# cambyse/po-rrt

Hardware: AMD Instinct MI355X
Metric: RRT node-expansions/sec on map_benchmark.pgm (higher is better)
Workload: dtype f64

## Files before the change

### po_rrt_amd/csrc/porrt_device.hpp

```cpp
#pragma once
#include <hip/hip_runtime.h>
#include <stdint.h>
#include <string>
#include <vector>
#include "../../include/porrt_hip.h"

namespace porrt {

template <int NEV>
struct ScopedEvents {
    hipEvent_t e[NEV];
    ScopedEvents() { for (int i = 0; i < NEV; ++i) e[i] = nullptr; }
    hipError_t create() {
        for (int i = 0; i < NEV; ++i) { const hipError_t r = hipEventCreate(&e[i]); if (r != hipSuccess) return r; }
        return hipSuccess;
    }
    ~ScopedEvents() { for (int i = 0; i < NEV; ++i) if (e[i]) (void)hipEventDestroy(e[i]); }
    ScopedEvents(const ScopedEvents &) = delete;
    ScopedEvents &operator=(const ScopedEvents &) = delete;
};

template <class Launch, class GoingOn>
static int sweep_to_fixpoint(hipStream_t stream, uint32_t *flags, size_t rows, int cur, Launch &&launch, GoingOn &&going_on, const char *who,
                             uint64_t &sweeps, std::string &err) {
    std::vector<uint32_t> h_flags(8 * rows), changed;
    hipError_t e;
    for (sweeps = 0;;) {
        if ((e = hipMemsetAsync(flags, 0, h_flags.size() * sizeof(uint32_t), stream)) != hipSuccess) break;
        for (uint32_t k = 0; k < 8; ++k, cur ^= 1) launch(k, cur);
        if ((e = hipMemcpyAsync(h_flags.data(), flags, h_flags.size() * sizeof(uint32_t), hipMemcpyDeviceToHost, stream)) != hipSuccess) break;
        if ((e = hipStreamSynchronize(stream)) != hipSuccess || (e = hipGetLastError()) != hipSuccess) break;
        sweeps += 8;
        changed.clear();
        for (size_t r = 0; r < rows; ++r) if (h_flags[8 * r + 7]) changed.push_back((uint32_t)r);
        if (changed.empty()) return PORRT_OK;
        if (sweeps > 16u * 1000u * 1000u) { err = std::string(who) + ": no fixpoint"; return PORRT_ERR_DEVICE; }
        if ((e = going_on(changed)) != hipSuccess) break;
    }
    err = std::string(who) + ": sweeps: " + hipGetErrorString(e);
    return PORRT_ERR_DEVICE;
}

constexpr int kConnectWaves = 4;
constexpr uint32_t kTileRMax = 31;
constexpr int kEmpty = 0x7FFFFFFF;
constexpr uint32_t kOnG = 0x80000000u;
constexpr int kParentPending = -2;

enum : uint32_t {
    ERR_RASTER = 1u,
    ERR_CAND_OVERFLOW = 2u,
    ERR_RNG_RETRY = 4u,
    ERR_EDGE_OVERFLOW = 8u,
    ERR_GPATH_OVERFLOW = 16u,
    ERR_PAGE_OVERFLOW = 32u,
    ERR_TIE_POOL = 64u
};

enum : uint8_t { CLS_FREE = 0, CLS_LOW = 1, CLS_HIGH = 2, CLS_HIGH0 = 3 , CLS_ZONE = 16, CLS_BAD = 255 };

struct __attribute__((aligned(8))) KdRec {
    double x, y;
    int child[2];
};

struct __attribute__((aligned(32))) KdBox {
    double lox, hix, loy, hiy;
};

struct KdMove {
    uint32_t t;
    int cur;
    uint32_t side, dcur, gex;
    bool onpath;
    double vx, vy;
    KdBox box;
};

struct Counters {
    uint32_t n_final;
    uint32_t n_edges;
    uint32_t err;
    uint32_t tie_fallbacks;
    unsigned long long finality;
    uint32_t g_len;
    uint32_t n_heavy;
    uint32_t g_nd_len;
    uint32_t g_first_dup[2];
    uint32_t n_pages;
    uint32_t kd_done;
    uint32_t pend_cnt, pool_n;
    uint32_t n_deferred, pend_lo;
    uint32_t n_losers;
    uint32_t kd_snap;
    uint32_t dbg[4];
    uint32_t clone_n;
    uint32_t clone_k[64];
    uint32_t coop_bar;
    uint32_t coop_filed;
    uint32_t coop_abort;
    uint32_t sched_stop;
    uint32_t sched_iter;
    uint32_t n_lca;
    uint32_t lca_next;
    unsigned long long tim[16];
};

#ifdef PORRT_TIMING
#define PORRT_T0() unsigned long long t__0 = wall_clock64()
#define PORRT_TACC(rc, slot)                                                                          \
    do {                                                                                              \
        const unsigned long long t__1 = wall_clock64();                                               \
        if ((threadIdx.x & 63u) == 0u) { atomicAdd(&(rc).cnt->tim[slot], t__1 - t__0); atomicAdd(&(rc).cnt->tim[(slot) + 8], 1ull); } \
        t__0 = t__1;                                                                                  \
    } while (0)
#else
#define PORRT_T0() do {} while (0)
#define PORRT_TACC(rc, slot) do {} while (0)
#endif
#ifndef PORRT_TIMING_FROM
#define PORRT_TIMING_FROM 0
#endif
#ifndef PORRT_TIMING_UNTIL
#define PORRT_TIMING_UNTIL 0x7FFFFFFF
#endif
#if defined(PORRT_TIMING) && PORRT_TIMING == 1
#define PORRT_TACC_A(rc, slot) do { if (b >= (uint32_t)PORRT_TIMING_FROM && b < (uint32_t)PORRT_TIMING_UNTIL) PORRT_TACC(rc, slot); else t__0 = wall_clock64(); } while (0)
#define PORRT_TACC_B(rc, slot) do { (void)t__0; } while (0)
#elif defined(PORRT_TIMING)
#define PORRT_TACC_A(rc, slot) do { (void)t__0; } while (0)
#define PORRT_TACC_B(rc, slot) do { if (b >= (uint32_t)PORRT_TIMING_FROM && b < (uint32_t)PORRT_TIMING_UNTIL) PORRT_TACC(rc, slot); else t__0 = wall_clock64(); } while (0)
#else
#define PORRT_TACC_A(rc, slot) do {} while (0)
#define PORRT_TACC_B(rc, slot) do {} while (0)
#endif
#if defined(PORRT_TIMING) && PORRT_TIMING == 3
#undef PORRT_TACC_B
#define PORRT_TACC_B(rc, slot) do { (void)t__0; } while (0)
#define PORRT_TACC_C(rc, slot) PORRT_TACC(rc, slot)
#elif defined(PORRT_TIMING)
#define PORRT_TACC_C(rc, slot) do { (void)t__0; } while (0)
#else
#define PORRT_TACC_C(rc, slot) do {} while (0)
#endif

#if defined(PORRT_TIMING) && PORRT_TIMING == 4
#undef PORRT_TACC_B
#define PORRT_TACC_B(rc, slot) do { (void)t__0; } while (0)
#define PORRT_TACC_H(rc, slot) do { if (b >= (uint32_t)PORRT_TIMING_FROM && b < (uint32_t)PORRT_TIMING_UNTIL) PORRT_TACC(rc, slot); else t__0 = wall_clock64(); } while (0)
#define PORRT_TACC_S(rc, slot) do { if (TeamT::kSize == 64 && b >= (uint32_t)PORRT_TIMING_FROM && b < (uint32_t)PORRT_TIMING_UNTIL) PORRT_TACC(rc, slot); else t__0 = wall_clock64(); } while (0)
#elif defined(PORRT_TIMING)
#define PORRT_TACC_H(rc, slot) do { (void)t__0; } while (0)
#define PORRT_TACC_S(rc, slot) PORRT_TACC_B(rc, slot)
#else
#define PORRT_TACC_H(rc, slot) do {} while (0)
#define PORRT_TACC_S(rc, slot) do {} while (0)
#endif

struct BestCost {
    unsigned long long cost_bits;
    uint32_t final_id, path_len, overflow, pad;
};

typedef float flt2 __attribute__((ext_vector_type(2)));
struct RunConst {
    double *nx, *ny;
    int *rep;
    flt2 *rep_f;
    double bx0, by0, binv_w, binv_h;
    uint32_t *rg_cnt;
    unsigned long long *rg_occ;
    uint32_t *rg_dir;
    double *pg_xy;
    int *pg_id;
    double *pg_d;
    uint32_t *slot_of;
    uint32_t rg_maxp, pg_cap;
    double *distA, *distB;
    int *parent;
    unsigned long long *reachA, *reachB;
    uint8_t *vid;
    uint8_t *final_flag;
    unsigned long long *final_mask;
    uint32_t *n_at;
    unsigned long long *valid_mask;
    Counters *cnt;
    double *sx, *sy;
    uint32_t *sworld;
    const double *inj_xy;
    unsigned long long inj_base, inj_n;
    double *q_x, *q_y;
    double *kq_x, *kq_y;
    int *kq_vid;
    int *q_nn;
    int *q_vid;
    uint32_t *cand_cnt;
    int *cand_id;
    double *cand_val;
    double *cand_xy;
    uint32_t cand_cap;
    uint32_t cand_K;
    const double *rad_T2;
    uint32_t *e_from, *e_to, *e_tv;
    uint32_t e_cap;
    KdRec *kd_rec;
    KdBox *kd_box;
    KdBox *loc_box;
    uint32_t loc_stride;
    KdMove *kd_losers;
    int *pend_new, *pend_pool;
    uint32_t *pend_off, *pend_n, *pend_cur, *pend_state;
    uint32_t pend_cap, pool_cap;
    int *bc_scratch;
    uint32_t bc_cap;
    uint32_t *bc_cursor;
    BestCost *bc_out;
    unsigned long long *kd_hint;
    int *kd_up;
    uint32_t *kd_depth;
    uint32_t *kd_gexit;
    int *loc_cur;
    uint32_t *loc_dcur, *loc_gex, *loc_flags, *g_nd;
    double *g_nd_x, *g_nd_y;
    KdBox *g_nd_box;
    int *g_id;
    double *g_x, *g_y;
    uint32_t g_cap;
    uint32_t *g_snap;
    double gp_x, gp_y;
    const uint8_t *cls;
    const uint32_t *sat;
    const uint8_t *clr;
    uint32_t W, H;
    double low0, low1, ppm;
    int domain, has_grid;
    int n_validities;
    unsigned long long validities[65];
    unsigned long long all_worlds;
    int goal_kind;
    uint32_t G;
    double gcx[64], gcy[64];
    unsigned long long gmask[64];
    double g_l1;
    double w2g_x[64], w2g_y[64];
    double zone_x, zone_y, visibility;
    double s_low0, s_low1, s_up0, s_up1;
    double max_step;
    int mode;
    uint16_t *perm;
    double *ssx, *ssy;
    double *bq_x, *bq_y;
    uint16_t *bq_k;
    double *t2_at;
    uint32_t tile_R;
    uint32_t part_stride;
    uint32_t q_stride;
    double start_x, start_y;
    unsigned long long root_reach;
    int root_vid;
    unsigned long long rng_st_lo, rng_st_hi, rng_inc_lo, rng_inc_hi;
    struct PcgJump *jump;
    RunConst *self;
    uint32_t *zero0;
    unsigned long long zero_words;
    uint32_t *sched_i0, *sched_nb;
    uint32_t sched_min, sched_max, sched_K, sched_steps;
    uint32_t sched_max_nodes;
    uint32_t cand_par3;
    uint32_t hint_max;
    uint32_t kd_lazy;
};

#define GPTR(T) T __attribute__((address_space(1))) *
template <class T>
__device__ __forceinline__ GPTR(T) as_global(T *p) { return (GPTR(T))(uintptr_t)p; }
template <class T>
__device__ __forceinline__ GPTR(const T) as_global(const T *p) { return (GPTR(const T))(uintptr_t)p; }
template <class T>
__device__ __forceinline__ T g_atomic_add(GPTR(T) p, T v) { return __hip_atomic_fetch_add(p, v, __ATOMIC_RELAXED, __HIP_MEMORY_SCOPE_AGENT); }
template <class T>
__device__ __forceinline__ T g_atomic_or(GPTR(T) p, T v) { return __hip_atomic_fetch_or(p, v, __ATOMIC_RELAXED, __HIP_MEMORY_SCOPE_AGENT); }
template <class T>
__device__ __forceinline__ T g_atomic_min(GPTR(T) p, T v) { return __hip_atomic_fetch_min(p, v, __ATOMIC_RELAXED, __HIP_MEMORY_SCOPE_AGENT); }

__device__ __forceinline__ uint32_t uni(uint32_t v) { return (uint32_t)__builtin_amdgcn_readfirstlane((int)v); }
__device__ __forceinline__ double uni_d(double v) {
    const unsigned long long b = (unsigned long long)__double_as_longlong(v);
    const unsigned long long lo = uni((uint32_t)b), hi = uni((uint32_t)(b >> 32));
    return __longlong_as_double((long long)(lo | (hi << 32)));
}

#ifndef PORRT_RC_SCALAR
#define PORRT_RC_SCALAR 1
#endif
__device__ __forceinline__ const RunConst &rc_const(const RunConst *p) {
#if PORRT_RC_SCALAR
    const uintptr_t a = (uintptr_t)p;
    const uintptr_t u = (uintptr_t)uni((uint32_t)a) | ((uintptr_t)uni((uint32_t)(a >> 32)) << 32);
    return *(const RunConst *)(const RunConst __attribute__((address_space(4))) *)u;
#else
    return *p;
#endif
}
__device__ __forceinline__ const RunConst &rc_const(const RunConst &rc) { return rc_const(&rc); }

__device__ __forceinline__ uint32_t row_nb(const RunConst &rc, uint32_t b, uint32_t nb_arg) {
    return rc.sched_nb ? ((GPTR(const uint32_t))(uintptr_t)rc.sched_nb)[b] : nb_arg;
}
__device__ __forceinline__ uint32_t row_i0(const RunConst &rc, uint32_t b, uint32_t i0_arg) {
// ... 204 lines not shown
    return false;
}

typedef unsigned __int128 u128;
__device__ __forceinline__ u128 mk128(unsigned long long lo, unsigned long long hi) { return ((u128)hi << 64) | lo; }

struct PcgJump {
    unsigned long long mult_lo[64], mult_hi[64], plus_lo[64], plus_hi[64];
};

__device__ __forceinline__ unsigned long long pcg_output(u128 s) {
    uint32_t rot = (uint32_t)(s >> 122);
    unsigned long long xsl = (unsigned long long)(s >> 64) ^ (unsigned long long)s;
    return (xsl >> rot) | (xsl << ((64 - rot) & 63));
}

__device__ __forceinline__ double gen_range_once(unsigned long long r, double low, double high, bool *retry) {
    double v12 = __longlong_as_double((long long)((r >> 12) | 0x3FF0000000000000ull));
    double v01 = v12 - 1.0;
    double scale = high - low;
    double prod = v01 * scale;
    double res = prod + low;
    if (!(res < high)) *retry = true;
    return res;
}

__global__ void k_gen_samples(const RunConst *__restrict__ rcp, const PcgJump *__restrict__ jt, unsigned long long it0,
                              unsigned long long n, unsigned long long st_lo, unsigned long long st_hi,
                              unsigned long long inc_lo, unsigned long long inc_hi, unsigned long long draws_before) {
    const RunConst &rc = rc_const(rcp + blockIdx.y);
    if (!jt) { jt = rc.jump; st_lo = rc.rng_st_lo; st_hi = rc.rng_st_hi; inc_lo = rc.rng_inc_lo; inc_hi = rc.rng_inc_hi; }
    unsigned long long t = (unsigned long long)blockIdx.x * blockDim.x + threadIdx.x;
    if (t >= n) return;
    if (rc.sched_nb && it0 + t >= rc.sched_max) return;
    unsigned long long idx = it0 + t;
    unsigned long long it = idx + 1;
    if (it % 100 == 0) {
        uint32_t w = rc.mode == 1 ? rc.sworld[idx] : 0u;
        double gx = 0.0, gy = 0.0;
        if (rc.goal_kind == 1) { gx = rc.w2g_x[w & 63]; gy = rc.w2g_y[w & 63]; }
        else if (rc.goal_kind == 2) { gx = rc.zone_x; gy = rc.zone_y; }
        rc.sx[idx] = gx;
        rc.sy[idx] = gy;
        return;
    }
    unsigned long long di = idx - idx / 100;
    if (rc.inj_xy) {
        unsigned long long e = rc.inj_base + di;
        if (e >= rc.inj_n) { atomicOr(&rc.cnt->err, ERR_RNG_RETRY); rc.sx[idx] = 0.0; rc.sy[idx] = 0.0; return; }
        rc.sx[idx] = rc.inj_xy[2 * e];
        rc.sy[idx] = rc.inj_xy[2 * e + 1];
        return;
    }
    (void)draws_before;
    unsigned long long delta = 2ull * di;
    u128 acc_mult = 1, acc_plus = 0;
    for (int b = 0; b < 64 && (delta >> b); ++b) {
        if ((delta >> b) & 1ull) {
            u128 m = mk128(jt->mult_lo[b], jt->mult_hi[b]), p = mk128(jt->plus_lo[b], jt->plus_hi[b]);
            acc_mult = acc_mult * m;
            acc_plus = acc_plus * m + p;
        }
    }
    const u128 MULT = mk128(0x4385DF649FCCF645ull, 0x2360ED051FC65DA4ull);
    u128 inc = mk128(inc_lo, inc_hi);
    u128 s = acc_mult * mk128(st_lo, st_hi) + acc_plus;
    bool retry = false;
    s = s * MULT + inc;
    double x = gen_range_once(pcg_output(s), rc.s_low0, rc.s_up0, &retry);
    s = s * MULT + inc;
    double y = gen_range_once(pcg_output(s), rc.s_low1, rc.s_up1, &retry);
    if (retry) atomicOr(&rc.cnt->err, ERR_RNG_RETRY);
    rc.sx[idx] = x;
    rc.sy[idx] = y;
}

constexpr int kRepLevels = 3;
__device__ __forceinline__ int rep_dim(int l) { return l == 0 ? 256 : (l == 1 ? 32 : 4); }
__device__ __forceinline__ int rep_off(int l) { return l == 0 ? 0 : (l == 1 ? 65536 : 65536 + 1024); }
constexpr int kRepTotal = 65536 + 1024 + 16;
constexpr uint32_t kRepCoarseUntil = 32768;
constexpr int kRepF = 65536 + 1024;
constexpr int kRepInts = kRepTotal + 2 * kRepF;
static_assert(kRepTotal % 2 == 0, "the positions start 8-byte aligned");

__device__ __forceinline__ void rep_cell(const RunConst &rc, double x, double y, int G, int &cx, int &cy) {
    double fx = (x - rc.bx0) * rc.binv_w * (double)G, fy = (y - rc.by0) * rc.binv_h * (double)G;
    cx = fx < 0.0 ? 0 : (fx >= (double)G ? G - 1 : (int)fx);
    cy = fy < 0.0 ? 0 : (fy >= (double)G ? G - 1 : (int)fy);
}

__device__ __forceinline__ void rep_insert(const RunConst &rc, double x, double y, int id) {
#pragma unroll
    for (int l = 0; l < kRepLevels; ++l) {
        int cx, cy;
        const int G = rep_dim(l);
        rep_cell(rc, x, y, G, cx, cy);
        rc.rep[rep_off(l) + cy * G + cx] = id;
        if (l < 2) rc.rep_f[rep_off(l) + cy * G + cx] = flt2{(float)x, (float)y};
    }
}

template <bool PTO>
__device__ __forceinline__ double nn_bound_wave(const RunConst &rc, uint32_t N, double qx, double qy, uint32_t world, uint32_t lane) {
    const double INF = __longlong_as_double(0x7FF0000000000000ll);
    double m = INF;
    for (int l = 0; l < kRepLevels; ++l) {
        const int G = rep_dim(l);
        int cx, cy;
        rep_cell(rc, qx, qy, G, cx, cy);
        int r = -1;
        if (lane < 9u) {
            const int x = cx + (int)(lane % 3u) - 1, y = cy + (int)(lane / 3u) - 1;
            if (x >= 0 && y >= 0 && x < G && y < G) r = as_global(rc.rep)[rep_off(l) + y * G + x];
        }
        double d2 = INF;
        if (r >= 0 && (uint32_t)r < N) {
            bool pass = true;
            if (PTO) pass = (as_global(rc.reachA)[r] >> world) & 1ull;
            if (pass) d2 = dist2(as_global(rc.nx)[r], as_global(rc.ny)[r], qx, qy);
        }
        for (int off = 8; off > 0; off >>= 1) {
            const double o = __shfl_xor(d2, off);
            d2 = o < d2 ? o : d2;
        }
        m = __shfl(d2, 0);
        if (m < INF) break;
    }
    if (m == INF && !PTO) m = dist2(rc.nx[0], rc.ny[0], qx, qy);
    return m;
}

__device__ __forceinline__ uint32_t rank_before(const RunConst &rc, uint32_t b, uint32_t vwords, uint32_t k);
__device__ __forceinline__ uint32_t wave_sum(uint32_t v);
__device__ void commit_rrt_sample(const RunConst &rc, uint32_t b, uint32_t vwords, uint32_t k, uint32_t lane, uint32_t stride = 64u, bool lag = false);
constexpr int kRG = 40;
constexpr uint32_t kRegions = kRG * kRG;
constexpr uint32_t kPage = 64;
constexpr uint32_t kOccWords = (kRegions + 63u) / 64u;
typedef double dbl2 __attribute__((ext_vector_type(2)));

__device__ __forceinline__ uint32_t region_of(const RunConst &rc, double x, double y) {
    int cx, cy;
    rep_cell(rc, x, y, kRG, cx, cy);
    return (uint32_t)(cy * kRG + cx);
}

__device__ __forceinline__ double disc_radius(double bound_d2, double qx, double qy) {
    return sqrt(bound_d2) * (1.0 + 1e-9) + 1e-12 * (1.0 + fabs(qx) + fabs(qy));
}

template <class Visit>
__device__ __forceinline__ void scan_disc(const RunConst &rc, uint32_t b, double qx, double qy, double rho, uint32_t N, uint32_t lane, Visit visit,
                                          uint32_t skip_region = 0xFFFFFFFFu) {
    int cx0, cy0, cx1, cy1;
    rep_cell(rc, qx - rho, qy - rho, kRG, cx0, cy0);
    rep_cell(rc, qx + rho, qy + rho, kRG, cx1, cy1);
    const uint32_t x0 = uni((uint32_t)cx0), y0 = uni((uint32_t)cy0);
    const uint32_t w = uni((uint32_t)(cx1 - cx0 + 1)), nreg = w * uni((uint32_t)(cy1 - cy0 + 1));
    if (nreg * 16u > N) {
        auto gx = as_global(rc.nx), gy = as_global(rc.ny);
        for (uint32_t j0 = 0; j0 < N; j0 += 128u) {
            double x[2], y[2];
#pragma unroll
            for (int u = 0; u < 2; ++u) {
                const uint32_t j = j0 + 64u * u + lane;
                x[u] = gx[j < N ? j : 0u];
                y[u] = gy[j < N ? j : 0u];
            }
#pragma unroll
            for (int u = 0; u < 2; ++u)
                if (j0 + 64u * u < N) visit(x[u], y[u], (int)(j0 + 64u * u + lane), j0 + 64u * u + lane < N);
        }
        return;
    }
    auto gcnt = as_global(rc.rg_cnt) + (b & 1u) * kRegions;
    auto gdir = as_global(rc.rg_dir);
    auto gxy = as_global(reinterpret_cast<const dbl2 *>(rc.pg_xy));
    auto gid = as_global(rc.pg_id);
    for (uint32_t r0 = 0; r0 < nreg; r0 += 64) {
        const uint32_t r = r0 + lane;
        uint32_t reg = 0, cnt = 0;
        if (r < nreg) {
            const uint32_t ry = r / w;
            reg = (y0 + ry) * kRG + x0 + (r - ry * w);
            cnt = reg == skip_region ? 0u : gcnt[reg];
        }
        const uint32_t npg = (uint32_t)__popcll(__ballot(cnt > 0u));
        if (__ballot(cnt >= npg || cnt > kPage) == 0ull && npg > 1u) {
            uint32_t cmax = cnt;
            for (int off = 32; off > 0; off >>= 1) {
                const uint32_t o = __shfl_xor(cmax, off);
                cmax = o > cmax ? o : cmax;
            }
            cmax = uni(cmax);
            for (uint32_t s0 = 0; s0 < cmax; s0 += 2) {
                dbl2 v[2];
                int id[2];
#pragma unroll
                for (int u = 0; u < 2; ++u) {
                    const uint32_t sl = s0 + u < cnt ? s0 + u : 0u;
                    v[u] = gxy[(size_t)reg * kPage + sl];
                    id[u] = gid[(size_t)reg * kPage + sl];
                }
#pragma unroll
                for (int u = 0; u < 2; ++u)
                    if (s0 + u < cmax) visit(v[u].x, v[u].y, id[u], s0 + u < cnt);
            }
            continue;
        }
        uint32_t page = reg;
        for (uint32_t j = 0;; ++j) {
            unsigned long long m = __ballot(cnt > j * kPage);
            if (!m) break;
            if (j && cnt > j * kPage) page = gdir[(size_t)reg * rc.rg_maxp + j];
            while (m) {
                uint32_t pg[2], pc[2];
#pragma unroll
                for (int u = 0; u < 2; ++u) {
                    pg[u] = 0; pc[u] = 0;
                    if (m) {
                        const uint32_t l = (uint32_t)__builtin_ctzll(m);
                        m &= m - 1;
                        pg[u] = (uint32_t)__builtin_amdgcn_readlane((int)page, (int)l);
                        const uint32_t c = (uint32_t)__builtin_amdgcn_readlane((int)cnt, (int)l) - j * kPage;
                        pc[u] = c < kPage ? c : kPage;
                    }
                }
                dbl2 v[2];
                int id[2];
#pragma unroll
                for (int u = 0; u < 2; ++u) {
                    const bool ld = lane < pc[u];
                    v[u] = ld ? gxy[(size_t)pg[u] * kPage + lane] : dbl2{0.0, 0.0};
                    id[u] = ld ? gid[(size_t)pg[u] * kPage + lane] : -1;
                }
#pragma unroll
                for (int u = 0; u < 2; ++u)
                    if (pc[u]) visit(v[u].x, v[u].y, id[u], lane < pc[u]);
            }
        }
    }
}

template <bool PTO>
__device__ __forceinline__ void near_sample(const RunConst &rc, uint32_t b, uint32_t i0, uint32_t vwords, uint32_t k, uint32_t lane) {
    const uint32_t N = uni(as_global(rc.n_at)[b]);
    const double sqx = uni_d(as_global(rc.sx)[i0 + k]), sqy = uni_d(as_global(rc.sy)[i0 + k]);
    uint32_t world = 0;
    if (PTO) world = uni(as_global(rc.sworld)[i0 + k]);
    const double INF = __longlong_as_double(0x7FF0000000000000ll);
    double bestD = INF;
    int best = 0x7FFFFFFF;
    const double T2 = rc.rad_T2[N + (rc.mode == 1 ? 1u : 0u)];
    {
        auto reach = as_global(rc.reachA);
        double thr = INF;
        auto visit = [&](double x, double y, int id, bool ok) {
            if (!ok) return;
            const double d2 = dist2(x, y, sqx, sqy);
            if (d2 > thr) return;
            bool pass = true;
            if (PTO) pass = (reach[id] >> world) & 1ull;
            if (!pass) return;
            const double D = sqrt(d2);
            if (D < bestD || (D == bestD && id < best)) { bestD = D; best = id; thr = d2 * (1.0 + 1e-15); }
        };
        auto wave_best = [&]() {
            double rd = bestD;
            int ri = best;
            for (int off = 32; off > 0; off >>= 1) {
                const double od = __shfl_xor(rd, off);
                const int oi = __shfl_xor(ri, off);
                if (od < rd || (od == rd && oi < ri)) { rd = od; ri = oi; }
            }
            const unsigned long long own = __ballot(best == ri && bestD == rd);
            const int src = own ? (int)__builtin_ctzll(own) : 0;
            thr = __shfl(thr, src);
            bestD = rd; best = ri;
        };
        const uint32_t own = uni(region_of(rc, sqx, sqy));
        scan_disc(rc, b, sqx, sqy, 0.0, N, lane, visit);
        wave_best();
        double m2;
        if (best != 0x7FFFFFFF) m2 = thr;
        else { m2 = nn_bound_wave<PTO>(rc, N, sqx, sqy, world, lane); thr = m2 * (1.0 + 1e-9); }
        scan_disc(rc, b, sqx, sqy, disc_radius(m2, sqx, sqy), N, lane, visit, own);
        wave_best();
    }
    const int nn = best == 0x7FFFFFFF ? 0 : best;
    const double fx = as_global(rc.nx)[nn], fy = as_global(rc.ny)[nn];
    double tx = sqx, ty = sqy;
    double step = fabs(tx - fx);
    step += fabs(ty - fy);
    if (step > rc.max_step) {
        const double lambda = rc.max_step / step;
        double ux = (tx - fx) * lambda, uy = (ty - fy) * lambda;
        tx = fx + ux;
        ty = fy + uy;
    }
    uint32_t err = 0;
    int vid = 0;
    bool valid = true;
    if (rc.has_grid) {
        int cls = state_class(rc, tx, ty, &err);
        if (rc.mode == 0) valid = cls == CLS_FREE;
        else { vid = class_to_validity(rc, cls); valid = vid >= 0; }
        if (err) valid = false;
    }
    if (lane == 0) {
        const uint32_t qo = q_off(rc, b);
        as_global(rc.q_x)[qo + k] = tx;
        as_global(rc.q_y)[qo + k] = ty;
        const size_t o2 = (size_t)b * rc.part_stride + k;
        as_global(rc.kq_x)[o2] = tx; as_global(rc.kq_y)[o2] = ty; as_global(rc.kq_vid)[o2] = valid ? vid : -1;
        as_global(rc.q_nn)[qo + k] = nn;
        as_global(rc.q_vid)[qo + k] = valid ? vid : -1;
        if (valid) atomicOr(&rc.valid_mask[(size_t)b * vwords + (k >> 6)], 1ull << (k & 63u));
        if (err) atomicOr(&rc.cnt->err, err);
    }
    if (!valid) return;
    auto cid = as_global(rc.cand_id) + cand_off(rc, b, k);
    auto cxy = as_global(reinterpret_cast<dbl2 *>(rc.cand_xy)) + cand_off(rc, b, k);
    const uint32_t cap = rc.cand_cap;
    uint32_t tot = 0;
    bool over = false;
    scan_disc(rc, b, tx, ty, disc_radius(T2, tx, ty), N, lane, [&](double x, double y, int id, bool ok) {
        const bool in = ok && dist2(x, y, tx, ty) <= T2;
        const unsigned long long hm = __ballot(in);
        const uint32_t pos = tot + (uint32_t)__popcll(hm & ((1ull << lane) - 1ull));
        if (in) {
            if (pos < cap) {
                cid[pos] = id;
                dbl2 v;
                v.x = x; v.y = y;
                cxy[pos] = v;
            } else {
                over = true;
            }
        }
        tot += (uint32_t)__popcll(hm);
    });
    if (lane == 0) as_global(rc.cand_cnt)[cand_cnt_at(rc, b, k)] = tot;
    if (over) atomicOr(&rc.cnt->err, (uint32_t)ERR_CAND_OVERFLOW);
}

template <bool PTO>
__global__ __launch_bounds__(256) void k_near(const RunConst *__restrict__ rcp, uint32_t b, uint32_t i0, uint32_t nb, uint32_t vwords, uint32_t cb,
                                              uint32_t cnb) {
    const RunConst &rc = rcp[blockIdx.y];
    const uint32_t lane = threadIdx.x & 63u;
    const uint32_t near_blocks = (nb + 3u) / 4u;
    if (blockIdx.x >= near_blocks) {
        const uint32_t ck = uni((blockIdx.x - near_blocks) * 4u + (threadIdx.x >> 6));
        if (!PTO && ck < cnb && ck < row_nb(rc, cb, cnb)) commit_rrt_sample(rc, cb, vwords, ck, lane);
        return;
    }
    const uint32_t k = uni(blockIdx.x * 4u + (threadIdx.x >> 6));
    if (k >= row_nb(rc, b, nb)) return;
    near_sample<PTO>(rc, b, row_i0(rc, b, i0), vwords, k, lane);
}

constexpr uint32_t kInsertLds = kRegions * 4u + 4096u * 2u + 16u;
template <int TAG = 0>
__device__ void insert_step_pages(const RunConst &rc_arg, uint32_t b, uint32_t nb, uint32_t vwords, uint8_t *scratch) {
    const RunConst &rc = TAG == 1 ? rc_const(rc_arg) : rc_arg;
    uint32_t *s_add = reinterpret_cast<uint32_t *>(scratch);
    uint16_t *s_off = reinterpret_cast<uint16_t *>(scratch + kRegions * 4u);
    uint32_t &s_np = *reinterpret_cast<uint32_t *>(scratch + kRegions * 4u + 4096u * 2u);
    uint32_t &s_base = *reinterpret_cast<uint32_t *>(scratch + kRegions * 4u + 4096u * 2u + 4u);
    const uint32_t T = blockDim.x;
    auto rg_old = as_global(rc.rg_cnt) + (b & 1u) * kRegions, rg_new = as_global(rc.rg_cnt) + ((b + 1u) & 1u) * kRegions;
    for (uint32_t r = threadIdx.x; r < kRegions; r += T) s_add[r] = 0;
    if (threadIdx.x < 64u) {
        uint32_t add = threadIdx.x < vwords ? (uint32_t)__popcll(as_global(rc.valid_mask)[(size_t)b * vwords + threadIdx.x]) : 0u;
        add = wave_sum(add);
        if (threadIdx.x == 0) {
        s_np = 0; s_base = kRegions + rc.cnt->n_pages;
        const uint32_t n_next = as_global(rc.n_at)[b] + add;
        as_global(rc.n_at)[b + 1] = n_next;
        as_global(rc.t2_at)[b + 1] = as_global(rc.rad_T2)[n_next];
        }
    }
    __syncthreads();
    const uint32_t qo = q_off(rc, b);
    for (uint32_t k = threadIdx.x; k < nb; k += T)
        if (rc.q_vid[qo + k] >= 0) s_off[k] = (uint16_t)atomicAdd(&s_add[region_of(rc, as_global(rc.q_x)[qo + k], as_global(rc.q_y)[qo + k])], 1u);
    __syncthreads();
    for (uint32_t r = threadIdx.x; r < kRegions; r += T) {
        const uint32_t add = s_add[r];
        if (!add) continue;
        const uint32_t old = rg_old[r];
        const uint32_t p_old = old ? (old + kPage - 1) / kPage : 1u, p_new = (old + add + kPage - 1) / kPage;
        if (p_new > p_old) {
            const uint32_t need = p_new - p_old;
            const uint32_t at = s_base + atomicAdd(&s_np, need);
            if (at + need > rc.pg_cap || p_new > rc.rg_maxp) { atomicOr(&rc.cnt->err, (uint32_t)ERR_PAGE_OVERFLOW); continue; }
            for (uint32_t i = 0; i < need; ++i) as_global(rc.rg_dir)[(size_t)r * rc.rg_maxp + p_old + i] = at + i;
        }
    }
    __syncthreads();
    if (rc.cnt->err & ERR_PAGE_OVERFLOW) return;
    const uint32_t N = as_global(rc.n_at)[b];
    dbl2 *pxy = reinterpret_cast<dbl2 *>(rc.pg_xy);
    for (uint32_t k = threadIdx.x; k < nb; k += T) {
        if (rc.q_vid[qo + k] < 0) continue;
        const double x = as_global(rc.q_x)[qo + k], y = as_global(rc.q_y)[qo + k];
        const uint32_t r = region_of(rc, x, y);
        const uint32_t slot = rg_old[r] + s_off[k], j = slot / kPage;
        const uint32_t page = j ? __hip_atomic_load(&rc.rg_dir[(size_t)r * rc.rg_maxp + j], __ATOMIC_RELAXED, __HIP_MEMORY_SCOPE_AGENT) : r;
        dbl2 v;
        v.x = x; v.y = y;
        pxy[(size_t)page * kPage + (slot % kPage)] = v;
        const uint32_t nid = N + rank_before(rc, b, vwords, k);
        as_global(rc.pg_id)[(size_t)page * kPage + (slot % kPage)] = (int)nid;
        as_global(rc.slot_of)[nid] = page * kPage + (slot % kPage);
        if (rc.q_stride) { as_global(rc.nx)[nid] = x; as_global(rc.ny)[nid] = y; }
    }
    __syncthreads();
    for (uint32_t r = threadIdx.x; r < kRegions; r += T) rg_new[r] = rg_old[r] + s_add[r];
    if (threadIdx.x < kOccWords) {
        unsigned long long w = 0;
        for (uint32_t i = 0; i < 64u; ++i) {
            const uint32_t r = threadIdx.x * 64u + i;
            if (r < kRegions && rg_old[r] + s_add[r] > 0u) w |= 1ull << i;
        }
        as_global(rc.rg_occ)[((b + 1u) & 1u) * kOccWords + threadIdx.x] = w;
    }
    if (threadIdx.x == 0) rc.cnt->n_pages += s_np;
}

constexpr uint32_t kFileLds = 2u * kRegions * 4u + 4096u * 2u + 64u * 8u + 66u * 4u + 32u;
template <uint32_t T = 1024u>
__device__ void file_step_fast(const RunConst &rc_arg, uint32_t b, uint32_t nb, uint32_t vwords, uint8_t *scratch) {
    const RunConst &rc = rc_const(rc_arg);
    uint32_t *s_add = reinterpret_cast<uint32_t *>(scratch);
    uint32_t *s_old = s_add + kRegions;
    uint16_t *s_off = reinterpret_cast<uint16_t *>(s_old + kRegions);
    unsigned long long *s_word = reinterpret_cast<unsigned long long *>(s_off + 4096);
    uint32_t *s_pref = reinterpret_cast<uint32_t *>(s_word + 64);
    uint32_t *s_misc = s_pref + 66;
    constexpr uint32_t SPT = 4u;
    const uint32_t tid = threadIdx.x, qo = q_off(rc, b);
    auto rg_old = as_global(rc.rg_cnt) + (b & 1u) * kRegions, rg_new = as_global(rc.rg_cnt) + ((b + 1u) & 1u) * kRegions;
    int vid[SPT];
    double x[SPT], y[SPT];
#pragma unroll
    for (uint32_t q = 0; q < SPT; ++q) {
        const uint32_t k = tid + q * T;
        vid[q] = k < nb ? as_global(rc.q_vid)[qo + k] : -1;
        x[q] = k < nb ? as_global(rc.q_x)[qo + k] : 0.0;
        y[q] = k < nb ? as_global(rc.q_y)[qo + k] : 0.0;
    }
    constexpr uint32_t RPT = (kRegions + T - 1u) / T;
    uint32_t oldc[RPT];
#pragma unroll
    for (uint32_t h = 0; h < RPT; ++h) oldc[h] = tid + h * T < kRegions ? rg_old[tid + h * T] : 0u;
    const unsigned long long word = tid < vwords ? as_global(rc.valid_mask)[(size_t)b * vwords + tid] : 0ull;
    uint32_t n_pages = 0, N0 = 0;
    if (tid == T - 1u) { n_pages = rc.cnt->n_pages; N0 = as_global(rc.n_at)[b]; }
#pragma unroll
    for (uint32_t h = 0; h < RPT; ++h) if (tid + h * T < kRegions) { s_add[tid + h * T] = 0; s_old[tid + h * T] = oldc[h]; }
    if (tid < 64u) s_word[tid] = word;
    if (tid == T - 1u) { s_misc[0] = 0; s_misc[1] = kRegions + n_pages; s_misc[2] = 0; s_misc[3] = N0; }
    __syncthreads();
    double t2_next = 0.0;
    if (tid == 0) {
        uint32_t acc = 0;
        for (uint32_t w = 0; w < vwords; ++w) { s_pref[w] = acc; acc += (uint32_t)__popcll(s_word[w]); }
        const uint32_t n_next = s_misc[3] + acc;
        as_global(rc.n_at)[b + 1] = n_next;
        t2_next = as_global(rc.rad_T2)[n_next];
    }
    uint32_t reg[SPT];
#pragma unroll
    for (uint32_t q = 0; q < SPT; ++q) {
        reg[q] = 0;
        if (vid[q] >= 0) { reg[q] = region_of(rc, x[q], y[q]); s_off[tid + q * T] = (uint16_t)atomicAdd(&s_add[reg[q]], 1u); }
    }
    __syncthreads();
#pragma unroll
    for (uint32_t h = 0; h < RPT; ++h) {
        const uint32_t r = tid + h * T;
        const uint32_t add = r < kRegions ? s_add[r] : 0u;
        if (!add) continue;
        const uint32_t old = s_old[r];
        const uint32_t p_old = old ? (old + kPage - 1) / kPage : 1u, p_new = (old + add + kPage - 1) / kPage;
        if (p_new > p_old) {
            const uint32_t need = p_new - p_old;
            const uint32_t at = s_misc[1] + atomicAdd(&s_misc[0], need);
            if (at + need > rc.pg_cap || p_new > rc.rg_maxp) { atomicOr(&rc.cnt->err, (uint32_t)ERR_PAGE_OVERFLOW); s_misc[2] = 1u; continue; }
            for (uint32_t i = 0; i < need; ++i) as_global(rc.rg_dir)[(size_t)r * rc.rg_maxp + p_old + i] = at + i;
        }
    }
    __threadfence_block();
    __syncthreads();
    if (s_misc[2]) return;
    const uint32_t N = s_misc[3];
    dbl2 *pxy = reinterpret_cast<dbl2 *>(rc.pg_xy);
#pragma unroll
    for (uint32_t q = 0; q < SPT; ++q) {
        if (vid[q] < 0) continue;
        const uint32_t k = tid + q * T, r = reg[q];
        const uint32_t slot = s_old[r] + s_off[k], j = slot / kPage;
        const uint32_t page = j ? __hip_atomic_load(&rc.rg_dir[(size_t)r * rc.rg_maxp + j], __ATOMIC_RELAXED, __HIP_MEMORY_SCOPE_AGENT) : r;
        dbl2 v;
        v.x = x[q]; v.y = y[q];
        pxy[(size_t)page * kPage + (slot % kPage)] = v;
        const uint32_t nid = N + s_pref[k >> 6] + (uint32_t)__popcll(s_word[k >> 6] & ((1ull << (k & 63u)) - 1ull));
        as_global(rc.pg_id)[(size_t)page * kPage + (slot % kPage)] = (int)nid;
        as_global(rc.slot_of)[nid] = page * kPage + (slot % kPage);
        as_global(rc.nx)[nid] = x[q];
        as_global(rc.ny)[nid] = y[q];
    }
#pragma unroll
    for (uint32_t h = 0; h < RPT; ++h) {
        const uint32_t r = tid + h * T;
        if (r < kRegions) rg_new[r] = s_old[r] + s_add[r];
    }
    if (tid < kOccWords) {
        unsigned long long w = 0;
        for (uint32_t i = 0; i < 64u; ++i) {
            const uint32_t r = tid * 64u + i;
            if (r < kRegions && s_old[r] + s_add[r] > 0u) w |= 1ull << i;
        }
        as_global(rc.rg_occ)[((b + 1u) & 1u) * kOccWords + tid] = w;
    }
    if (tid == 0) { as_global(rc.t2_at)[b + 1] = t2_next; rc.cnt->n_pages += s_misc[0]; }
}

__device__ __forceinline__ uint32_t rank_before(const RunConst &rc, uint32_t b, uint32_t vwords, uint32_t k) {
    uint32_t r = 0;
    auto vm = as_global(rc.valid_mask) + (size_t)b * vwords;
    for (uint32_t w = 0; w < (k >> 6); ++w) r += __popcll(vm[w]);
    r += __popcll(vm[k >> 6] & ((1ull << (k & 63u)) - 1ull));
    return r;
}
template <int CTRL>
__device__ __forceinline__ uint32_t dpp_u32(uint32_t v) { return (uint32_t)__builtin_amdgcn_update_dpp((int)v, (int)v, CTRL, 0xF, 0xF, false); }
template <int CTRL>
__device__ __forceinline__ double dpp_f64(double v) {
    const unsigned long long b = (unsigned long long)__double_as_longlong(v);
    const unsigned long long lo = dpp_u32<CTRL>((uint32_t)b), hi = dpp_u32<CTRL>((uint32_t)(b >> 32));
    return __longlong_as_double((long long)(lo | (hi << 32)));
}
constexpr int kDppRowRor = 0x120;
constexpr int kDppRowBcast = 0x150;
#ifndef PORRT_DPP
#define PORRT_DPP 1
#endif

__device__ __forceinline__ uint32_t rank_before_lanes(const RunConst &rc, uint32_t b, uint32_t vwords, uint32_t k, uint32_t lane, uint32_t stride) {
    auto vm = as_global(rc.valid_mask) + (size_t)b * vwords;
    const uint32_t wk = k >> 6;
    uint32_t r = 0;
    for (uint32_t w0 = 0; w0 <= wk; w0 += stride) {
        const uint32_t w = w0 + lane;
        unsigned long long v = w <= wk ? vm[w] : 0ull;
        if (w == wk) v &= (1ull << (k & 63u)) - 1ull;
        r += (uint32_t)__popcll(v);
    }
    if (PORRT_DPP && stride == 16u) {
        r += dpp_u32<kDppRowRor + 8>(r); r += dpp_u32<kDppRowRor + 4>(r); r += dpp_u32<kDppRowRor + 2>(r); r += dpp_u32<kDppRowRor + 1>(r);
        return r;
    }
    for (uint32_t off = stride >> 1; off > 0; off >>= 1) r += (uint32_t)__shfl_xor((int)r, (int)off);
    return r;
}

__device__ __forceinline__ TileGrid load_tile(const RunConst &rc, uint8_t *tile, double px, double py, uint32_t lane, uint32_t stride) {
    TileGrid g;
    g.lds = tile; g.glob = rc.cls; g.W = rc.W; g.TW = 2u * rc.tile_R + 1u;
    uint32_t ci, cj;
    to_pixel(rc, px, py, ci, cj);
    g.oi = (int)ci - (int)rc.tile_R;
    g.oj = (int)cj - (int)rc.tile_R;
    const uint32_t n = g.TW * g.TW;
    for (uint32_t t = lane; t < n; t += stride) {
        const uint32_t ri = t / g.TW, rj = t - ri * g.TW;
        const int i = g.oi + (int)ri, j = g.oj + (int)rj;
        uint8_t c = CLS_BAD;
        if (i >= 0 && j >= 0 && (uint32_t)i < rc.H && (uint32_t)j < rc.W) c = as_global(rc.cls)[(uint32_t)i * rc.W + (uint32_t)j];
        tile[t] = c;
    }
    return g;
}

template <class T>
__device__ __forceinline__ T wave_min_u(T v) {
    for (int off = 32; off > 0; off >>= 1) {
        T o = __shfl_xor(v, off);
        v = o < v ? o : v;
    }
    return v;
}
__device__ __forceinline__ uint32_t wave_sum(uint32_t v) {
    for (int off = 32; off > 0; off >>= 1) v += __shfl_xor(v, off);
    return v;
}
__device__ __forceinline__ unsigned long long wave_or(unsigned long long v) {
    for (int off = 32; off > 0; off >>= 1) v |= __shfl_xor(v, off);
    return v;
}

__device__ __forceinline__ bool kd_left(double x, double y, double wx, double wy, uint32_t depth) {
    return (depth & 1u) ? (y < wy) : (x < wx);
}

__device__ bool kd_preorder_less(const RunConst &rc, int u, int v) {
    const uint32_t gu = as_global(rc.kd_gexit)[u], gv = as_global(rc.kd_gexit)[v];
    const bool ou = gu & kOnG, ov = gv & kOnG;
    const uint32_t iu = gu & ~kOnG, iv = gv & ~kOnG;
    if (ou && ov) return iu < iv;
    if (ou) {
        if (iu <= iv) return true;
        return !kd_left(as_global(rc.nx)[v], as_global(rc.ny)[v], as_global(rc.g_x)[iv], as_global(rc.g_y)[iv], iv);
    }
    if (ov) {
        if (iv <= iu) return false;
        return kd_left(as_global(rc.nx)[u], as_global(rc.ny)[u], as_global(rc.g_x)[iu], as_global(rc.g_y)[iu], iu);
    }
    if (iu != iv) {
        if (iu < iv) return kd_left(as_global(rc.nx)[u], as_global(rc.ny)[u], as_global(rc.g_x)[iu], as_global(rc.g_y)[iu], iu);
        return !kd_left(as_global(rc.nx)[v], as_global(rc.ny)[v], as_global(rc.g_x)[iv], as_global(rc.g_y)[iv], iv);
    }
    int a = u, b = v;
    uint32_t da = as_global(rc.kd_depth)[a], db = as_global(rc.kd_depth)[b];
    int a_from = -1, b_from = -1;
    while (da > db) { const int p = as_global(rc.kd_up)[a]; a_from = as_global(rc.kd_rec)[p].child[1] == a; a = p; --da; }
    while (db > da) { const int p = as_global(rc.kd_up)[b]; b_from = as_global(rc.kd_rec)[p].child[1] == b; b = p; --db; }
    if (a == b) return a_from >= 0 ? false : true;
    while (a != b) {
        const int pa = as_global(rc.kd_up)[a], pb = as_global(rc.kd_up)[b];
        a_from = as_global(rc.kd_rec)[pa].child[1] == a;
        b_from = as_global(rc.kd_rec)[pb].child[1] == b;
        a = pa; b = pb;
    }
    return a_from < b_from;
}

template <int W>
struct Team {
    static constexpr bool kOneWave = W == 1;
    static constexpr uint32_t kSize = W * 64u;
    double *scr_d;
    int *scr_i;
    uint32_t wave, lane;
    __device__ __forceinline__ uint32_t tl() const { return wave * 64u + lane; }
    __device__ __forceinline__ uint32_t sub() const { return lane; }
    __device__ __forceinline__ unsigned long long ballot(bool p) const { return __ballot(p); }
    template <class T>
    __device__ __forceinline__ T shfl(T v, int src) const { return __shfl(v, src); }
    __device__ __forceinline__ void sync() const { if (W > 1) __syncthreads(); }
    __device__ __forceinline__ uint32_t sum(uint32_t v) const {
        v = wave_sum(v);
        if (W == 1) return v;
        sync();
        if (lane == 0) scr_i[wave] = (int)v;
        sync();
        uint32_t t = 0;
#pragma unroll
        for (int w = 0; w < W; ++w) t += (uint32_t)scr_i[w];
        return t;
    }
    __device__ __forceinline__ int min_i(int v) const {
        v = wave_min_u(v);
// ... 726 lines not shown

__global__ __launch_bounds__(1024) void k_file_commit(const RunConst *__restrict__ rcp, uint32_t bf, uint32_t nbf, uint32_t cb, uint32_t cnb, uint32_t vwords) {
    __shared__ __attribute__((aligned(16))) uint8_t s_ins[kFileLds];
    const RunConst &rc = rcp[blockIdx.y];
    if (blockIdx.x == 0) { file_step_fast<1024u>(rc, bf, nbf, vwords, s_ins); return; }
    const uint32_t ck = uni((blockIdx.x - 1u) * 16u + (threadIdx.x >> 6));
    if (ck < cnb) commit_rrt_sample(rc, cb, vwords, ck, threadIdx.x & 63u);
}

__device__ __forceinline__ bool coop_grid_sync(const RunConst &rc, uint32_t nblocks, uint32_t &phase) {
    __shared__ uint32_t s_go;
    __syncthreads();
    if (threadIdx.x == 0) {
        ++phase;
        const uint32_t target = phase * nblocks;
        __threadfence();
        __hip_atomic_fetch_add(&rc.cnt->coop_bar, 1u, __ATOMIC_RELEASE, __HIP_MEMORY_SCOPE_AGENT);
        const unsigned long long t0 = wall_clock64();
        uint32_t go = 1u;
        while (__hip_atomic_load(&rc.cnt->coop_bar, __ATOMIC_RELAXED, __HIP_MEMORY_SCOPE_AGENT) < target) {
            __builtin_amdgcn_s_sleep(1);
            if (wall_clock64() - t0 > 200000000ull || __hip_atomic_load(&rc.cnt->coop_abort, __ATOMIC_RELAXED, __HIP_MEMORY_SCOPE_AGENT)) {
                atomicOr(&rc.cnt->coop_abort, 1u); go = 0u; break;
            }
        }
        __builtin_amdgcn_fence(__ATOMIC_ACQUIRE, "agent");
        s_go = go;
    }
    __syncthreads();
    __builtin_amdgcn_s_dcache_inv();
    return s_go != 0u;
}

template <bool LDSGRID>
__global__ __launch_bounds__(kConnectWaves * 64) __attribute__((amdgpu_waves_per_eu(8, 8))) void k_coop_rrt(const RunConst *__restrict__ rcp, uint32_t n_steps, uint32_t K,
                                                                  uint32_t n_iter, uint32_t vwords) {
    extern __shared__ __attribute__((aligned(16))) uint8_t lds_tiles[];
    __shared__ double s_d[kConnectWaves];
    __shared__ int s_i[kConnectWaves];
    __shared__ uint32_t s_heavy[kConnectWaves];
    __shared__ __attribute__((aligned(16))) uint8_t s_ins[kFileLds];
    const RunConst &rc = rcp[0];
    const uint32_t bid = blockIdx.x, nblk = gridDim.x, lane = threadIdx.x & 63u, wv = threadIdx.x >> 6;
    uint32_t phase = 0;
    auto nb_of = [&](uint32_t b) { const uint32_t i0 = b * K; return b < n_steps ? (n_iter - i0 < K ? n_iter - i0 : K) : 0u; };
    {
        const uint32_t nb0 = nb_of(0);
        for (uint32_t it = bid; it * 4u < nb0; it += nblk) {
            const uint32_t k = uni(it * 4u + wv);
            if (k < nb0) near_sample<false>(rc, 0u, 0u, vwords, k, lane);
        }
        if (!coop_grid_sync(rc, nblk, phase)) return;
        if (bid == 0) file_step_fast<kConnectWaves * 64u>(rc, 0u, nb0, vwords, s_ins);
        if (!coop_grid_sync(rc, nblk, phase)) return;
        if (bid == 0 && threadIdx.x == 0) __hip_atomic_store(&rc.cnt->coop_filed, 1u, __ATOMIC_RELEASE, __HIP_MEMORY_SCOPE_AGENT);
    }
    for (uint32_t b = 0; b < n_steps; ++b) {
        const uint32_t nb = nb_of(b), nbn = nb_of(b + 1u), i0n = (b + 1u) * K;
        const uint32_t cb4 = (nb + kConnectWaves - 1u) / kConnectWaves, items = cb4 + (nbn + 3u) / 4u;
        for (uint32_t it = bid; it < items; it += nblk) {
            if (it < cb4) {
                connect_block<LDSGRID>(rc, b, nb, vwords, it, lds_tiles, s_d, s_i, s_heavy);
                __syncthreads();
            } else {
                const uint32_t k = uni((it - cb4) * 4u + wv);
                if (k < nbn) near_sample<false>(rc, b + 1u, i0n, vwords, k, lane);
            }
        }
        if (!coop_grid_sync(rc, nblk, phase)) return;
        const uint32_t first_commit = nbn ? 1u : 0u;
        if (nbn && bid == 0) file_step_fast<kConnectWaves * 64u>(rc, b + 1u, nbn, vwords, s_ins);
        if (bid >= first_commit) {
            for (uint32_t it = bid - first_commit; it * 4u < nb; it += nblk - first_commit) {
                const uint32_t ck = uni(it * 4u + wv);
                if (ck < nb) commit_rrt_sample(rc, b, vwords, ck, lane);
            }
        }
        if (!coop_grid_sync(rc, nblk, phase)) return;
        if (bid == 0 && threadIdx.x == 0) __hip_atomic_store(&rc.cnt->coop_filed, b + 2u, __ATOMIC_RELEASE, __HIP_MEMORY_SCOPE_AGENT);
    }
}

__device__ void commit_rrt_sample(const RunConst &rc, uint32_t b, uint32_t vwords, uint32_t k, uint32_t lane, uint32_t stride, bool lag) {
    const unsigned long long vword = as_global(rc.valid_mask)[(size_t)b * vwords + (k >> 6)];
    const uint32_t N = as_global(rc.n_at)[b];
    const uint32_t rank = stride < 64u ? rank_before_lanes(rc, b, vwords, k, lane, stride) : rank_before(rc, b, vwords, k);
    const uint32_t cnt = cand_count(rc, b, k);
    auto cid = as_global(rc.cand_id) + cand_off(rc, b, k);
    auto cval = as_global(rc.cand_val) + cand_val_off(rc, b, k);
    if (!((vword >> (k & 63u)) & 1ull)) return;
    const int id = (int)(N + rank);
    const bool odd = lag && (b & 1u);
    auto gdB = as_global(odd ? rc.distA : rc.distB);
    auto gother = as_global(reinterpret_cast<unsigned long long *>(odd ? rc.distB : rc.distA));
    auto gpd = as_global(rc.pg_d);
    auto gso = as_global(rc.slot_of);
    if (lane == 0) gpd[gso[id]] = as_global(rc.distA)[id];
    constexpr int U = 4;
    for (uint32_t a0 = lane; a0 < cnt; a0 += stride * U) {
        double via[U], dB[U];
        int j[U];
#pragma unroll
        for (int u = 0; u < U; ++u) {
            const uint32_t a = a0 + (uint32_t)u * stride;
            via[u] = a < cnt ? cval[a] : -1.0;
            j[u] = a < cnt ? cid[a] : 0;
        }
#pragma unroll
        for (int u = 0; u < U; ++u) dB[u] = via[u] >= 0.0 ? gdB[j[u]] : 0.0;
#pragma unroll
        for (int u = 0; u < U; ++u) {
            if (!(via[u] >= 0.0) || f64_bits(via[u]) != f64_bits(dB[u])) continue;
            auto gpar = as_global(rc.parent) + j[u];
            int old = *gpar;
            while (old < (int)N || id < old) {
                int expect = old;
                if (__hip_atomic_compare_exchange_strong(gpar, &expect, id, __ATOMIC_RELAXED, __ATOMIC_RELAXED, __HIP_MEMORY_SCOPE_AGENT)) break;
                old = expect;
            }
            if (lag) g_atomic_min(gother + j[u], f64_bits(via[u]));
            else as_global(rc.distA)[j[u]] = via[u];
            gpd[gso[j[u]]] = via[u];
        }
    }
}

__global__ __launch_bounds__(256) void k_commit_rrt(const RunConst *__restrict__ rcp, uint32_t b, uint32_t nb, uint32_t vwords, uint32_t lag) {
    const uint32_t k = uni((blockIdx.x * 256u + threadIdx.x) >> 6);
    if (k < nb && k < row_nb(rcp[blockIdx.y], b, nb)) commit_rrt_sample(rcp[blockIdx.y], b, vwords, k, threadIdx.x & 63u, 64u, lag != 0u);
}

template <int TAG> __device__ void g_track_step(const RunConst &rc_arg, uint32_t b, uint32_t nb, uint32_t vwords, uint8_t *lds) {
    const RunConst &rc = rc_const(rc_arg);
#ifdef PORRT_GTRACK_TIMING
    const unsigned long long gt0 = wall_clock64();
#define GT_MARK(slot) do { if (threadIdx.x == 0) { atomicAdd(&rc.cnt->tim[slot], wall_clock64() - gt0); atomicAdd(&rc.cnt->tim[(slot) + 8], 1ull); } } while (0)
#else
#define GT_MARK(slot) do {} while (0)
#endif
    constexpr uint32_t kNd = kGTrackNd;
    uint16_t *s_k = reinterpret_cast<uint16_t *>(lds);
    unsigned long long *s_cand = reinterpret_cast<unsigned long long *>(lds + 8192);
    uint32_t *s_wpre = reinterpret_cast<uint32_t *>(lds + 8192 + 512);
    double *s_blx = reinterpret_cast<double *>(lds + 8192 + 512 + 272);
    double *s_bhx = s_blx + kNd, *s_bly = s_bhx + kNd, *s_bhy = s_bly + kNd;
    uint32_t *s_ndi = reinterpret_cast<uint32_t *>(s_bhy + kNd);
    constexpr uint32_t kApp = 256, kCand = 160;
    double *s_ax = reinterpret_cast<double *>(lds + kGTrackLds0), *s_ay = s_ax + kApp;
    double *s_cx = s_ay + kApp, *s_cy = s_cx + kCand;
    const uint32_t tid = threadIdx.x, lane = tid & 63u;
    auto vm = as_global(rc.valid_mask) + (size_t)b * vwords;
    const uint32_t N = as_global(rc.n_at)[b];
    const uint32_t glen0 = rc.cnt->g_len, n_nd = rc.cnt->g_nd_len, d0 = rc.cnt->g_first_dup[0], d1 = rc.cnt->g_first_dup[1];
    if (tid < 64u) s_cand[tid] = 0ull;
    if (tid < 64u) {
        const uint32_t c = tid < vwords ? (uint32_t)__popcll(vm[tid]) : 0u;
        uint32_t inc = c;
        for (int off = 1; off < 64; off <<= 1) { const uint32_t o = (uint32_t)__shfl_up((int)inc, off); if ((int)lane >= off) inc += o; }
        if (tid < vwords) s_wpre[tid] = inc - c;
        if (tid == 63u) s_wpre[vwords] = inc;
    }
    for (uint32_t t2 = tid; t2 < n_nd && t2 < kNd; t2 += blockDim.x) {
        const KdBox bx = rc.g_nd_box[t2];
        s_ndi[t2] = as_global(rc.g_nd)[t2]; s_blx[t2] = bx.lox; s_bhx[t2] = bx.hix; s_bly[t2] = bx.loy; s_bhy[t2] = bx.hiy;
    }
    __syncthreads();
    const uint32_t n_new = s_wpre[vwords];
    for (uint32_t k = tid; k < nb; k += blockDim.x) {
        const unsigned long long w = vm[k >> 6];
        if ((w >> (k & 63u)) & 1ull) s_k[s_wpre[k >> 6] + (uint32_t)__popcll(w & ((1ull << (k & 63u)) - 1ull))] = (uint16_t)k;
    }
    __syncthreads();
    const double px = rc.gp_x, py = rc.gp_y;
    auto gex = as_global(rc.kd_gexit);
    const uint32_t qo = q_off(rc, b);
    GT_MARK(0);
    for (uint32_t t0 = tid; t0 < ((n_new + blockDim.x - 1u) / blockDim.x) * blockDim.x; t0 += 4u * blockDim.x) {
        double cvx[4], cvy[4];
        uint32_t cE[4], lo[4], hi[4];
#pragma unroll
        for (uint32_t u = 0; u < 4u; ++u) {
            const uint32_t t = t0 + u * blockDim.x;
            const uint32_t k = t < n_new ? s_k[t] : 0u;
            cvx[u] = t < n_new ? as_global(rc.q_x)[qo + k] : 0.0;
            cvy[u] = t < n_new ? as_global(rc.q_y)[qo + k] : 0.0;
            cE[u] = 0xFFFFFFFFu;
            const bool open = t < n_new && !(cvx[u] == px && cvy[u] == py);
            lo[u] = 0u; hi[u] = open ? n_nd : 0u;
        }
        for (;;) {
            bool more = false;
#pragma unroll
            for (uint32_t u = 0; u < 4u; ++u) more = more || lo[u] < hi[u];
            if (!more) break;
#pragma unroll
            for (uint32_t u = 0; u < 4u; ++u) {
                if (lo[u] >= hi[u]) continue;
                const uint32_t mid = (lo[u] + hi[u]) >> 1;
                double blx, bhx, bly, bhy;
                if (mid < kNd) { blx = s_blx[mid]; bhx = s_bhx[mid]; bly = s_bly[mid]; bhy = s_bhy[mid]; }
                else { const KdBox bx = rc.g_nd_box[mid]; blx = bx.lox; bhx = bx.hix; bly = bx.loy; bhy = bx.hiy; }
                const bool in = !(cvx[u] < blx) && cvx[u] < bhx && !(cvy[u] < bly) && cvy[u] < bhy;
                if (in) lo[u] = mid + 1u; else hi[u] = mid;
            }
        }
        GT_MARK(4);
#pragma unroll
        for (uint32_t u = 0; u < 4u; ++u) {
            const uint32_t t = t0 + u * blockDim.x;
            if (t < n_new && !(cvx[u] == px && cvy[u] == py) && lo[u] < n_nd) cE[u] = lo[u] < kNd ? s_ndi[lo[u]] : as_global(rc.g_nd)[lo[u]];
        }
#pragma unroll
        for (uint32_t u = 0; u < 4u; ++u) {
            const uint32_t t = t0 + u * blockDim.x;
            if (t >= n_new) continue;
            uint32_t E = cE[u];
            if (cvx[u] < px && d0 < E) E = d0;
            if (cvy[u] < py && d1 < E) E = d1;
            if (E != 0xFFFFFFFFu) gex[N + t] = E;
            else atomicOr(&s_cand[t >> 6], 1ull << (t & 63u));
        }
    }
    __syncthreads();
    GT_MARK(5);
    if (tid < 64u) {
        const uint32_t c = (uint32_t)__popcll(s_cand[tid]);
        uint32_t inc = c;
        for (int off = 1; off < 64; off <<= 1) { const uint32_t o = (uint32_t)__shfl_up((int)inc, off); if ((int)lane >= off) inc += o; }
        s_wpre[tid] = inc - c;
    }
    __syncthreads();
    for (uint32_t t = tid; t < n_new; t += blockDim.x) {
        const unsigned long long w = s_cand[t >> 6];
        if (!((w >> (t & 63u)) & 1ull)) continue;
        const uint32_t rank = s_wpre[t >> 6] + (uint32_t)__popcll(w & ((1ull << (t & 63u)) - 1ull));
        if (rank < kCand) { const uint32_t k = s_k[t]; s_cx[rank] = as_global(rc.q_x)[qo + k]; s_cy[rank] = as_global(rc.q_y)[qo + k]; }
    }
    __syncthreads();
    GT_MARK(1);
    if (tid < 64u) {
        uint32_t len = glen0, nd_len = n_nd, fd0 = d0, fd1 = d1;
        KdBox cell = n_nd ? rc.g_nd_box[n_nd - 1u] : g_box_all();
        auto gx = as_global(reinterpret_cast<unsigned long long *>(rc.g_x)), gy = as_global(reinterpret_cast<unsigned long long *>(rc.g_y));
        uint32_t c_at = 0;
        for (uint32_t w = 0; w < (n_new + 63u) / 64u; ++w) {
            for (unsigned long long m = s_cand[w]; m;) {
                const uint32_t t = w * 64u + (uint32_t)__builtin_ctzll(m);
                m &= m - 1ull;
                double vx, vy;
                if (c_at < kCand) { vx = s_cx[c_at]; vy = s_cy[c_at]; }
                else { const uint32_t k = s_k[t]; vx = as_global(rc.q_x)[qo + k]; vy = as_global(rc.q_y)[qo + k]; }
                ++c_at;
                uint32_t E = 0xFFFFFFFFu;
                if (!(vx == px && vy == py)) {
                    for (uint32_t l0 = glen0; l0 < len && E == 0xFFFFFFFFu; l0 += 64u) {
                        const uint32_t lvl = l0 + lane;
                        bool out = false;
                        if (lvl < len) {
                            double wx, wy;
                            if (lvl - glen0 < kApp) { wx = s_ax[lvl - glen0]; wy = s_ay[lvl - glen0]; }
                            else {
                                __builtin_amdgcn_s_waitcnt(0);
                                wx = __longlong_as_double((long long)__hip_atomic_load(gx + lvl, __ATOMIC_RELAXED, __HIP_MEMORY_SCOPE_AGENT));
                                wy = __longlong_as_double((long long)__hip_atomic_load(gy + lvl, __ATOMIC_RELAXED, __HIP_MEMORY_SCOPE_AGENT));
                            }
                            out = kd_left(vx, vy, wx, wy, lvl) != kd_left(px, py, wx, wy, lvl);
                        }
                        const unsigned long long ob = __ballot(out);
                        if (ob) E = l0 + (uint32_t)__builtin_ctzll(ob);
                    }
                }
                if (lane == 0) {
                    if (E != 0xFFFFFFFFu) {
                        gex[N + t] = E;
                    } else {
                        if (len + 8u < rc.g_cap) {
                            as_global(rc.g_id)[len] = (int)(N + t);
                            __hip_atomic_store(gx + len, (unsigned long long)__double_as_longlong(vx), __ATOMIC_RELAXED, __HIP_MEMORY_SCOPE_AGENT);
                            __hip_atomic_store(gy + len, (unsigned long long)__double_as_longlong(vy), __ATOMIC_RELAXED, __HIP_MEMORY_SCOPE_AGENT);
                        } else {
                            atomicOr(&rc.cnt->err, (uint32_t)ERR_GPATH_OVERFLOW);
                        }
                        if (len - glen0 < kApp) { s_ax[len - glen0] = vx; s_ay[len - glen0] = vy; }
                        gex[N + t] = len | kOnG;
                        if (!(vx == px && vy == py)) {
                            as_global(rc.g_nd)[nd_len] = len; as_global(rc.g_nd_x)[nd_len] = vx; as_global(rc.g_nd_y)[nd_len] = vy;
                            cell = g_box_after(cell, vx, vy, len, px, py);
                            rc.g_nd_box[nd_len] = cell;
                        }
                    }
                }
                if (E == 0xFFFFFFFFu) {
                    if (vx == px && vy == py) { if (len & 1u) fd1 = len < fd1 ? len : fd1; else fd0 = len < fd0 ? len : fd0; }
                    else ++nd_len;
                    ++len;
                }
                __builtin_amdgcn_fence(__ATOMIC_RELEASE, "workgroup", "local");
                __builtin_amdgcn_wave_barrier();
                __builtin_amdgcn_fence(__ATOMIC_ACQUIRE, "workgroup", "local");
            }
        }
        GT_MARK(2);
        if (lane == 0) {
            rc.cnt->g_len = len; rc.cnt->g_nd_len = nd_len; rc.cnt->g_first_dup[0] = fd0; rc.cnt->g_first_dup[1] = fd1;
            __threadfence();
            __hip_atomic_store(&rc.cnt->kd_done, N + n_new, __ATOMIC_RELEASE, __HIP_MEMORY_SCOPE_AGENT);
        }
        GT_MARK(3);
    }
}

__global__ __launch_bounds__(256) void k_gtrack(const RunConst *__restrict__ rcp, uint32_t b, uint32_t nb, uint32_t vwords) {
    __shared__ __attribute__((aligned(16))) uint8_t s_lds[kGTrackLds];
    const RunConst &rc = rcp[blockIdx.y];
    nb = row_nb(rc, b, nb);
    if (nb == 0) return;
    g_track_step<1>(rc, b, nb, vwords, s_lds);
}

__global__ __launch_bounds__(256) void k_kd_reset(const RunConst *__restrict__ rcp) {
    const RunConst &rc = rcp[blockIdx.y];
    for (uint32_t i = blockIdx.x * 256u + threadIdx.x; i < (uint32_t)(128 * 128); i += gridDim.x * 256u) rc.kd_hint[i] = 0ull;
    if (blockIdx.x == 0 && threadIdx.x == 0) {
        const double x = rc.nx[0], y = rc.ny[0];
        rc.cnt->g_len = 1;
        rc.cnt->g_first_dup[0] = 0xFFFFFFFFu;
        rc.cnt->g_first_dup[1] = 0xFFFFFFFFu;
        if (x == rc.gp_x && y == rc.gp_y) { rc.cnt->g_first_dup[0] = 0; rc.cnt->g_nd_len = 0; }
        else { rc.g_nd[0] = 0; rc.g_nd_x[0] = x; rc.g_nd_y[0] = y; rc.g_nd_box[0] = g_box_after(g_box_all(), x, y, 0u, rc.gp_x, rc.gp_y); rc.cnt->g_nd_len = 1; }
        rc.kd_rec[0].child[0] = kEmpty; rc.kd_rec[0].child[1] = kEmpty;
        rc.cnt->kd_done = 1;
        rc.cnt->kd_snap = 0;
        rc.cnt->n_losers = 0;
        rc.g_snap[0] = 1; rc.g_snap[1] = rc.cnt->g_nd_len; rc.g_snap[2] = rc.cnt->g_first_dup[0]; rc.g_snap[3] = rc.cnt->g_first_dup[1];
    }
}

enum : uint32_t { LOC_SIDE = 1u, LOC_ONPATH = 2u };
constexpr uint32_t kWaitFiled = 0x80000000u;
__device__ __forceinline__ bool coop_wait_filed(const RunConst &rc, uint32_t need) {
    __shared__ uint32_t s_ok;
    if (threadIdx.x == 0) {
        const unsigned long long t0 = wall_clock64();
        uint32_t ok = 1u;
        while (__hip_atomic_load(&rc.cnt->coop_filed, __ATOMIC_ACQUIRE, __HIP_MEMORY_SCOPE_AGENT) < need) {
            __builtin_amdgcn_s_sleep(64);
            if (wall_clock64() - t0 > 200000000ull || __hip_atomic_load(&rc.cnt->coop_abort, __ATOMIC_RELAXED, __HIP_MEMORY_SCOPE_AGENT)) {
                atomicOr(&rc.cnt->coop_abort, 1u); ok = 0u; break;
            }
        }
        s_ok = ok;
    }
    __syncthreads();
    return s_ok != 0u;
}
constexpr int kHG = 128;
constexpr uint32_t kHintMaxSquares = 256;

__device__ __forceinline__ KdBox load_box(const KdBox *p, size_t i) {
    auto g = as_global(p);
    KdBox b;
    b.lox = g[i].lox; b.hix = g[i].hix; b.loy = g[i].loy; b.hiy = g[i].hiy;
    return b;
}
__device__ __forceinline__ bool box_holds(const KdBox &bx, double x, double y) {
    return bx.lox <= x && x < bx.hix && bx.loy <= y && y < bx.hiy;
}
__device__ __forceinline__ void box_cut(KdBox &bx, double wx, double wy, uint32_t depth, uint32_t side) {
    if (depth & 1u) { if (side) bx.loy = wy; else bx.hiy = wy; }
    else { if (side) bx.lox = wx; else bx.hix = wx; }
}

__device__ __forceinline__ void kd_descend(const RunConst &rc, uint32_t Nsnap, double vx, double vy, int &cur, uint32_t &dcur, uint32_t &side,
                                           KdBox &bx) {
    auto grec = as_global(rc.kd_rec);
    KdRec rec;
    rec.x = grec[cur].x; rec.y = grec[cur].y; rec.child[0] = grec[cur].child[0]; rec.child[1] = grec[cur].child[1];
    for (;;) {
        box_cut(bx, rec.x, rec.y, dcur, side);
        const int c = side ? rec.child[1] : rec.child[0];
        if ((uint32_t)c >= Nsnap) break;
        rec.x = grec[c].x; rec.y = grec[c].y; rec.child[0] = grec[c].child[0]; rec.child[1] = grec[c].child[1];
        cur = c;
        dcur += 1;
        side = kd_left(vx, vy, rec.x, rec.y, dcur) ? 0u : 1u;
    }
}

constexpr uint32_t kTieParts = 8;
__device__ __forceinline__ void kd_hint_block(const RunConst &rc, uint32_t b0, uint32_t nsteps, uint32_t vwords, uint32_t bx);
template <int T>
__device__ __forceinline__ void tie_fix_block(const RunConst &rc, uint32_t part, uint32_t nparts);
template <int LPN>
__global__ __launch_bounds__(256) void k_kd_locate(const RunConst *__restrict__ rcp, uint32_t b0, uint32_t nsteps, uint32_t K, uint32_t nb_last,
                                                    uint32_t vwords, uint32_t lpar, uint32_t hb0 = 0, uint32_t hns = 0) {
// ... 804 lines not shown
```

### po_rrt_amd/csrc/porrt_engine.hip

```cpp
#include "../../include/porrt_hip.h"
#include "porrt_host.hpp"
#include "porrt_device.hpp"
#include "porrt_group.hpp"
#include "porrt_belief.hpp"
#include "porrt_dp.hpp"
#include "porrt_prm.hpp"
#include "porrt_edges.hpp"
#include "porrt_refine.hpp"
#include "porrt_refine_batch.hpp"
#include "porrt_reparent.hpp"
#include "porrt_qmdp.hpp"
#include "porrt_policy_graph.hpp"
#include "porrt_join.hpp"
#include "porrt_mm_recipe.hpp"

#include <algorithm>
#include <functional>
#include <chrono>
#include <cmath>
#include <cstdio>
#include <cstring>
#include <string>
#include <system_error>
#include <mutex>
#include <thread>
#include <unordered_map>
#include <limits>
#include <memory>
#include <vector>

template <class F> static inline auto abi_guard(F &&f) noexcept -> decltype(f()) {
    try { return f(); } catch (const std::bad_alloc &) { return PORRT_ERR_NOMEM; } catch (...) { return PORRT_ERR_INVALID; }
}

using namespace porrt;

namespace {

struct DevBufBase {
    void *vp = nullptr;
    size_t n = 0, want = 0, elem = 1;
};
template <class T>
struct DevBuf : DevBufBase {
    T *p = nullptr;
    DevBuf() { elem = sizeof(T); }
    hipError_t reserve(size_t w) { if (w > want) want = w; return hipSuccess; }
    void release() {}
};
struct Arena {
    void *base = nullptr;
    size_t cap = 0;
};

}

#include "porrt_mmprm.hpp"
#include "porrt_mmplan.hpp"
#include "porrt_policy.hpp"
#include "porrt_launch.hpp"

struct MmRoadmapDev {
    double *x, *y;
    uint32_t *base, *rank, *deg, *err, *seg, *aux, *sz, *tmp, *from, *to;
    int *child, *par;
    unsigned long long *off, *tot;
    unsigned long long E;
};

struct porrt_ctx {
    int device = 0;
    hipStream_t stream = nullptr;
    std::string err;
    void set_err(const std::string &s) { err = s; }

    std::vector<uint8_t> occ, zones, cls;
    uint32_t W = 0, H = 0;
    double low[2] = {0, 0}, up[2] = {0, 0}, ppm = 0;
    int domain = 0;
    bool has_grid = false, cls_dirty = true;
    double visibility = 0;
    int n_zones = 0, n_worlds = 1, n_validities = 1;
    double zone_pos[64][2];
    uint64_t validities[65];
    double s_low[2] = {-1, -1}, s_up[2] = {1, 1};
    Pcg64 crng, drng;
    std::vector<double> inj_xy;
    size_t inj_pos = 0;
    bool has_inj = false, inj_dirty = false;
    std::vector<uint32_t> inj_worlds;
    size_t inj_wpos = 0;
    bool has_inj_worlds = false;
    int goal_kind = 0;
    uint32_t G = 0;
    double gcx[64], gcy[64];
    uint64_t gmask[64];
    double g_l1 = 0;
    double w2g[64][2];
    uint32_t obs_zone = 0;
    bool opt_profile = false;
    bool opt_graph = true;
    uint32_t opt_kd_group = 0;
    bool opt_kd_after = false;
    int opt_kd_inline = 0;
    int opt_kd_lazy = 1;
    uint32_t opt_claim_threads = 0;
    int opt_host_ranks = 1;
    int opt_compact = 1;
    uint32_t n_compactions = 0;
    int opt_kd_ride = 0;
    int opt_group_req = -1;
    uint32_t opt_early_wave = 0;
    uint32_t opt_conn_wg_waves = 1;
    bool opt_conn_riders_first = true;
    uint32_t opt_nn_wg_waves = 4;
    uint32_t opt_commit_flat = 1;
    uint32_t opt_batch_streams = 0;
    int opt_pipeline = 4;
    std::vector<void *> dl_pin;
    std::vector<hipStream_t> dl_streams;
    std::vector<size_t> dl_pin_cap;
    hipStream_t dl_out_stream = nullptr;
    TreeOut *d_tree_out = nullptr;
    size_t d_tree_out_cap = 0;
    uint32_t opt_tree_out_blocks = 4;
    uint32_t opt_fetch_workers = 8;
    bool sub_eager = false;
    int last_launch_mode = 0;
    uint32_t sub_streams_tried = 0;
    std::vector<hipStream_t> sub_streams;
    bool opt_gtrack_side = false;
    bool opt_box_table = true;
    bool opt_dp_sweeps = false;
    uint64_t opt_dp_wide_rows = kDpWideRows;
    uint32_t opt_cand_cap = 2048;
    uint64_t edge_per_node = 256, tie_pool_mult = 16;
    uint64_t tie_pool_ids = 0;
    DevBuf<double> d_nx, d_ny, d_distA, d_distB, d_sx, d_sy, d_qx, d_qy, d_pgxy, d_pgd, d_candxy, d_candval, d_radT2, d_inj, d_ssx, d_ssy, d_bqx, d_bqy, d_t2at;
    DevBuf<int> d_parent, d_qnn, d_qvid, d_pgid, d_candid, d_gid, d_kdup;
    DevBuf<KdRec> d_kdrec;
    DevBuf<KdBox> d_kdbox, d_locbox, d_gndbox;
    DevBuf<KdMove> d_kdlosers;
    DevBuf<int> d_bcscratch;
    DevBuf<BestCost> d_bcout;
    DevBuf<uint32_t> d_bccursor;
    DevBuf<int> d_loccur;
    DevBuf<uint32_t> d_locdcur, d_locgex, d_locflags, d_kdsurv;
    DevBuf<double> d_gx, d_gy, d_gndx, d_gndy, d_kqx, d_kqy;
    DevBuf<int> d_kqvid;
    DevBuf<uint32_t> d_rgcnt, d_rgdir, d_gsnap, d_pendoff, d_pendn, d_pendcur, d_pendstate;
    DevBuf<int> d_pendnew, d_pendpool;
    DevBuf<int> d_rep;
    DevBuf<uint32_t> d_kddepth, d_kdgexit;
    DevBuf<unsigned long long> d_reachA, d_reachB, d_finalmask, d_validmask, d_kdhint, d_rgocc;
    DevBuf<uint8_t> d_vid, d_finalflag, d_cls;
    DevBuf<uint32_t> d_nat, d_sworld, d_candcnt, d_efrom, d_eto, d_etv;
    DevBuf<uint16_t> d_perm, d_bqk;
    DevBuf<uint32_t> d_slotof;
    DevBuf<uint32_t> d_sched_i0, d_sched_nb;
    DevBuf<Counters> d_cnt;
    DevBuf<RunConst> d_rc;
    DevBuf<PcgJump> d_jump;
    Arena arena;
    std::vector<DevBufBase *> all_bufs;
    int layout_buffers();
    std::vector<double> radT2;
    double rad_max_step = -1, rad_search_radius = -1;
    int rad_mode = -1;
    size_t rad_uploaded = 0;
    bool jump_valid = false;
    PcgJump jump_host;
    u128 jump_inc = 0;
    RunConst rc;
    int mode = 0;
    uint64_t n_iter = 0, n_nodes = 0, n_steps = 0;
    Counters counters;
    bool complete = false;
    bool have_results = false;
    std::vector<double> h_nx, h_ny, h_dist;
    std::vector<int> h_parent;
    std::vector<unsigned long long> h_reach, h_finalmask;
    std::vector<uint8_t> h_vid, h_finalflag;
    std::vector<uint64_t> h_final_ids;
    std::vector<uint32_t> h_efrom, h_eto, h_etv;
    porrt_metrics metrics;
    std::vector<hipEvent_t> ev_pool;

    int build_cls();
    int ensure_radius_table(double max_step, double search_radius, size_t n_needed);
    int grow(const double start[2], double max_step, double search_radius, uint64_t n_iter_min, uint64_t n_iter_max,
             uint32_t K, int mode);
    int grow_once(const double start[2], double max_step, double search_radius, uint64_t n_iter_min, uint64_t n_iter_max,
                  uint32_t K, int mode, bool host_samples, int stage = 0);
    void about_to_grow();
    int ensure_profile_events(size_t want) {
        while (ev_pool.size() < want) { hipEvent_t e; HIPCHK(hipEventCreate(&e)); ev_pool.push_back(e); }
        return PORRT_OK;
    }
    int finish_growth(const Counters &hc, uint32_t n_final_nodes, uint64_t iters, uint32_t steps, uint32_t own_steps, float device_ms, bool member, const Pcg64 *host_rng);
    int profile_summary(uint32_t steps, size_t ev_used, uint32_t K, uint64_t n_iter_min, uint64_t n_iter_max, porrt_ctx *const *rows, uint32_t n_rows, bool batch);
    hipError_t ensure_compact_rows(uint32_t n);
    Pcg64 batch_drng0;
    size_t batch_wpos0 = 0;
    uint64_t batch_world_draws = 0;
    void rewind_worlds(uint64_t n_iter_done) {
        if (has_inj_worlds) inj_wpos = batch_wpos0 + n_iter_done;
        else { drng = batch_drng0; for (uint64_t t = 0; t < n_iter_done; ++t) (void)drng.gen_range_usize((uint64_t)n_worlds); }
    }
    BatchOut *d_batch_out = nullptr;
    uint32_t *d_active = nullptr, *h_active = nullptr;
    RunConst *d_rcarr_c[2] = {nullptr, nullptr};
    uint32_t *d_live_idx = nullptr;
    size_t rcarr_c_cap = 0;
    size_t active_cap = 0;
    std::vector<RunConst> rc_staging;
    std::vector<uint32_t> worlds_staging;
    size_t batch_out_cap = 0;
    size_t run_lds_bytes = 0;
    int best_cost_device(double *cost, uint64_t *final_id);
    BeliefGraphState bg;
    int build_belief_graph(const double *start_belief, uint32_t n_worlds_in);
    DpState dp;
    int compute_expected_costs();
    int extract_policy();
    PoliciesResult policies, mm_policies, policy, mm_policy;
    void mm_policy_states(PoliciesResult &res) const;
    bool costs_current() const { return bg.valid && dp.valid && bg_graph_tag == results_tag && costs_stamp == bg_stamp; }
    bool mm_costs_current() const { return mm.valid && mmp.valid && mmp.gen == mm.gen && mmp.costs_gen == mmp.gen && mmp.dp.valid; }
    bool policies_current(const PoliciesResult &res) const { return res.valid && costs_current() && res.tag == results_tag && res.stamp == bg_stamp; }
    bool mm_policies_current(const PoliciesResult &res) const { return res.valid && mm_costs_current() && res.tag == mmp.gen && res.stamp == mm_costs_runs; }
    GrowScratch policies_scratch;
    uint32_t opt_policy_max_nodes = 1u << 16;
    int policies_last = 0;
    uint64_t costs_stamp = ~0ull;
    uint64_t mm_costs_runs = 0;
    int64_t extract_policies(const uint64_t *starts, uint64_t n, uint64_t *pol_off, uint8_t *status, double *expected_costs, uint64_t *original_ids,
                             int64_t *parents, uint8_t *is_leaf, uint64_t cap);
    int64_t mm_extract_policies(const uint64_t *starts, uint64_t n, uint64_t *pol_off, uint8_t *status, double *expected_costs, uint64_t *original_ids,
                                int64_t *parents, uint8_t *is_leaf, double *xy, uint64_t cap);
    uint64_t bg_stamp = 0;
    uint64_t raster_gen = 1, cls_host_gen = 0;
    void classify_raster();
    void raster_view(RunConst &g, const uint8_t *d_raster) const;
    int refine_raster(RunConst &g);
    RefineHost refine;
    double refine_total_s = 0, refine_device_s = 0;
    bool refine_done = false;
    struct porrt_refine_policies_info refp_info = {};
    bool refp_done = false;
    bool opt_refine_short_lds = true;
    struct RefineInBuf { std::vector<double> xy; std::vector<uint32_t> row; std::vector<unsigned long long> compat; };
    RefinePoliciesIn refine_in(const PoliciesResult &res, RefineInBuf &buf) const;
    RefinePoliciesIn mm_refine_in(const PoliciesResult &res, RefineInBuf &buf) const;
    int64_t refine_call(const char *who, bool single, const RefinePoliciesIn &in, uint64_t n_iter, const RefinePoliciesOut &out, double *expected_cost);
    ReparentResult reparented;
    struct porrt_reparent_policies_info rp_info = {};
    bool rp_done = false;
    uint32_t opt_reparent_max_tree_nodes = 16384;
    uint32_t opt_reparent_max_pops_per_node = 64;
    int64_t reparent_call(const char *who, bool single, const ReparentGraph &gr, const RefinePoliciesIn &in, double radius, ReparentResult &res);
    PrmState prm;
    PrmPathsResult prm_paths;
    GrowScratch prm_paths_scratch;
    uint32_t opt_prm_rows = 256;
    uint32_t opt_prm_xcd_rows = 1;
    int ensure_prm_weights();
    int prm_answer(const double *starts, const double *goals, uint64_t n, PrmPathsResult &res, const char *who, bool single);
// ... 268 lines not shown
    rc.ny[0] = y;
    rc.parent[0] = -1;
    rc.distA[0] = 0.0;
    rc.distB[0] = 0.0;
    rc.reachA[0] = reach;
    rc.reachB[0] = reach;
    rc.vid[0] = (uint8_t)vid;
    rc.final_flag[0] = 0;
    rc.final_mask[0] = 0;
    rc.n_at[0] = 1;
    rc.t2_at[0] = 0.0;
    rep_insert(rc, x, y, 0);
    {
        const uint32_t r = region_of(rc, x, y);
        rc.pg_xy[2 * ((size_t)r * kPage)] = x; rc.pg_xy[2 * ((size_t)r * kPage) + 1] = y;
        rc.pg_id[(size_t)r * kPage] = 0;
        rc.pg_d[(size_t)r * kPage] = 0.0;
        rc.slot_of[0] = r * kPage;
        rc.rg_cnt[r] = 1;
        for (uint32_t w = 0; w < kOccWords; ++w) rc.rg_occ[w] = w == r / 64u ? 1ull << (r % 64u) : 0ull;
    }
    rc.g_id[0] = 0;
    rc.cnt->g_len = 1;
    rc.cnt->g_first_dup[0] = 0xFFFFFFFFu;
    rc.cnt->g_first_dup[1] = 0xFFFFFFFFu;
    if (x == rc.gp_x && y == rc.gp_y) { rc.cnt->g_first_dup[0] = 0; rc.cnt->g_nd_len = 0; }
    else { rc.g_nd[0] = 0; rc.g_nd_x[0] = x; rc.g_nd_y[0] = y; rc.g_nd_box[0] = g_box_after(g_box_all(), x, y, 0u, rc.gp_x, rc.gp_y); rc.cnt->g_nd_len = 1; }
    KdRec rec;
    rec.x = x; rec.y = y; rec.child[0] = kEmpty; rec.child[1] = kEmpty;
    rc.kd_rec[0] = rec;
    rc.g_x[0] = x;
    rc.g_y[0] = y;
    rc.kd_up[0] = -1;
    {
        const double INF = __longlong_as_double(0x7FF0000000000000ll);
        KdBox bx;
        bx.lox = -INF; bx.hix = INF; bx.loy = -INF; bx.hiy = INF;
        rc.kd_box[0] = bx;
    }
    rc.kd_depth[0] = 0;
    rc.kd_gexit[0] = kOnG;
    rc.cnt->kd_done = 1;
    rc.cnt->kd_snap = 0;
    rc.g_snap[0] = 1; rc.g_snap[1] = rc.cnt->g_nd_len; rc.g_snap[2] = rc.cnt->g_first_dup[0]; rc.g_snap[3] = rc.cnt->g_first_dup[1];
}

__global__ void k_wait_us(uint32_t us) {
    const unsigned long long t0 = wall_clock64();
    while (wall_clock64() - t0 < 100ull * us) __builtin_amdgcn_s_sleep(8);
}
void LaunchSeq::launch_step(uint32_t b, uint32_t i0, uint32_t nb, bool prof, size_t &ev_used, uint32_t nxt_i0, uint32_t nxt_nb) {
    const uint32_t wave_blocks = (nb * 64 + 255) / 256;
    const hipStream_t stream = cx.stream, stream2 = cx.stream2;
    const hipEvent_t ev_steered = cx.ev_steered;
    auto ev = [&](void) {
        if (prof && ev_used < cx.ev_pool.size()) (void)hipEventRecord(cx.ev_pool[ev_used++], stream);
    };
    const bool rrt = mode == PORRT_MODE_RRT;
    if (rrt && lag_on && opt_group == 0) {
        ev();
        if (lag_near_done != b) {
            hipLaunchKernelGGL(k_near<false>, dim3(wave_blocks, Q), dim3(256), 0, stream, rcp, b, i0, nb, vwords, 0xFFFFFFFFu, 0u);
        }
        ev();
        (void)hipEventRecord(ev_steered, stream);
        ev();
        const uint32_t cb4 = (nb + kConnectWaves - 1) / kConnectWaves;
        const uint32_t cnb = commit_pend_b != 0xFFFFFFFFu ? commit_pend_nb : 0u;
        const bool gt_side = kd_lazy && cx.opt_gtrack_side && !prof;
        if (gt_side) {
            if (gt_pend) (void)hipStreamWaitEvent(stream, cx.ev_kd[gt_par], 0);
            (void)hipStreamWaitEvent(stream2, ev_steered, 0);
            hipLaunchKernelGGL(k_gtrack, dim3(1, Q), dim3(256), 0, stream2, rcp, b, nb, vwords);
            gt_par ^= 1u;
            (void)hipEventRecord(cx.ev_kd[gt_par], stream2);
            gt_pend = true;
        }
        const uint32_t lazy = (kd_lazy && !gt_side) ? 1u : 0u;
        const dim3 xg(cb4 + (nxt_nb + 3) / 4 + 1 + lazy + (cnb + 3) / 4, Q);
        if (lds_bytes) hipLaunchKernelGGL(k_step1_rrt<true>, xg, dim3(256), lds_bytes, stream, rcp, b, nb, nxt_i0, nxt_nb, vwords, commit_pend_b, cnb, lazy);
        else hipLaunchKernelGGL(k_step1_rrt<false>, xg, dim3(256), 0, stream, rcp, b, nb, nxt_i0, nxt_nb, vwords, commit_pend_b, cnb, lazy);
        ev();
        lag_near_done = nxt_nb ? b + 1 : 0xFFFFFFFFu;
        commit_pend_b = b; commit_pend_nb = nb;
        kd_last_b = b; kd_last_nb = nb;
        side_active = true;
        if (!cx.opt_kd_after && !kd_lazy && b + 1 - kd_b0 >= kd_group) launch_kd_group();
        return;
    }
    if (rrt && pipe_on && opt_group == 0) {
        const uint32_t cb4 = (nb + kConnectWaves - 1) / kConnectWaves;
        ev();
        if (pipe_near_done != b) {
            hipLaunchKernelGGL(k_near<false>, dim3(wave_blocks, Q), dim3(256), 0, stream, rcp, b, i0, nb, vwords, 0xFFFFFFFFu, 0u);
            const uint32_t cnb = commit_pend_b != 0xFFFFFFFFu ? commit_pend_nb : 0u;
            hipLaunchKernelGGL(k_file_commit, dim3(1 + (cnb + 15) / 16, Q), dim3(1024), 0, stream, rcp, b, nb, commit_pend_b, cnb, vwords);
            commit_pend_b = 0xFFFFFFFFu;
        }
        ev();
        (void)hipEventRecord(ev_steered, stream);
        ev();
        const dim3 sg(cb4 + (nxt_nb + 3) / 4, Q);
        if (lds_bytes) hipLaunchKernelGGL(k_step_rrt<true>, sg, dim3(256), lds_bytes, stream, rcp, b, nb, nxt_i0, nxt_nb, vwords);
        else hipLaunchKernelGGL(k_step_rrt<false>, sg, dim3(256), 0, stream, rcp, b, nb, nxt_i0, nxt_nb, vwords);
        ev();
        if (nxt_nb) {
            hipLaunchKernelGGL(k_file_commit, dim3(1 + (nb + 15) / 16, Q), dim3(1024), 0, stream, rcp, b + 1, nxt_nb, b, nb, vwords);
            pipe_near_done = b + 1;
        } else {
            commit_pend_b = b; commit_pend_nb = nb;
            pipe_near_done = 0xFFFFFFFFu;
        }
        kd_last_b = b; kd_last_nb = nb;
        side_active = true;
        if (!cx.opt_kd_after && b + 1 - kd_b0 >= kd_group) launch_kd_group();
        return;
    }
    ev();
    const uint32_t GLn = rrt ? opt_group : 0u;
    const uint32_t GLc = (GLn == 16u && b < cx.opt_early_wave) ? 64u : GLn;
    if (mode == PORRT_MODE_PTO) hipLaunchKernelGGL(k_near<true>, dim3(wave_blocks, Q), dim3(256), 0, stream, rcp, b, i0, nb, vwords, 0xFFFFFFFFu, 0u);
    else if (GLn) {
        const uint32_t spb = cx.opt_nn_wg_waves * 64u / GLn, sblocks = (nb + spb - 1) / spb;
        const uint32_t cflat = cx.opt_commit_flat, cspb = cflat ? kSpan : spb;
        const uint32_t cblocks = commit_pend_b != 0xFFFFFFFFu ? (commit_pend_nb + cspb - 1) / cspb : 0;
        const dim3 g(sblocks + cblocks, Q);
        const uint32_t cnb = cblocks ? commit_pend_nb : 0u;
        if (cx.opt_nn_wg_waves == 1u) with_lanes(GLn, [&](auto gl) { hipLaunchKernelGGL((k_nn2<decltype(gl)::value, 1>), g, dim3(64), 0, stream, rcp, b, i0, nb, vwords, commit_pend_b, cnb, cflat); });
        else with_lanes(GLn, [&](auto gl) { hipLaunchKernelGGL(k_nn2<decltype(gl)::value>, g, dim3(256), 0, stream, rcp, b, i0, nb, vwords, commit_pend_b, cnb, cflat); });
        commit_pend_b = 0xFFFFFFFFu;
    } else {
        const uint32_t cblocks = commit_pend_b != 0xFFFFFFFFu ? (commit_pend_nb + 3) / 4 : 0;
        hipLaunchKernelGGL(k_near<false>, dim3(wave_blocks + cblocks, Q), dim3(256), 0, stream, rcp, b, i0, nb, vwords, commit_pend_b, cblocks ? commit_pend_nb : 0u);
        commit_pend_b = 0xFFFFFFFFu;
    }
    ev();
    const dim3 cgrid((nb + kConnectWaves - 1) / kConnectWaves + 1, Q), cblock(kConnectWaves * 64);
    if (!rrt) {
        ev();
        if (lds_bytes) hipLaunchKernelGGL(k_connect_pto<true>, cgrid, cblock, lds_bytes, stream, rcp, b, nb, vwords);
        else hipLaunchKernelGGL(k_connect_pto<false>, cgrid, cblock, 0, stream, rcp, b, nb, vwords);
        ev();
        hipLaunchKernelGGL(k_commit_pto, dim3(wave_blocks, Q), dim3(256), 0, stream, rcp, b, nb, vwords);
        return;
    }
    (void)hipEventRecord(ev_steered, stream);
    ev();
    if (GLn) {
        const uint32_t lazy = kd_lazy ? 1u : 0u;
        if (cx.opt_conn_wg_waves == 4u) {
            const uint32_t spb = 256u / GLc;
            const dim3 g2((nb + spb - 1) / spb + 2 + lazy, Q);
            const size_t dyn = conn2_wg4_lds_bytes(GLc);
            with_lanes(GLc, [&](auto gl) { hipLaunchKernelGGL(k_conn2_wg4<decltype(gl)::value>, g2, dim3(256), dyn, stream, rcp, b, nb, vwords, lazy); });
        } else {
            const uint32_t spb = 64u / GLc;
            const dim3 g2((nb + spb - 1) / spb, Q), gr(2 + lazy, Q);
            const size_t dyn = conn2_lds_bytes(GLc);
            if (cx.opt_conn_riders_first) hipLaunchKernelGGL(k_conn2_riders, gr, dim3(256), conn2_riders_lds_bytes(), stream, rcp, b, nb, vwords, lazy);
            with_lanes(GLc, [&](auto gl) { hipLaunchKernelGGL(k_conn2<decltype(gl)::value>, g2, dim3(64), dyn, stream, rcp, b, nb, vwords); });
            if (!cx.opt_conn_riders_first) hipLaunchKernelGGL(k_conn2_riders, gr, dim3(256), conn2_riders_lds_bytes(), stream, rcp, b, nb, vwords, lazy);
        }
    } else if (lds_bytes) hipLaunchKernelGGL(k_connect_rrt<true>, cgrid, cblock, lds_bytes, stream, rcp, b, nb, vwords);
    else hipLaunchKernelGGL(k_connect_rrt<false>, cgrid, cblock, 0, stream, rcp, b, nb, vwords);
    ev();
    commit_pend_b = b; commit_pend_nb = nb;
    kd_last_b = b; kd_last_nb = nb;
    side_active = true;
    if (!cx.opt_kd_after && !kd_lazy && b + 1 - kd_b0 >= kd_group) launch_kd_group();
}

static void launch_kd_claim(hipStream_t st, const RunConst *rcp, uint32_t Q, uint32_t b0, uint32_t ns, uint32_t K, uint32_t vwords, uint32_t threads) {
    const uint64_t nodes = (uint64_t)ns * K;
    if (Q == 1 && threads == 0) {
        if (nodes <= 2048u) hipLaunchKernelGGL(k_kd_claim<2048>, dim3(1, 1), dim3(1024), 0, st, rcp, b0, ns, vwords);
        else hipLaunchKernelGGL(k_kd_claim<kClaimMax>, dim3(1, 1), dim3(1024), 0, st, rcp, b0, ns, vwords);
        return;
    }
    if (threads == 0) threads = 256u;
    if (nodes <= 1024u) {
        if (threads <= 256u) hipLaunchKernelGGL((k_kd_claim<1024, false, 256>), dim3(1, Q), dim3(256), 0, st, rcp, b0, ns, vwords);
        else if (threads <= 512u) hipLaunchKernelGGL((k_kd_claim<1024, false, 512>), dim3(1, Q), dim3(512), 0, st, rcp, b0, ns, vwords);
        else hipLaunchKernelGGL((k_kd_claim<1024, false, 1024>), dim3(1, Q), dim3(1024), 0, st, rcp, b0, ns, vwords);
    } else if (nodes <= 2048u) {
        if (threads <= 256u) hipLaunchKernelGGL((k_kd_claim<2048, false, 256>), dim3(1, Q), dim3(256), 0, st, rcp, b0, ns, vwords);
        else if (threads <= 512u) hipLaunchKernelGGL((k_kd_claim<2048, false, 512>), dim3(1, Q), dim3(512), 0, st, rcp, b0, ns, vwords);
        else hipLaunchKernelGGL((k_kd_claim<2048, false, 1024>), dim3(1, Q), dim3(1024), 0, st, rcp, b0, ns, vwords);
    } else {
        if (threads <= 512u) hipLaunchKernelGGL((k_kd_claim<kClaimMax, false, 512>), dim3(1, Q), dim3(512), 0, st, rcp, b0, ns, vwords);
        else hipLaunchKernelGGL((k_kd_claim<kClaimMax, false, 1024>), dim3(1, Q), dim3(1024), 0, st, rcp, b0, ns, vwords);
    }
}

void LaunchSeq::kd_group_on(hipStream_t st, uint32_t b0, uint32_t ns, uint32_t nb_last, uint32_t wait, uint32_t hint_b0, uint32_t hint_ns, KdClaim claim, KdThen then) {
    const uint32_t per_node = (ns * K + 255) / 256;
    const uint32_t extra = hint_ns ? (hint_ns * K + 255) / 256 + kTieParts : 0;
    if ((uint64_t)ns * K * Q >= 4096u) hipLaunchKernelGGL(k_kd_locate<1>, dim3(per_node + extra, Q), dim3(256), 0, st, rcp, b0, ns, K, nb_last, vwords, wait, hint_b0, hint_ns);
    else hipLaunchKernelGGL(k_kd_locate<64>, dim3((ns * K * 64 + 255) / 256 + extra, Q), dim3(256), 0, st, rcp, b0, ns, K, nb_last, vwords, wait, hint_b0, hint_ns);
    hipLaunchKernelGGL(k_kd_link, dim3(per_node, Q), dim3(256), 0, st, rcp, b0, ns, vwords, 0u);
    if (claim == KdClaim::SingleSide) hipLaunchKernelGGL((k_kd_claim<kClaimMax, true>), dim3(1, 1), dim3(1024), 0, st, rcp, b0, ns, vwords);
    else launch_kd_claim(st, rcp, Q, b0, ns, K, vwords, claim == KdClaim::Plain ? 0u : cx.opt_claim_threads);
    if (then == KdThen::Hint) hipLaunchKernelGGL(k_kd_hint, dim3(per_node, Q), dim3(256), 0, st, rcp, b0, ns, vwords);
    else if (then == KdThen::HintFix) hipLaunchKernelGGL(k_kd_hint_fix, dim3(per_node + kTieParts, Q), dim3(256), 0, st, rcp, b0, ns, vwords);
}

void LaunchSeq::launch_kd_group() {
    if (kd_b0 > kd_last_b) return;
    const hipStream_t stream = cx.stream, stream2 = cx.stream2;
    const uint32_t nsteps = kd_last_b - kd_b0 + 1;
    if (cx.opt_kd_inline && Q > 1) {
        kd_group_on(stream, kd_b0, nsteps, kd_last_nb, 0u, 0u, 0u, KdClaim::ByRows, KdThen::HintFix);
        ++kd_gidx;
        kd_b0 = kd_last_b + 1;
        return;
    }
    (void)hipStreamWaitEvent(stream2, cx.ev_steered, 0);
    const bool ride = cx.opt_kd_ride != 0 || Q == 1;
    const uint32_t hns = ride ? kd_hint_ns : 0u;
    kd_group_on(stream2, kd_b0, nsteps, kd_last_nb, 0u, hns ? kd_hint_b0 : 0u, hns, Q == 1 ? KdClaim::SingleSide : KdClaim::ByRows, ride ? KdThen::Nothing : KdThen::Hint);
    if (ride) {
        kd_hint_b0 = kd_b0; kd_hint_ns = nsteps;
    } else {
        (void)hipEventRecord(cx.ev_step_done, stream);
        (void)hipStreamWaitEvent(stream2, cx.ev_step_done, 0);
        hipLaunchKernelGGL(k_tie_fix<256>, dim3(1, Q), dim3(256), 0, stream2, rcp);
    }
    const uint32_t ring = Q == 1 ? 3u : 2u;
    const uint32_t par = kd_gidx % ring, oldest = (kd_gidx + 1u) % ring;
    (void)hipEventRecord(cx.ev_kd[par], stream2);
    kd_pend[par] = true;
    if (kd_pend[oldest]) { (void)hipStreamWaitEvent(stream, cx.ev_kd[oldest], 0); kd_pend[oldest] = false; }
    ++kd_gidx;
    kd_b0 = kd_last_b + 1;
}

static uint32_t kd_group_for(uint32_t K, uint32_t opt, uint32_t Q) {
    const uint32_t cap = std::max<uint32_t>(1u, std::min<uint32_t>(8u, kClaimMax / K));
    uint32_t g = std::max<uint32_t>(1u, std::min<uint32_t>(8u, (Q > 1 ? 2048u : kClaimMax) / K));
    if (opt) g = std::min(opt, cap);
    return g;
}

LaunchForms porrt_ctx::launch_forms(int mode_, uint32_t Q, uint32_t K, bool row_plans, int stage) const {
    LaunchForms f;
    const bool rrt = mode_ == PORRT_MODE_RRT;
    f.group = opt_group_req < 0 ? ((stage == 2 && Q >= 8) ? 16u : 0u) : (uint32_t)opt_group_req;
    f.pipe = stage != 1 && rrt && opt_pipeline != 0 && f.group == 0 && !row_plans;
    f.lag = stage == 0 && f.pipe && opt_pipeline == 4 && K <= 1024;
    f.kd_lazy = opt_kd_lazy && (f.group != 0 || f.lag) && rrt && !opt_kd_after;
    return f;
}

void LaunchSeq::begin(const RunConst *rows, uint32_t n_rows, uint32_t K_, int mode_, size_t lds, const LaunchForms &f) {
    rcp = rows; Q = n_rows;
    K = K_; vwords = (K_ + 63) / 64; mode = mode_; lds_bytes = lds;
    opt_group = f.group; pipe_on = f.pipe; lag_on = f.lag; kd_lazy = f.kd_lazy;
    kd_group = kd_group_for(K_, cx.opt_kd_group, n_rows);
    kd_built_after = 0;
    lag_near_done = pipe_near_done = 0xFFFFFFFFu;
    kd_last_b = 0; kd_last_nb = 0;
    gt_pend = false; gt_par = 0;
    side_active = false; kd_build_now = false;
    rewind_kd();
}

void LaunchSeq::rewind_kd() {
    kd_b0 = 0; kd_gidx = 0; kd_hint_ns = 0;
    kd_pend[0] = kd_pend[1] = kd_pend[2] = false;
    commit_pend_b = 0xFFFFFFFFu;
}

void LaunchSeq::flush_commit() {
    if (commit_pend_b == 0xFFFFFFFFu) return;
    const hipStream_t stream = cx.stream;
    const uint32_t cb = commit_pend_b, cnb = commit_pend_nb;
    if (opt_group && cx.opt_commit_flat) hipLaunchKernelGGL(k_commit_flat, dim3((cnb + kSpan - 1) / kSpan, Q), dim3(256), 0, stream, rcp, cb, cnb, vwords);
    else with_lanes(opt_group, [&](auto gl) {
        constexpr int GL = decltype(gl)::value;
        if constexpr (GL == 64) hipLaunchKernelGGL(k_commit_rrt, dim3((cnb * 64 + 255) / 256, Q), dim3(256), 0, stream, rcp, cb, cnb, vwords, lag_on ? 1u : 0u);
        else hipLaunchKernelGGL(k_commit2<GL>, dim3((cnb * GL + 255) / 256, Q), dim3(256), 0, stream, rcp, cb, cnb, vwords);
    });
    commit_pend_b = 0xFFFFFFFFu;
}

uint32_t LaunchSeq::launch_steps(uint64_t n_iter, bool prof, size_t &ev_used) {
    uint64_t i = 0;
    uint32_t b = 0;
    while (i < n_iter) {
        const uint32_t nb = (uint32_t)std::min<uint64_t>(K, n_iter - i);
        const uint64_t i2 = i + nb;
        const uint32_t nb2 = i2 < n_iter ? (uint32_t)std::min<uint64_t>(K, n_iter - i2) : 0;
        launch_step(b, (uint32_t)i, nb, prof, ev_used, (uint32_t)i2, nb2);
        i += nb;
        ++b;
    }
    join_side();
    return b;
}

int LaunchSeq::replay_steps(uint64_t n_iter, double *t_capture) {
    const uint64_t key[6] = {(uint64_t)mode, K, n_iter, lds_bytes, (uint64_t)(uintptr_t)rcp,
                             kd_group | ((uint64_t)cx.opt_early_wave << 8) | ((uint64_t)Q << 32) | ((uint64_t)opt_group << 48) | ((uint64_t)pipe_on << 56) | ((uint64_t)lag_on << 57) |
                                 ((uint64_t)kd_lazy << 58) | ((uint64_t)(kd_lazy && cx.opt_gtrack_side) << 59) | ((uint64_t)cx.opt_commit_flat << 60)};
    if (!cx.graph_exec || memcmp(key, cx.graph_key, sizeof key)) {
        const double t0 = now_s();
        if (cx.graph_exec) { (void)hipGraphExecDestroy(cx.graph_exec); cx.graph_exec = nullptr; }
        hipGraph_t g = nullptr;
        size_t ev_used = 0;
        HIPCHK_CTX(&cx, hipStreamBeginCapture(cx.stream, hipStreamCaptureModeThreadLocal));
        (void)launch_steps(n_iter, false, ev_used);
        HIPCHK_CTX(&cx, hipStreamEndCapture(cx.stream, &g));
        HIPCHK_CTX(&cx, hipGraphInstantiate(&cx.graph_exec, g, nullptr, nullptr, 0));
        (void)hipGraphDestroy(g);
        memcpy(cx.graph_key, key, sizeof key);
// ... 3794 lines not shown
int64_t porrt_tamp_batch_bnb_nodes(const porrt_ctx *cc, uint32_t plan, int64_t *parents, int32_t *targets, double *ec, uint8_t *pushed, uint64_t cap) {
    const AstarBatchPlan *B = astar_batch_plan_of(cc, plan, true);
    if (!B) return PORRT_ERR_INVALID;
    const uint64_t n = B->node_parents.size();
    if (cap < n) return (int64_t)n;
    if (parents) memcpy(parents, B->node_parents.data(), n * sizeof(int64_t));
    if (targets) memcpy(targets, B->node_targets.data(), n * sizeof(int32_t));
    if (ec) memcpy(ec, B->node_ec.data(), n * sizeof(double));
    if (pushed) memcpy(pushed, B->node_pushed.data(), n);
    return (int64_t)n;
}

int porrt_tamp_shortcut_paths_resident(porrt_ctx *c, const double *xy, const uint64_t *offsets, uint64_t n_paths, double *out) {
    if (!c || !offsets || !out || (!xy && offsets[n_paths])) return PORRT_ERR_INVALID;
    if (!c->has_grid) { c->set_err("tamp_shortcut: the shortcut checks segments on the context's grid (porrt_set_grid)"); return PORRT_ERR_INVALID; }
    if (offsets[0] != 0) { c->set_err("tamp_shortcut: offsets[0] must be 0"); return PORRT_ERR_INVALID; }
    for (uint64_t i = 0; i < n_paths; ++i) if (offsets[i + 1] < offsets[i]) { c->set_err("tamp_shortcut: offsets must not decrease"); return PORRT_ERR_INVALID; }
    if (offsets[n_paths] >= (1ull << 31)) { c->set_err("tamp_shortcut: too many states"); return PORRT_ERR_INVALID; }
    return abi_guard([&]() {
        std::vector<double> v(xy, xy + 2 * offsets[n_paths]);
        std::vector<uint64_t> off(offsets, offsets + n_paths + 1);
        const int r = tamp_shortcut_resident(c, tamp_state(c), v, off);
        if (r < 0) return r;
        memcpy(out, v.data(), v.size() * sizeof(double));
        return (int)PORRT_OK;
    });
}

int porrt_solutions(porrt_ctx *const *ctxs, uint32_t n_ctx, uint64_t *n_solutions, uint64_t *n_states, uint64_t *ids, uint64_t *lens,
                    double *costs, uint64_t cap_solutions, double *xy, uint64_t cap_states) {
    if (!ctxs || !n_ctx) return PORRT_ERR_INVALID;
    for (uint32_t q = 0; q < n_ctx; ++q) if (!ctxs[q]) return PORRT_ERR_INVALID;
    porrt_ctx *c = ctxs[0];
    if (ids && (!lens || !costs || !xy)) { c->set_err("solutions: ids, lens, costs and xy go together"); return PORRT_ERR_INVALID; }
    return abi_guard([&]() {
        TampState &T = tamp_state(c);
        SolGather G;
        int r = solutions_select(c, T, ctxs, n_ctx, G);
        if (r < 0) return r;
        for (uint32_t q = 0; q < n_ctx; ++q) {
            const bool has = G.rows[q].status == kSolOk;
            if (n_solutions) n_solutions[q] = has ? G.rows[q].count : 0;
            if (n_states) n_states[q] = has ? G.rows[q].n_states : 0;
        }
        if (!ids) return (int)PORRT_OK;
        if (G.n_solutions > cap_solutions || G.n_states > cap_states) {
            c->set_err("solutions: " + std::to_string(G.n_solutions) + " solutions of " + std::to_string(G.n_states) + " states do not fit the caps");
            return (int)PORRT_ERR_CAPACITY;
        }
        return solutions_write(c, T, G, ids, lens, costs, xy);
    });
}

int porrt_best_paths(porrt_ctx *const *ctxs, uint32_t n_ctx, double *xy, uint64_t cap, uint64_t *lens, double *costs) {
    if (!ctxs || !n_ctx || !lens) return PORRT_ERR_INVALID;
    for (uint32_t q = 0; q < n_ctx; ++q) if (!ctxs[q]) return PORRT_ERR_INVALID;
    porrt_ctx *c = ctxs[0];
    return abi_guard([&]() {
        std::vector<std::vector<double>> paths;
        std::vector<double> cs;
        std::vector<char> ok;
        const int r = tamp_gather(c, tamp_state(c), ctxs, n_ctx, paths, cs, ok);
        if (r < 0) return r;
        uint64_t at = 0;
        for (uint32_t q = 0; q < n_ctx; ++q) {
            lens[q] = ok[q] ? paths[q].size() / 2 : 0;
            if (costs) costs[q] = ok[q] ? cs[q] : std::numeric_limits<double>::infinity();
            if (xy && at + lens[q] <= cap) memcpy(xy + 2 * at, paths[q].data(), paths[q].size() * sizeof(double));
            at += lens[q];
        }
        return at <= cap || !xy ? (int)PORRT_OK : (int)PORRT_ERR_CAPACITY;
    });
}

int porrt_tamp_shortcut_paths(porrt_ctx *c, const double *xy, const uint64_t *offsets, uint64_t n_paths, double *out) {
    if (!c || !offsets || !out || (!xy && offsets[n_paths])) return PORRT_ERR_INVALID;
    if (!c->has_grid) { c->set_err("tamp_shortcut: the shortcut checks segments on the context's grid (porrt_set_grid)"); return PORRT_ERR_INVALID; }
    if (offsets[0] != 0) { c->set_err("tamp_shortcut: offsets[0] must be 0"); return PORRT_ERR_INVALID; }
    for (uint64_t i = 0; i < n_paths; ++i) if (offsets[i + 1] < offsets[i]) { c->set_err("tamp_shortcut: offsets must not decrease"); return PORRT_ERR_INVALID; }
    return abi_guard([&]() {
        std::vector<double> v(xy, xy + 2 * offsets[n_paths]);
        std::vector<uint64_t> off(offsets, offsets + n_paths + 1);
        const int r = tamp_shortcut_device(c, tamp_state(c), v, off, nullptr);
        if (r < 0) return r;
        memcpy(out, v.data(), v.size() * sizeof(double));
        return (int)PORRT_OK;
    });
}

int porrt_get_metrics(const porrt_ctx *c, porrt_metrics *out) {
    if (!c || !out) return PORRT_ERR_INVALID;
    *out = c->metrics;
    return PORRT_OK;
}

int porrt_selftest(porrt_ctx *c, uint64_t n, uint64_t *sqrt_mismatch, uint64_t *div_mismatch) {
    if (!c || !n) return PORRT_ERR_INVALID;
    std::vector<double> a(n), b(n), rs(n), rd(n);
    Pcg64 r;
    r.seed_from_u64(12345);
    for (uint64_t i = 0; i < n; ++i) {
        double u = r.gen_range_f64(0.0, 1.0), v = r.gen_range_f64(0.0, 1.0);
        int e = (int)(r.next_u64() % 80) - 40;
        a[i] = ldexp(u, (i % 3 == 0) ? e : ((i % 3 == 1) ? -10 : 2));
        b[i] = ldexp(v + 1e-3, (i % 5 == 0) ? -e : 0);
    }
    double *da = nullptr, *db = nullptr, *ds = nullptr, *dd = nullptr;
    if (hipSetDevice(c->device) != hipSuccess) return PORRT_ERR_DEVICE;
    if (hipMalloc((void **)&da, n * 8) != hipSuccess || hipMalloc((void **)&db, n * 8) != hipSuccess ||
        hipMalloc((void **)&ds, n * 8) != hipSuccess || hipMalloc((void **)&dd, n * 8) != hipSuccess) {
        c->set_err("selftest: hipMalloc");
        return PORRT_ERR_DEVICE;
    }
    (void)hipMemcpy(da, a.data(), n * 8, hipMemcpyHostToDevice);
    (void)hipMemcpy(db, b.data(), n * 8, hipMemcpyHostToDevice);
    hipLaunchKernelGGL(k_selftest, dim3((unsigned)((n + 255) / 256)), dim3(256), 0, c->stream, da, db, ds, dd, (unsigned long long)n);
    (void)hipStreamSynchronize(c->stream);
    hipError_t e1 = hipMemcpy(rs.data(), ds, n * 8, hipMemcpyDeviceToHost);
    hipError_t e2 = hipMemcpy(rd.data(), dd, n * 8, hipMemcpyDeviceToHost);
    (void)hipFree(da); (void)hipFree(db); (void)hipFree(ds); (void)hipFree(dd);
    if (e1 != hipSuccess || e2 != hipSuccess) { c->set_err("selftest: copy back"); return PORRT_ERR_DEVICE; }
    uint64_t ms = 0, md = 0;
    for (uint64_t i = 0; i < n; ++i) {
        volatile double hs = sqrt(a[i]), hd = a[i] / b[i];
        double xs = hs, xd = hd;
        if (memcmp(&xs, &rs[i], 8)) ++ms;
        if (memcmp(&xd, &rd[i], 8)) ++md;
    }
    if (sqrt_mismatch) *sqrt_mismatch = ms;
    if (div_mismatch) *div_mismatch = md;
    return PORRT_OK;
}

porrt_tree_device_view porrt_tree_device(const porrt_ctx *c) {
    porrt_tree_device_view v;
    memset(&v, 0, sizeof v);
    if (!c || !c->have_results || c->mode != PORRT_MODE_RRT) return v;
    v.nx = c->d_nx.p; v.ny = c->d_ny.p; v.dist_root = c->d_distA.p; v.parent = c->d_parent.p; v.n_nodes = c->n_nodes;
    return v;
}

int porrt_get_option(const porrt_ctx *c, const char *name, int64_t *value) {
    if (!c || !name || !value) return PORRT_ERR_INVALID;
    if (!strcmp(name, "launch_mode")) *value = c->last_launch_mode;
    else if (!strcmp(name, "pipeline")) *value = c->seq.lag_on ? 4 : (c->seq.pipe_on ? 1 : 0);
    else if (!strcmp(name, "group_lanes")) *value = c->seq.opt_group;
    else if (!strcmp(name, "kd_lazy")) *value = c->seq.kd_lazy ? 1 : 0;
    else if (!strcmp(name, "kd_lca_steps")) *value = (int64_t)c->counters.lca_next;
    else if (!strcmp(name, "compactions")) *value = c->n_compactions;
    else if (!strcmp(name, "kd_built_after")) *value = c->seq.kd_built_after;
    else if (!strcmp(name, "n_heavy")) *value = (int64_t)c->counters.n_heavy;
    else if (!strcmp(name, "conn_wg_waves")) *value = c->opt_conn_wg_waves;
    else if (!strcmp(name, "conn_riders_first")) *value = c->opt_conn_riders_first ? 1 : 0;
    else if (!strcmp(name, "nn_wg_waves")) *value = c->opt_nn_wg_waves;
    else if (!strcmp(name, "commit_flat")) *value = c->opt_commit_flat;
    else if (!strcmp(name, "cand_cap")) *value = c->opt_cand_cap;
    else if (!strcmp(name, "edge_per_node")) *value = (int64_t)c->edge_per_node;
    else if (!strcmp(name, "tie_pool_ids")) *value = (int64_t)c->tie_pool_ids;
    else if (!strcmp(name, "tie_pooled_ids")) *value = (int64_t)c->counters.pool_n;
    else if (!strcmp(name, "tie_records")) *value = (int64_t)c->counters.pend_cnt;
    else if (!strcmp(name, "dp_wide_rows")) *value = (int64_t)c->opt_dp_wide_rows;
    else if (!strcmp(name, "dp_levels")) *value = c->dp.valid ? (int64_t)c->dp.levels : 0;
    else if (!strcmp(name, "tamp_streams")) *value = c->opt_tamp_streams;
    else if (!strcmp(name, "tamp_wave")) *value = c->opt_tamp_wave;
    else if (!strcmp(name, "tamp_pool")) *value = c->opt_tamp_pool;
    else if (!strcmp(name, "tamp_search")) *value = c->opt_tamp_search;
    else if (!strcmp(name, "tamp_arena_states")) *value = (int64_t)c->opt_tamp_arena_states;
    else if (!strcmp(name, "prm_rows")) *value = c->opt_prm_rows;
    else if (!strcmp(name, "prm_xcd_rows")) *value = c->opt_prm_xcd_rows;
    else if (!strcmp(name, "qmdp_max_states")) *value = c->opt_qmdp_max_states;
    else if (!strcmp(name, "policy_graph_max_pivots")) *value = c->opt_policy_graph_max_pivots;
    else if (!strcmp(name, "policy_max_nodes")) *value = c->opt_policy_max_nodes;
    else if (!strcmp(name, "plan_batch_max_belief_nodes")) *value = (int64_t)c->opt_plan_batch_max_belief_nodes;
    else if (!strcmp(name, "plan_batch_host_ranks")) *value = c->opt_plan_batch_host_ranks;
    else if (!strcmp(name, "mm_plan_batch_max_nodes")) *value = (int64_t)c->opt_mm_plan_batch_max_nodes;
    else if (!strcmp(name, "refine_short_lds")) *value = c->opt_refine_short_lds ? 1 : 0;
    else if (!strcmp(name, "reparent_max_tree_nodes")) *value = c->opt_reparent_max_tree_nodes;
    else if (!strcmp(name, "reparent_max_pops_per_node")) *value = c->opt_reparent_max_pops_per_node;
    else if (!strcmp(name, "dp_wide_levels")) *value = c->dp.valid ? (int64_t)c->dp.wide_levels : 0;
    else return PORRT_ERR_INVALID;
    return PORRT_OK;
}

int porrt_set_option(porrt_ctx *c, const char *name, int64_t value) {
    if (!c || !name) return PORRT_ERR_INVALID;
    if (!strcmp(name, "profile")) c->opt_profile = value != 0;
    else if (!strcmp(name, "cand_cap")) c->opt_cand_cap = (uint32_t)std::max<int64_t>(64, std::min<int64_t>(value, 1 << 26));
    else if (!strcmp(name, "edge_per_node")) { if (value < 1 || value > 65536) { c->set_err("edge_per_node: 1 .. 65536"); return PORRT_ERR_INVALID; } c->edge_per_node = (uint64_t)value; }
    else if (!strcmp(name, "tie_pool_ids")) { if (value < 0 || value > (1ll << 30)) { c->set_err("tie_pool_ids: 0 (the default pool) or 1 .. 2^30"); return PORRT_ERR_INVALID; } c->tie_pool_ids = (uint64_t)value; }
    else if (!strcmp(name, "graph")) c->opt_graph = value != 0;
    else if (!strcmp(name, "group_lanes")) { if (value != -1 && value != 0 && value != 16 && value != 32 && value != 64) { c->set_err("group_lanes: -1 (auto), 0, 16, 32 or 64"); return PORRT_ERR_INVALID; } c->opt_group_req = (int)value; }
    else if (!strcmp(name, "dp_sweeps")) c->opt_dp_sweeps = value != 0;
    else if (!strcmp(name, "dp_wide_rows")) c->opt_dp_wide_rows = (uint64_t)std::max<int64_t>(0, value);
    else if (!strcmp(name, "mm_levels")) c->mmp.use_levels = value != 0;
    else if (!strcmp(name, "mm_lds_nodes")) c->mmp.lds_cap = (uint32_t)std::max<int64_t>(0, std::min<int64_t>(value, kMmLdsNodes));
    else if (!strcmp(name, "box_table")) { c->opt_box_table = value != 0; c->cls_dirty = true; }
    else if (!strcmp(name, "refine_short_lds")) c->opt_refine_short_lds = value != 0;
    else if (!strcmp(name, "reparent_max_tree_nodes")) { if (value < 1 || value > (int64_t)kReparentMaxTreeNodesLimit) { c->set_err("reparent_max_tree_nodes: 1 .. 2^15"); return PORRT_ERR_INVALID; } c->opt_reparent_max_tree_nodes = (uint32_t)value; }
    else if (!strcmp(name, "reparent_max_pops_per_node")) { if (value < 1 || value > 64) { c->set_err("reparent_max_pops_per_node: 1 .. 64"); return PORRT_ERR_INVALID; } c->opt_reparent_max_pops_per_node = (uint32_t)value; }
    else if (!strcmp(name, "gtrack_side")) c->opt_gtrack_side = value != 0;
    else if (!strcmp(name, "pipeline")) {
#ifndef PORRT_DEV_NONCOOP
        if (value == 3) { c->set_err("pipeline = 3 (non-cooperative persistent launch) is a developer build option"); return PORRT_ERR_INVALID; }
#endif
        c->opt_pipeline = (value >= 2 && value <= 4) ? (int)value : (value ? 1 : 0);
    }
    else if (!strcmp(name, "batch_streams")) c->opt_batch_streams = (uint32_t)std::max<int64_t>(0, std::min<int64_t>(value, 8));
    else if (!strcmp(name, "kd_after")) c->opt_kd_after = value != 0;
    else if (!strcmp(name, "kd_ride")) c->opt_kd_ride = value != 0;
    else if (!strcmp(name, "kd_lazy")) c->opt_kd_lazy = value == 2 ? 2 : (value != 0);
    else if (!strcmp(name, "kd_claim_threads")) { if (value != 0 && value != 256 && value != 512 && value != 1024) return PORRT_ERR_INVALID; c->opt_claim_threads = (uint32_t)value; }
    else if (!strcmp(name, "kd_inline")) c->opt_kd_inline = value != 0;
    else if (!strcmp(name, "compact_rows")) c->opt_compact = value != 0;
    else if (!strcmp(name, "fetch_workers")) c->opt_fetch_workers = (uint32_t)std::max<int64_t>(1, std::min<int64_t>(value, 32));
    else if (!strcmp(name, "tree_out_blocks")) c->opt_tree_out_blocks = (uint32_t)std::max<int64_t>(1, std::min<int64_t>(value, 1024));
    else if (!strcmp(name, "host_ranks")) { c->opt_host_ranks = value != 0; c->eo.tag = ~0ull; }
    else if (!strcmp(name, "early_wave_steps")) c->opt_early_wave = (uint32_t)std::max<int64_t>(0, std::min<int64_t>(value, 64));
    else if (!strcmp(name, "conn_wg_waves")) { if (value != 1 && value != 4) { c->set_err("conn_wg_waves: 1 or 4"); return PORRT_ERR_INVALID; } c->opt_conn_wg_waves = (uint32_t)value; }
    else if (!strcmp(name, "conn_riders_first")) c->opt_conn_riders_first = value != 0;
    else if (!strcmp(name, "nn_wg_waves")) { if (value != 1 && value != 4) { c->set_err("nn_wg_waves: 1 or 4"); return PORRT_ERR_INVALID; } c->opt_nn_wg_waves = (uint32_t)value; }
    else if (!strcmp(name, "commit_flat")) { if (value != 0 && value != 1) { c->set_err("commit_flat: 0 or 1"); return PORRT_ERR_INVALID; } c->opt_commit_flat = (uint32_t)value; }
    else if (!strcmp(name, "kd_group")) c->opt_kd_group = (uint32_t)std::max<int64_t>(0, std::min<int64_t>(value, 8));
    else if (!strcmp(name, "tamp_streams")) { if (value != 0 && value != 1) { c->set_err("tamp_streams: 0 or 1"); return PORRT_ERR_INVALID; } c->opt_tamp_streams = (int)value; }
    else if (!strcmp(name, "tamp_wave")) { if (value < 1 || value > 65536) { c->set_err("tamp_wave: 1 .. 65536"); return PORRT_ERR_INVALID; } c->opt_tamp_wave = (uint32_t)value; }
    else if (!strcmp(name, "tamp_pool")) { if (value < 1 || value > 4096) { c->set_err("tamp_pool: 1 .. 4096"); return PORRT_ERR_INVALID; } c->opt_tamp_pool = (uint32_t)value; }
    else if (!strcmp(name, "tamp_arena_states")) { if (value < 1024 || value > (1ll << 31)) { c->set_err("tamp_arena_states: 1024 (one row's gather) .. 2^31"); return PORRT_ERR_INVALID; } c->opt_tamp_arena_states = (uint64_t)value; }
    else if (!strcmp(name, "tamp_search")) { if (value < 0 || value > 2) { c->set_err("tamp_search: 0 (BranchAndBound), 1 (AStar), 2 (BranchAndBoundMultipleViewPoints)"); return PORRT_ERR_INVALID; } c->opt_tamp_search = (int)value; }
    else if (!strcmp(name, "prm_rows")) { if (value < 1 || value > 4096) { c->set_err("prm_rows: 1 .. 4096"); return PORRT_ERR_INVALID; } c->opt_prm_rows = (uint32_t)value; }
    else if (!strcmp(name, "prm_xcd_rows")) c->opt_prm_xcd_rows = value != 0;
    else if (!strcmp(name, "policy_max_nodes")) { if (value < 1 || value > (int64_t)kPolMaxNodesLimit) { c->set_err("policy_max_nodes: 1 .. 2^24"); return PORRT_ERR_INVALID; } c->opt_policy_max_nodes = (uint32_t)value; }
    else if (!strcmp(name, "plan_batch_max_belief_nodes")) { if (value < 1 || value > (int64_t)kJoinBeliefNodesLimit) { c->set_err("plan_batch_max_belief_nodes: 1 .. 2^32 - 2"); return PORRT_ERR_INVALID; } c->opt_plan_batch_max_belief_nodes = (uint64_t)value; }
    else if (!strcmp(name, "plan_batch_host_ranks")) c->opt_plan_batch_host_ranks = value != 0;
    else if (!strcmp(name, "mm_plan_batch_max_nodes")) { if (value < 1 || value > (int64_t)kMmBatchNodesLimit) { c->set_err("mm_plan_batch_max_nodes: 1 .. 2^31 - 2"); return PORRT_ERR_INVALID; } c->opt_mm_plan_batch_max_nodes = (uint64_t)value; }
    else if (!strcmp(name, "policy_graph_max_pivots")) { if (value < 0 || value > (int64_t)0x7FFFFFFF) { c->set_err("policy_graph_max_pivots: 0 .. 2^31 - 1"); return PORRT_ERR_INVALID; } c->opt_policy_graph_max_pivots = (uint32_t)value; }
    else if (!strcmp(name, "qmdp_max_states")) { if (value < 1 || value > (int64_t)0x7FFFFFFF) { c->set_err("qmdp_max_states: 1 .. 2^31 - 1"); return PORRT_ERR_INVALID; } c->opt_qmdp_max_states = (uint32_t)value; }
    else { c->set_err(std::string("unknown option ") + name); return PORRT_ERR_INVALID; }
    if (strcmp(name, "profile") && c->graph_exec) { (void)hipGraphExecDestroy(c->graph_exec); c->graph_exec = nullptr; }
    return PORRT_OK;
}

}

#include "porrt_exchange.hpp"
#include "porrt_formats.hpp"
```

### po_rrt_amd/csrc/porrt_group.hpp

```cpp
#pragma once
#include "porrt_device.hpp"
#include "porrt_span.hpp"

namespace porrt {


template <int GL, int R, bool WITHD, class Visit>
__device__ __forceinline__ void gscan_disc(const RunConst &rc, uint32_t b, const GTeam<GL> &tm, double qx, double qy, double rho, uint32_t N, Visit visit,
                                           uint32_t skip_region = 0xFFFFFFFFu) {
    const uint32_t gl = tm.gl;
    int cx0, cy0, cx1, cy1;
    rep_cell(rc, qx - rho, qy - rho, kRG, cx0, cy0);
    rep_cell(rc, qx + rho, qy + rho, kRG, cx1, cy1);
    const uint32_t x0 = (uint32_t)cx0, y0 = (uint32_t)cy0;
    const uint32_t w = (uint32_t)(cx1 - cx0 + 1), nreg = w * (uint32_t)(cy1 - cy0 + 1);
    constexpr int U = (int)kPage / GL;
    if (nreg * 16u > N) {
        auto gx = as_global(rc.nx), gy = as_global(rc.ny), gdA = as_global(rc.distA);
        for (uint32_t j0 = 0; j0 < N; j0 += (uint32_t)(U * GL)) {
            double x[U], y[U], d[U];
#pragma unroll
            for (int u = 0; u < U; ++u) {
                const uint32_t j = j0 + (uint32_t)(GL * u) + gl;
                x[u] = gx[j < N ? j : 0u];
// ... 392 lines not shown
        }
        span_prefix_lane(s_prefix, tid, c, incl - s);
    }
    auto gdA = as_global(rc.distA);
    auto gpd = as_global(rc.pg_d);
    auto gso = as_global(rc.slot_of);
    for (uint32_t t = tid; t < kSpan; t += T)
        if (k0 + t < limit && span_valid(words, t)) {
            const uint32_t id = base + span_rank_in(words, t);
            gpd[gso[id]] = gdA[id];
        }
    __syncthreads();
    const uint32_t total = s_prefix[kSpan];
    auto gcid = as_global(rc.cand_id);
    auto gcval = as_global(rc.cand_val);
    auto gdB = as_global(rc.distB);
    constexpr int U = 4;
    for (uint32_t r0 = tid; r0 < total; r0 += T * (uint32_t)U) {
        double via[U], dB[U];
        int j[U], id[U];
#pragma unroll
        for (int u = 0; u < U; ++u) {
            const uint32_t r = r0 + (uint32_t)u * T;
            via[u] = -1.0; j[u] = 0; id[u] = 0;
            if (r < total) {
                const uint32_t t = span_find(s_prefix, r), a = r - s_prefix[t];
                via[u] = gcval[cand_val_off(rc, cb, k0 + t) + a];
                j[u] = gcid[cand_off(rc, cb, k0 + t) + a];
                id[u] = (int)(base + span_rank_in(words, t));
            }
        }
#pragma unroll
        for (int u = 0; u < U; ++u) dB[u] = via[u] >= 0.0 ? gdB[j[u]] : 0.0;
#pragma unroll
        for (int u = 0; u < U; ++u) {
            if (!(via[u] >= 0.0) || f64_bits(via[u]) != f64_bits(dB[u])) continue;
            auto gpar = as_global(rc.parent) + j[u];
            int old = *gpar;
            while (old < N || id[u] < old) {
                int expect = old;
                if (__hip_atomic_compare_exchange_strong(gpar, &expect, id[u], __ATOMIC_RELAXED, __ATOMIC_RELAXED, __HIP_MEMORY_SCOPE_AGENT)) break;
                old = expect;
            }
            gdA[j[u]] = via[u];
            gpd[gso[j[u]]] = via[u];
        }
    }
}

#ifndef PORRT_NN2_WAVES
#define PORRT_NN2_WAVES 5
#endif
template <int GL, int WV = 4>
__global__ __launch_bounds__(WV * 64) __attribute__((amdgpu_waves_per_eu(PORRT_NN2_WAVES, 8))) void k_nn2(const RunConst *__restrict__ rcp, uint32_t b, uint32_t i0, uint32_t nb, uint32_t vwords, uint32_t cb,
                                             uint32_t cnb, uint32_t cflat) {
    static_assert(GL == 16 || GL == 32 || GL == 64, "group size");
    constexpr uint32_t SPB = (uint32_t)WV * 64u / GL;
    uint32_t bx = blockIdx.x, by = blockIdx.y;
    xcd_swizzle(bx, by);
    const RunConst &rc = rc_const(rcp + by);
    GTeam<GL> tm;
    tm.gl = threadIdx.x % GL;
    tm.base = (threadIdx.x & 63u) - tm.gl;
    const uint32_t near_blocks = (nb + SPB - 1u) / SPB;
    if (bx >= near_blocks) {
        if (cflat) {
            PORRT_T0();
            commit_flat_span<(uint32_t)WV * 64u>(rc, cb, vwords, cnb, bx - near_blocks);
            PORRT_TACC_A(rc, 4);
            return;
        }
        const uint32_t ck = (bx - near_blocks) * SPB + threadIdx.x / GL;
        PORRT_T0();
        if (ck < cnb && ck < row_nb(rc, cb, cnb)) commit_rrt_sample(rc, cb, vwords, ck, tm.gl, GL);
        PORRT_TACC_A(rc, 4);
        return;
    }
    const uint32_t slot = bx * SPB + threadIdx.x / GL;
    if (slot >= row_nb(rc, b, nb)) return;
    PORRT_T0();
    const size_t so = (size_t)b * rc.part_stride + slot;
    const uint32_t k = as_global(rc.perm)[so];
    const uint32_t N = as_global(rc.n_at)[b];
    const double sqx = as_global(rc.ssx)[so], sqy = as_global(rc.ssy)[so];
    (void)i0;
    int nn = -1;
    double fx = 0.0, fy = 0.0;
    bool easy = false;
    const double lim = 0.7 * rc.max_step, t2b = as_global(rc.t2_at)[b];
    const double lim2 = lim * lim < t2b ? lim * lim : t2b;
    uint32_t err = 0;
    int cls_own = CLS_FREE;
    if (rc.has_grid) cls_own = state_class(rc, sqx, sqy, &err);
    const double perr = 1.3e-7 * (fabs(sqx) + fabs(sqy) + 2.0 * lim);
    const double limf = lim - perr, limf2 = limf > 0.0 ? (limf * limf < t2b ? limf * limf : t2b * (1.0 - 1e-6)) : -1.0;
    (void)lim2;
    for (int l = 0; l < 2 && !easy; ++l) {
        int cx, cy;
        const int G = rep_dim(l);
        rep_cell(rc, sqx, sqy, G, cx, cy);
        bool near = false;
        if (tm.gl < 9u) {
            const int x = cx + (int)(tm.gl % 3u) - 1, y = cy + (int)(tm.gl / 3u) - 1;
            if (x >= 0 && y >= 0 && x < G && y < G) {
                const flt2 pf = as_global(rc.rep_f)[rep_off(l) + y * G + x];
                near = dist2((double)pf.x, (double)pf.y, sqx, sqy) <= limf2;
            }
        }
        easy = tm.ballot(near) != 0ull;
    }
    PORRT_TACC_A(rc, 0);
    if (!easy) group_nn<GL>(rc, b, tm, N, sqx, sqy, nn, fx, fy);
    PORRT_TACC_A(rc, 1);
    double tx = sqx, ty = sqy;
    if (!easy) {
        double step = fabs(tx - fx);
        step += fabs(ty - fy);
        if (step > rc.max_step) {
            const double lambda = rc.max_step / step;
            double ux = (tx - fx) * lambda, uy = (ty - fy) * lambda;
            tx = fx + ux;
            ty = fy + uy;
        }
    }
    bool valid = true;
    if (rc.has_grid) {
        int cls = cls_own;
        if (tx != sqx || ty != sqy) { err = 0; cls = state_class(rc, tx, ty, &err); }
        valid = cls == CLS_FREE && !err;
    }
    PORRT_TACC_A(rc, 2);
    if (tm.gl == 0) {
        as_global(rc.q_x)[k] = tx;
        as_global(rc.q_y)[k] = ty;
        const size_t o2 = (size_t)b * rc.part_stride + k;
        as_global(rc.kq_x)[o2] = tx; as_global(rc.kq_y)[o2] = ty; as_global(rc.kq_vid)[o2] = valid ? 0 : -1;
        as_global(rc.q_nn)[k] = nn;
        int qv = valid ? 0 : -1;
        if (valid && rc.goal_kind != 0 && tx == rc.gp_x && ty == rc.gp_y) {
            const uint32_t slot = atomicAdd(&rc.cnt->clone_n, 1u);
            if (slot < 64u) { rc.cnt->clone_k[slot] = k; qv = 1; }
        }
        as_global(rc.q_vid)[k] = qv;
        as_global(rc.bq_x)[slot] = tx; as_global(rc.bq_y)[slot] = ty; as_global(rc.bq_k)[slot] = qv == 0 ? (uint16_t)k : (uint16_t)0xFFFFu;
        if (valid) atomicOr(&rc.valid_mask[(size_t)b * vwords + (k >> 6)], 1ull << (k & 63u));
        if (err) atomicOr(&rc.cnt->err, err);
    }
}

__host__ __device__ inline size_t conn2_lds_bytes(uint32_t GL) {
    (void)GL;
    return (64u / 16u) * kHitBytes;
}
__host__ __device__ inline size_t conn2_riders_lds_bytes() { return kInsertLds > kGTrackLds ? kInsertLds : kGTrackLds; }
__host__ __device__ inline size_t conn2_wg4_lds_bytes(uint32_t GL) {
    const size_t a = 4u * conn2_lds_bytes(GL);
    static_assert(kGTrackLds <= 4u * (64u / 16u) * kHitBytes, "g_track_step uses the same bytes");
    return a > kInsertLds ? a : kInsertLds;
}

template <int GL>
__device__ __attribute__((noinline)) int group_nn_call(const RunConst &rc_arg, uint32_t b, uint32_t gl, uint32_t base, uint32_t N, double px, double py) {
    const RunConst &rc = rc_const(rc_arg);
    GTeam<GL> tm;
    tm.gl = gl; tm.base = base;
    int nn;
    double fx, fy;
    group_nn<GL>(rc, b, tm, N, px, py, nn, fx, fy);
    return nn;
}
__device__ __attribute__((noinline)) int wave_nn(const RunConst &rc_arg, uint32_t b, uint32_t N, double px, double py) {
    const RunConst &rc = rc_const(rc_arg);
    GTeam<64> t64;
    t64.gl = threadIdx.x & 63u;
    t64.base = 0;
    int nn;
    double fx, fy;
    group_nn<64>(rc, b, t64, N, px, py, nn, fx, fy);
    return nn;
}

__device__ __forceinline__ void list_scan_wave(const RunConst &rc, uint32_t b, uint32_t N, double T2, uint32_t kh, double pxh, double pyh, uint32_t lane,
                                               uint32_t &err) {
    auto cid = as_global(rc.cand_id) + cand_off(rc, b, kh);
    auto cxy = as_global(reinterpret_cast<dbl2 *>(rc.cand_xy)) + cand_off(rc, b, kh);
    const uint32_t cap = rc.cand_cap;
    uint32_t tot = 0;
    bool over = false;
    scan_disc(rc, b, pxh, pyh, disc_radius(T2, pxh, pyh), uni(N), lane, [&](double x, double y, int jd, bool ok) {
        const bool in = ok && dist2(x, y, pxh, pyh) <= T2;
        const unsigned long long hm = __ballot(in);
        const uint32_t pos = tot + (uint32_t)__popcll(hm & ((1ull << lane) - 1ull));
        if (in) {
            if (pos < cap) {
                cid[pos] = jd;
                dbl2 v;
                v.x = x; v.y = y;
                cxy[pos] = v;
            } else {
                over = true;
            }
        }
        tot += (uint32_t)__popcll(hm);
    });
    if (lane == 0) as_global(rc.cand_cnt)[cand_cnt_at(rc, b, kh)] = tot;
    if (over) err |= (uint32_t)ERR_CAND_OVERFLOW;
}

__device__ __attribute__((noinline)) void clone_workgroup(const RunConst &rc_arg, uint32_t b, uint32_t vwords, uint32_t N, double T2) {
    const RunConst &rc = rc_const(rc_arg);
    __shared__ double s_d[kConnectWaves];
    __shared__ int s_i[kConnectWaves];
    __shared__ uint32_t s_cid[64], s_ck[64];
    const uint32_t lane = threadIdx.x & 63u, wv = threadIdx.x >> 6;
    uint32_t err = 0;
    uint32_t n = rc.cnt->clone_n;
    n = n < 64u ? n : 64u;
    if (n == 0) return;
    if (threadIdx.x < n) {
        const uint32_t kc = rc.cnt->clone_k[threadIdx.x];
        s_ck[threadIdx.x] = kc;
        s_cid[threadIdx.x] = N + rank_before(rc, b, vwords, kc);
    }
    __syncthreads();
    if (threadIdx.x == 0) {
        uint32_t lead = 0;
        for (uint32_t t = 1; t < n; ++t) if (s_cid[t] < s_cid[lead]) lead = t;
        const uint32_t ti = s_cid[0], tk = s_ck[0];
        s_cid[0] = s_cid[lead]; s_ck[0] = s_ck[lead]; s_cid[lead] = ti; s_ck[lead] = tk;
        rc.cnt->clone_n = 0;
    }
    __syncthreads();
    const uint32_t kh = uni(s_ck[0]), idh = uni(s_cid[0]);
    if (threadIdx.x >= 1 && threadIdx.x < n) as_global(rc.cand_cnt)[cand_cnt_at(rc, b, s_ck[threadIdx.x])] = 0u;
    const double pxh = uni_d(as_global(rc.q_x)[kh]), pyh = uni_d(as_global(rc.q_y)[kh]);
    if (wv == 0) {
        list_scan_wave(rc, b, N, T2, kh, pxh, pyh, lane, err);
        __threadfence();
    }
    __syncthreads();
    const uint32_t hc = cand_count(rc, b, kh);
    TableGrid grid;
    grid.p = rc.cls; grid.W = rc.W;
    Team<kConnectWaves> tmh;
    tmh.scr_d = s_d; tmh.scr_i = s_i; tmh.wave = wv; tmh.lane = lane;
    connect_rrt_sample(rc, tmh, global_list(rc, b, kh), grid, b, kh, idh, pxh, pyh, hc, err, s_cid + 1, n - 1u, -1,
                       [&]() { return wave_nn(rc, b, N, pxh, pyh); });
    if (err) atomicOr(&rc.cnt->err, err);
}

__device__ __forceinline__ MemHits mem_hits(const RunConst &rc, uint32_t b, uint32_t k) {
    MemHits M;
    M.sid = as_global(rc.cand_id) + cand_off(rc, b, k);
    M.sxy = as_global(reinterpret_cast<dbl2 *>(rc.cand_xy)) + cand_off(rc, b, k);
    M.sd = as_global(rc.cand_val) + cand_val_off(rc, b, k);
    M.out_id = M.sid;
    M.out_val = M.sd;
    M.out_cnt = as_global(rc.cand_cnt) + cand_cnt_at(rc, b, k);
    M.out_cap = rc.cand_cap;
    return M;
}

template <int GL>
__device__ __attribute__((noinline)) void heavy_sample_wave(const RunConst &rc_arg, uint32_t b, uint32_t N, uint32_t kh, uint32_t idh, uint32_t toth, int clrh,
                                                            double pxh, double pyh, uint8_t *wb, uint32_t &err) {
    const RunConst &rc = rc_const(rc_arg);
    const uint32_t lane = threadIdx.x & 63u;
    constexpr uint32_t kWaveHits = (64u / (uint32_t)GL) * (kLdsHits * (uint32_t)(GL / 16));
    Team<1> tw;
    tw.scr_d = nullptr; tw.scr_i = nullptr; tw.wave = 0; tw.lane = lane;
    TableGrid grid;
    grid.p = rc.cls; grid.W = rc.W;
    const uint32_t cap = rc.cand_cap;
    const MemHits Mh = mem_hits(rc, b, kh);
    PORRT_T0();
    if (toth <= kWaveHits) {
        LdsHits Wl;
        Wl.hx = reinterpret_cast<double *>(wb);
        Wl.hy = Wl.hx + kWaveHits;
        Wl.hd = Wl.hy + kWaveHits;
        Wl.hid = reinterpret_cast<int *>(Wl.hd + kWaveHits);
        Wl.out_id = Mh.out_id; Wl.out_val = Mh.out_val; Wl.out_cnt = Mh.out_cnt; Wl.out_cap = Mh.out_cap;
        for (uint32_t a0 = 0; a0 < toth; a0 += 256u) {
            int jd[4];
            dbl2 v[4];
            double d[4];
#pragma unroll
            for (uint32_t u = 0; u < 4u; ++u) {
                const uint32_t a = a0 + u * 64u + lane;
                jd[u] = a < toth ? Mh.sid[a] : 0;
                v[u] = a < toth ? Mh.sxy[a] : dbl2{0.0, 0.0};
                d[u] = a < toth ? Mh.sd[a] : 0.0;
            }
#pragma unroll
            for (uint32_t u = 0; u < 4u; ++u) {
                const uint32_t a = a0 + u * 64u + lane;
                if (a < toth) { Wl.hid[a] = jd[u]; Wl.hx[a] = v[u].x; Wl.hy[a] = v[u].y; Wl.hd[a] = d[u]; }
            }
        }
        __builtin_amdgcn_wave_barrier();
        PORRT_TACC_H(rc, 0);
        connect_rrt_sample(rc, tw, Wl, grid, b, kh, idh, pxh, pyh, toth, err, nullptr, 0, clrh, [&]() { return wave_nn(rc, b, N, pxh, pyh); });
        __builtin_amdgcn_wave_barrier();
        PORRT_TACC_H(rc, 3);
    } else {
        connect_rrt_sample(rc, tw, Mh, grid, b, kh, idh, pxh, pyh, toth < cap ? toth : cap, err, nullptr, 0, clrh,
                           [&]() { return wave_nn(rc, b, N, pxh, pyh); });
    }
}

#ifndef PORRT_CONN2_WAVES
#define PORRT_CONN2_WAVES 4
#endif
template <int GL>
__device__ __forceinline__ void conn2_wave(const RunConst &rc, uint32_t b, uint32_t vwords, uint32_t N, double T2, uint32_t k, double px, double py, uint8_t *wl) {
    const uint32_t lane = threadIdx.x & 63u;
    GTeam<GL> tm;
    tm.gl = threadIdx.x % GL;
    tm.base = lane - tm.gl;
    const bool act = k != 0xFFFFu;
    uint32_t err = 0;
    PORRT_T0();
    uint32_t id = 0, tot = 0;
    int clr_b = 0;
    bool heavy = false;
    const uint32_t cap = rc.cand_cap;
    TableGrid grid;
    grid.p = rc.cls; grid.W = rc.W;
    if (act) {
        id = N + rank_before_lanes(rc, b, vwords, k, tm.gl, (uint32_t)GL);
        if (rc.has_grid) {
            uint32_t bi, bj;
            to_pixel(rc, px, py, bi, bj);
            if (bi < rc.H && bj < rc.W) clr_b = as_global(rc.clr)[bi * rc.W + bj];
        }
        constexpr uint32_t kHits = kLdsHits * (uint32_t)(GL / 16);
        uint8_t *hb = wl + (lane / (uint32_t)GL) * (kHits * 28u);
        LdsHits L;
        L.hx = reinterpret_cast<double *>(hb);
        L.hy = L.hx + kHits;
        L.hd = L.hy + kHits;
        L.hid = reinterpret_cast<int *>(L.hd + kHits);
        const MemHits M = mem_hits(rc, b, k);
        L.out_id = M.out_id; L.out_val = M.out_val; L.out_cnt = M.out_cnt; L.out_cap = M.out_cap;
        PORRT_TACC_B(rc, 0);
        gscan_disc<GL, 1, true>(rc, b, tm, px, py, disc_radius(T2, px, py), N, [&](double x, double y, double dA, int jd, bool ok) {
            const bool in = ok && dist2(x, y, px, py) <= T2;
            const unsigned long long hm = tm.ballot(in);
            const uint32_t pos = tot + (uint32_t)__popcll(hm & ((1ull << tm.gl) - 1ull));
            if (in) {
                if (pos < kHits) { L.hid[pos] = jd; L.hx[pos] = x; L.hy[pos] = y; L.hd[pos] = dA; }
                else if (pos < cap) { M.sid[pos] = jd; dbl2 v; v.x = x; v.y = y; M.sxy[pos] = v; M.sd[pos] = dA; }
                else err |= (uint32_t)ERR_CAND_OVERFLOW;
            }
            tot += (uint32_t)__popcll(hm);
        });
        __builtin_amdgcn_wave_barrier();
        PORRT_TACC_B(rc, 1);
        if (tot <= kHits) {
            connect_rrt_sample(rc, tm, L, grid, b, k, id, px, py, tot, err, nullptr, 0, clr_b,
                               [&]() { return group_nn_call<GL>(rc, b, tm.gl, tm.base, N, px, py); });
            PORRT_TACC_B(rc, 2);
        } else {
            heavy = true;
            if (tm.gl == 0) atomicAdd(&rc.cnt->n_heavy, 1u);
            for (uint32_t a = tm.gl; a < kHits; a += (uint32_t)GL) {
                M.sid[a] = L.hid[a];
                dbl2 v;
                v.x = L.hx[a]; v.y = L.hy[a];
                M.sxy[a] = v;
                M.sd[a] = L.hd[a];
            }
        }
    }
    unsigned long long hv = __ballot(heavy && tm.gl == 0);
    if (hv) {
        __builtin_amdgcn_s_waitcnt(0x0F70);
        __builtin_amdgcn_wave_barrier();
        while (hv) {
            const int l = (int)__builtin_ctzll(hv);
            hv &= hv - 1;
            const uint32_t kh = uni((uint32_t)__shfl((int)k, l)), idh = uni((uint32_t)__shfl((int)id, l)), toth = uni((uint32_t)__shfl((int)tot, l));
            const int clrh = (int)uni((uint32_t)__shfl(clr_b, l));
            const double pxh = uni_d(__shfl(px, l)), pyh = uni_d(__shfl(py, l));
            heavy_sample_wave<GL>(rc, b, N, kh, idh, toth, clrh, pxh, pyh, wl, err);
        }
        PORRT_TACC_B(rc, 3);
    }
    if (err) atomicOr(&rc.cnt->err, err);
}

template <int GL>
__global__ __launch_bounds__(64) __attribute__((amdgpu_waves_per_eu(PORRT_CONN2_WAVES, 8))) void k_conn2(const RunConst *__restrict__ rcp, uint32_t b, uint32_t nb, uint32_t vwords) {
    static_assert(GL == 16 || GL == 32 || GL == 64, "group size");
    constexpr uint32_t SPB = 64u / GL;
    extern __shared__ __attribute__((aligned(16))) uint8_t lds_dyn[];
    uint32_t bx = blockIdx.x, by = blockIdx.y;
    xcd_swizzle(bx, by);
    const RunConst &rc = rc_const(rcp + by);
    nb = row_nb(rc, b, nb);
    const uint32_t slot = bx * SPB + threadIdx.x / GL;
    if (bx * SPB >= nb) return;
    const uint32_t N = as_global(rc.n_at)[b];
    const double T2 = as_global(rc.t2_at)[b];
    uint32_t k = 0xFFFFu;
    double px = 0.0, py = 0.0;
    if (slot < nb) { k = as_global(rc.bq_k)[slot]; px = as_global(rc.bq_x)[slot]; py = as_global(rc.bq_y)[slot]; }
    conn2_wave<GL>(rc, b, vwords, N, T2, k, px, py, lds_dyn);
}

__global__ __launch_bounds__(256) __attribute__((amdgpu_waves_per_eu(PORRT_CONN2_WAVES, 8))) void k_conn2_riders(const RunConst *__restrict__ rcp, uint32_t b, uint32_t nb, uint32_t vwords, uint32_t lazy) {
    extern __shared__ __attribute__((aligned(16))) uint8_t lds_dyn[];
    const RunConst &rc = rc_const(rcp + blockIdx.y);
    const uint32_t role = blockIdx.x;
    nb = row_nb(rc, b, nb);
    if (nb == 0) return;
    if (role == 0) { insert_step_pages<1>(rc, b, nb, vwords, lds_dyn); return; }
    if (lazy && role == 2u) { g_track_step<1>(rc, b, nb, vwords, lds_dyn); return; }
    clone_workgroup(rc, b, vwords, as_global(rc.n_at)[b], as_global(rc.t2_at)[b]);
}

template <int GL>
__global__ __launch_bounds__(256) __attribute__((amdgpu_waves_per_eu(PORRT_CONN2_WAVES, 8))) void k_conn2_wg4(const RunConst *__restrict__ rcp, uint32_t b, uint32_t nb, uint32_t vwords, uint32_t lazy) {
    static_assert(GL == 16 || GL == 32 || GL == 64, "group size");
    constexpr uint32_t SPB = 256u / GL;
    extern __shared__ __attribute__((aligned(16))) uint8_t lds_dyn[];
    uint32_t bx = blockIdx.x, by = blockIdx.y;
    const uint32_t ns = lazy ? 3u : 2u;
    const uint32_t role = xcd_swizzle_roles(bx, by, ns);
    const RunConst &rc = rc_const(rcp + by);
    nb = row_nb(rc, b, nb);
    if (nb == 0) return;
    if (role == 0) { insert_step_pages<1>(rc, b, nb, vwords, lds_dyn); return; }
    if (lazy && role == 2u) { g_track_step<1>(rc, b, nb, vwords, lds_dyn); return; }
    const uint32_t slot = bx * SPB + threadIdx.x / GL;
    const uint32_t N = as_global(rc.n_at)[b];
    const double T2 = as_global(rc.t2_at)[b];
    uint32_t k = 0xFFFFu;
    double px = 0.0, py = 0.0;
    if (role == ns && slot < nb) { k = as_global(rc.bq_k)[slot]; px = as_global(rc.bq_x)[slot]; py = as_global(rc.bq_y)[slot]; }
    if (role == 1) { clone_workgroup(rc, b, vwords, N, T2); return; }
    conn2_wave<GL>(rc, b, vwords, N, T2, k, px, py, lds_dyn + (threadIdx.x >> 6) * conn2_lds_bytes(GL));
}

template <int GL>
__global__ __launch_bounds__(256) void k_commit2(const RunConst *__restrict__ rcp, uint32_t b, uint32_t nb, uint32_t vwords) {
    const RunConst &rc = rc_const(rcp + blockIdx.y);
    const uint32_t k = (blockIdx.x * 256u + threadIdx.x) / GL;
    if (k < nb && k < row_nb(rc, b, nb)) commit_rrt_sample(rc, b, vwords, k, threadIdx.x % GL, GL);
}
__global__ __launch_bounds__(256) __attribute__((amdgpu_waves_per_eu(8, 8))) void k_commit_flat(const RunConst *__restrict__ rcp, uint32_t b, uint32_t nb, uint32_t vwords) {
    commit_flat_span<256u>(rc_const(rcp + blockIdx.y), b, vwords, nb, blockIdx.x);
}

}
```

Before: 332.2 million.

## Speed up rider roles: multi-wave clone scan, fused file step, single-pass g-track

Adds a 'fast' flag to the rider kernels. When it is set, the clone workgroup splits its disc scan across four waves using a shared LDS atomic counter, the file rider uses a grouped file_step_fast for small batches, and g_track gets a single-pass variant that fuses compaction with the kd binary search and keeps candidate coordinates in registers. The aim is to shorten the serial critical path of the rider blocks that run alongside conn2. In exchange it adds code complexity, LDS atomics and new error-handling paths, and candidate order may differ from the single-wave version.

Result: faster. 339.8 million (median of 6 runs) (+2.3%).

```diff
diff --git a/po_rrt_amd/csrc/porrt_device.hpp b/po_rrt_amd/csrc/porrt_device.hpp
--- a/po_rrt_amd/csrc/porrt_device.hpp
+++ b/po_rrt_amd/csrc/porrt_device.hpp
@@ -155,6 +155,10 @@
 #else
 #define PORRT_TACC_H(rc, slot) do {} while (0)
 #define PORRT_TACC_S(rc, slot) do {} while (0)
+#endif
+#if defined(PORRT_TIMING) && PORRT_TIMING == 5
+#undef PORRT_TACC_B
+#define PORRT_TACC_B(rc, slot) do { (void)t__0; } while (0)
 #endif
 
 struct BestCost {
@@ -665,7 +669,7 @@
 
 template <class Visit>
 __device__ __forceinline__ void scan_disc(const RunConst &rc, uint32_t b, double qx, double qy, double rho, uint32_t N, uint32_t lane, Visit visit,
-                                          uint32_t skip_region = 0xFFFFFFFFu) {
+                                          uint32_t skip_region = 0xFFFFFFFFu, uint32_t share = 0u, uint32_t nshare = 1u) {
     int cx0, cy0, cx1, cy1;
     rep_cell(rc, qx - rho, qy - rho, kRG, cx0, cy0);
     rep_cell(rc, qx + rho, qy + rho, kRG, cx1, cy1);
@@ -673,7 +677,7 @@
     const uint32_t w = uni((uint32_t)(cx1 - cx0 + 1)), nreg = w * uni((uint32_t)(cy1 - cy0 + 1));
     if (nreg * 16u > N) {
         auto gx = as_global(rc.nx), gy = as_global(rc.ny);
-        for (uint32_t j0 = 0; j0 < N; j0 += 128u) {
+        for (uint32_t j0 = share * 128u; j0 < N; j0 += nshare * 128u) {
             double x[2], y[2];
 #pragma unroll
             for (int u = 0; u < 2; ++u) {
@@ -701,6 +705,7 @@
         }
         const uint32_t npg = (uint32_t)__popcll(__ballot(cnt > 0u));
         if (__ballot(cnt >= npg || cnt > kPage) == 0ull && npg > 1u) {
+            if (nshare > 1u && r % nshare != share) cnt = 0u;
             uint32_t cmax = cnt;
             for (int off = 32; off > 0; off >>= 1) {
                 const uint32_t o = __shfl_xor(cmax, off);
@@ -726,6 +731,7 @@
         for (uint32_t j = 0;; ++j) {
             unsigned long long m = __ballot(cnt > j * kPage);
             if (!m) break;
+            if (nshare > 1u) m = __ballot(cnt > j * kPage && (r + j) % nshare == share);
             if (j && cnt > j * kPage) page = gdir[(size_t)reg * rc.rg_maxp + j];
             while (m) {
                 uint32_t pg[2], pc[2];
@@ -944,7 +950,7 @@
 }
 
 constexpr uint32_t kFileLds = 2u * kRegions * 4u + 4096u * 2u + 64u * 8u + 66u * 4u + 32u;
-template <uint32_t T = 1024u>
+template <uint32_t T = 1024u, uint32_t SPT = 4u, bool GROUP = false>
 __device__ void file_step_fast(const RunConst &rc_arg, uint32_t b, uint32_t nb, uint32_t vwords, uint8_t *scratch) {
     const RunConst &rc = rc_const(rc_arg);
     uint32_t *s_add = reinterpret_cast<uint32_t *>(scratch);
@@ -953,7 +959,6 @@
     unsigned long long *s_word = reinterpret_cast<unsigned long long *>(s_off + 4096);
     uint32_t *s_pref = reinterpret_cast<uint32_t *>(s_word + 64);
     uint32_t *s_misc = s_pref + 66;
-    constexpr uint32_t SPT = 4u;
     const uint32_t tid = threadIdx.x, qo = q_off(rc, b);
     auto rg_old = as_global(rc.rg_cnt) + (b & 1u) * kRegions, rg_new = as_global(rc.rg_cnt) + ((b + 1u) & 1u) * kRegions;
     int vid[SPT];
@@ -970,12 +975,12 @@
 #pragma unroll
     for (uint32_t h = 0; h < RPT; ++h) oldc[h] = tid + h * T < kRegions ? rg_old[tid + h * T] : 0u;
     const unsigned long long word = tid < vwords ? as_global(rc.valid_mask)[(size_t)b * vwords + tid] : 0ull;
-    uint32_t n_pages = 0, N0 = 0;
-    if (tid == T - 1u) { n_pages = rc.cnt->n_pages; N0 = as_global(rc.n_at)[b]; }
+    uint32_t n_pages = 0, N0 = 0, err0 = 0;
+    if (tid == T - 1u) { n_pages = rc.cnt->n_pages; N0 = as_global(rc.n_at)[b]; if (GROUP) err0 = rc.cnt->err & (uint32_t)ERR_PAGE_OVERFLOW; }
 #pragma unroll
     for (uint32_t h = 0; h < RPT; ++h) if (tid + h * T < kRegions) { s_add[tid + h * T] = 0; s_old[tid + h * T] = oldc[h]; }
     if (tid < 64u) s_word[tid] = word;
-    if (tid == T - 1u) { s_misc[0] = 0; s_misc[1] = kRegions + n_pages; s_misc[2] = 0; s_misc[3] = N0; }
+    if (tid == T - 1u) { s_misc[0] = 0; s_misc[1] = kRegions + n_pages; s_misc[2] = err0; s_misc[3] = N0; }
     __syncthreads();
     double t2_next = 0.0;
     if (tid == 0) {
@@ -1008,7 +1013,10 @@
     }
     __threadfence_block();
     __syncthreads();
-    if (s_misc[2]) return;
+    if (s_misc[2]) {
+        if (GROUP && tid == 0) as_global(rc.t2_at)[b + 1] = t2_next;
+        return;
+    }
     const uint32_t N = s_misc[3];
     dbl2 *pxy = reinterpret_cast<dbl2 *>(rc.pg_xy);
 #pragma unroll
@@ -1023,8 +1031,10 @@
         const uint32_t nid = N + s_pref[k >> 6] + (uint32_t)__popcll(s_word[k >> 6] & ((1ull << (k & 63u)) - 1ull));
         as_global(rc.pg_id)[(size_t)page * kPage + (slot % kPage)] = (int)nid;
         as_global(rc.slot_of)[nid] = page * kPage + (slot % kPage);
-        as_global(rc.nx)[nid] = x[q];
-        as_global(rc.ny)[nid] = y[q];
+        if (!GROUP || rc.q_stride) {
+            as_global(rc.nx)[nid] = x[q];
+            as_global(rc.ny)[nid] = y[q];
+        }
     }
 #pragma unroll
     for (uint32_t h = 0; h < RPT; ++h) {
@@ -2057,95 +2067,207 @@
     auto vm = as_global(rc.valid_mask) + (size_t)b * vwords;
     const uint32_t N = as_global(rc.n_at)[b];
     const uint32_t glen0 = rc.cnt->g_len, n_nd = rc.cnt->g_nd_len, d0 = rc.cnt->g_first_dup[0], d1 = rc.cnt->g_first_dup[1];
-    if (tid < 64u) s_cand[tid] = 0ull;
-    if (tid < 64u) {
-        const uint32_t c = tid < vwords ? (uint32_t)__popcll(vm[tid]) : 0u;
-        uint32_t inc = c;
-        for (int off = 1; off < 64; off <<= 1) { const uint32_t o = (uint32_t)__shfl_up((int)inc, off); if ((int)lane >= off) inc += o; }
-        if (tid < vwords) s_wpre[tid] = inc - c;
-        if (tid == 63u) s_wpre[vwords] = inc;
-    }
-    for (uint32_t t2 = tid; t2 < n_nd && t2 < kNd; t2 += blockDim.x) {
-        const KdBox bx = rc.g_nd_box[t2];
-        s_ndi[t2] = as_global(rc.g_nd)[t2]; s_blx[t2] = bx.lox; s_bhx[t2] = bx.hix; s_bly[t2] = bx.loy; s_bhy[t2] = bx.hiy;
-    }
-    __syncthreads();
-    const uint32_t n_new = s_wpre[vwords];
-    for (uint32_t k = tid; k < nb; k += blockDim.x) {
-        const unsigned long long w = vm[k >> 6];
-        if ((w >> (k & 63u)) & 1ull) s_k[s_wpre[k >> 6] + (uint32_t)__popcll(w & ((1ull << (k & 63u)) - 1ull))] = (uint16_t)k;
-    }
-    __syncthreads();
+    constexpr bool FAST = TAG == 2;
+    uint32_t n_new = 0;
+    if constexpr (!FAST) {
+        if (tid < 64u) s_cand[tid] = 0ull;
+        if (tid < 64u) {
+            const uint32_t c = tid < vwords ? (uint32_t)__popcll(vm[tid]) : 0u;
+            uint32_t inc = c;
+            for (int off = 1; off < 64; off <<= 1) { const uint32_t o = (uint32_t)__shfl_up((int)inc, off); if ((int)lane >= off) inc += o; }
+            if (tid < vwords) s_wpre[tid] = inc - c;
+            if (tid == 63u) s_wpre[vwords] = inc;
+        }
+        for (uint32_t t2 = tid; t2 < n_nd && t2 < kNd; t2 += blockDim.x) {
+            const KdBox bx = rc.g_nd_box[t2];
+            s_ndi[t2] = as_global(rc.g_nd)[t2]; s_blx[t2] = bx.lox; s_bhx[t2] = bx.hix; s_bly[t2] = bx.loy; s_bhy[t2] = bx.hiy;
+        }
+        __syncthreads();
+        n_new = s_wpre[vwords];
+        for (uint32_t k = tid; k < nb; k += blockDim.x) {
+            const unsigned long long w = vm[k >> 6];
+            if ((w >> (k & 63u)) & 1ull) s_k[s_wpre[k >> 6] + (uint32_t)__popcll(w & ((1ull << (k & 63u)) - 1ull))] = (uint16_t)k;
+        }
+        __syncthreads();
+    }
     const double px = rc.gp_x, py = rc.gp_y;
     auto gex = as_global(rc.kd_gexit);
     const uint32_t qo = q_off(rc, b);
     GT_MARK(0);
-    for (uint32_t t0 = tid; t0 < ((n_new + blockDim.x - 1u) / blockDim.x) * blockDim.x; t0 += 4u * blockDim.x) {
-        double cvx[4], cvy[4];
-        uint32_t cE[4], lo[4], hi[4];
-#pragma unroll
-        for (uint32_t u = 0; u < 4u; ++u) {
-            const uint32_t t = t0 + u * blockDim.x;
-            const uint32_t k = t < n_new ? s_k[t] : 0u;
-            cvx[u] = t < n_new ? as_global(rc.q_x)[qo + k] : 0.0;
-            cvy[u] = t < n_new ? as_global(rc.q_y)[qo + k] : 0.0;
-            cE[u] = 0xFFFFFFFFu;
-            const bool open = t < n_new && !(cvx[u] == px && cvy[u] == py);
-            lo[u] = 0u; hi[u] = open ? n_nd : 0u;
-        }
-        for (;;) {
-            bool more = false;
-#pragma unroll
-            for (uint32_t u = 0; u < 4u; ++u) more = more || lo[u] < hi[u];
-            if (!more) break;
-#pragma unroll
+    if constexpr (FAST) {
+        constexpr uint32_t SPT = 4u;
+        const uint32_t T = blockDim.x;
+        double cvx[SPT], cvy[SPT];
+        unsigned long long cw[SPT];
+        uint32_t tt[SPT];
+        auto load_chunk = [&](uint32_t k0) {
+#pragma unroll
+            for (uint32_t u = 0; u < SPT; ++u) {
+                const uint32_t k = k0 + tid + u * T;
+                cw[u] = k < nb ? vm[k >> 6] : 0ull;
+                cvx[u] = k < nb ? as_global(rc.q_x)[qo + k] : 0.0;
+                cvy[u] = k < nb ? as_global(rc.q_y)[qo + k] : 0.0;
+            }
+        };
+        const unsigned long long mword = tid < vwords && tid < 64u ? vm[tid] : 0ull;
+        load_chunk(0u);
+        const uint32_t n_stage = kNd < rc.g_cap ? kNd : rc.g_cap;
+        static_assert(kNd <= 256u, "one cell per thread");
+        KdBox sbx = g_box_all();
+        uint32_t sdi = 0u;
+        if (tid < n_stage) { sbx = rc.g_nd_box[tid]; sdi = as_global(rc.g_nd)[tid]; }
+        if (tid < 64u) {
+            s_cand[tid] = 0ull;
+            const uint32_t c = (uint32_t)__popcll(mword);
+            uint32_t inc = c;
+            for (int off = 1; off < 64; off <<= 1) { const uint32_t o = (uint32_t)__shfl_up((int)inc, off); if ((int)lane >= off) inc += o; }
+            if (tid < vwords) s_wpre[tid] = inc - c;
+            if (tid == 63u) s_wpre[vwords] = inc;
+        }
+        if (tid < n_stage && tid < n_nd) { s_ndi[tid] = sdi; s_blx[tid] = sbx.lox; s_bhx[tid] = sbx.hix; s_bly[tid] = sbx.loy; s_bhy[tid] = sbx.hiy; }
+        __syncthreads();
+        n_new = s_wpre[vwords];
+        for (uint32_t k0 = 0; k0 < nb; k0 += SPT * T) {
+            if (k0) load_chunk(k0);
+            uint32_t cE[SPT], lo[SPT], hi[SPT];
+#pragma unroll
+            for (uint32_t u = 0; u < SPT; ++u) {
+                const uint32_t k = k0 + tid + u * T;
+                const bool v = (cw[u] >> (k & 63u)) & 1ull;
+                tt[u] = v ? s_wpre[k >> 6] + (uint32_t)__popcll(cw[u] & ((1ull << (k & 63u)) - 1ull)) : 0xFFFFFFFFu;
+                if (v) s_k[tt[u]] = (uint16_t)k;
+                cE[u] = 0xFFFFFFFFu;
+                const bool open = v && !(cvx[u] == px && cvy[u] == py);
+                lo[u] = 0u; hi[u] = open ? n_nd : 0u;
+            }
+            for (;;) {
+                bool more = false;
+#pragma unroll
+                for (uint32_t u = 0; u < SPT; ++u) more = more || lo[u] < hi[u];
+                if (!more) break;
+#pragma unroll
+                for (uint32_t u = 0; u < SPT; ++u) {
+                    if (lo[u] >= hi[u]) continue;
+                    const uint32_t mid = (lo[u] + hi[u]) >> 1;
+                    double blx, bhx, bly, bhy;
+                    if (mid < kNd) { blx = s_blx[mid]; bhx = s_bhx[mid]; bly = s_bly[mid]; bhy = s_bhy[mid]; }
+                    else { const KdBox bx = rc.g_nd_box[mid]; blx = bx.lox; bhx = bx.hix; bly = bx.loy; bhy = bx.hiy; }
+                    const bool in = !(cvx[u] < blx) && cvx[u] < bhx && !(cvy[u] < bly) && cvy[u] < bhy;
+                    if (in) lo[u] = mid + 1u; else hi[u] = mid;
+                }
+            }
+#pragma unroll
+            for (uint32_t u = 0; u < SPT; ++u)
+                if (tt[u] != 0xFFFFFFFFu && !(cvx[u] == px && cvy[u] == py) && lo[u] < n_nd) cE[u] = lo[u] < kNd ? s_ndi[lo[u]] : as_global(rc.g_nd)[lo[u]];
+#pragma unroll
+            for (uint32_t u = 0; u < SPT; ++u) {
+                const uint32_t t = tt[u];
+                if (t == 0xFFFFFFFFu) continue;
+                uint32_t E = cE[u];
+                if (cvx[u] < px && d0 < E) E = d0;
+                if (cvy[u] < py && d1 < E) E = d1;
+                if (E != 0xFFFFFFFFu) gex[N + t] = E;
+                else atomicOr(&s_cand[t >> 6], 1ull << (t & 63u));
+            }
+        }
+        __syncthreads();
+        if (tid < 64u) {
+            const uint32_t c = (uint32_t)__popcll(s_cand[tid]);
+            uint32_t inc = c;
+            for (int off = 1; off < 64; off <<= 1) { const uint32_t o = (uint32_t)__shfl_up((int)inc, off); if ((int)lane >= off) inc += o; }
+            s_wpre[tid] = inc - c;
+        }
+        __syncthreads();
+        if (nb <= SPT * T) {
+#pragma unroll
+            for (uint32_t u = 0; u < SPT; ++u) {
+                const uint32_t t = tt[u];
+                if (t == 0xFFFFFFFFu) continue;
+                const unsigned long long w = s_cand[t >> 6];
+                if (!((w >> (t & 63u)) & 1ull)) continue;
+                const uint32_t rank = s_wpre[t >> 6] + (uint32_t)__popcll(w & ((1ull << (t & 63u)) - 1ull));
+                if (rank < kCand) { s_cx[rank] = cvx[u]; s_cy[rank] = cvy[u]; }
+            }
+        } else {
+            for (uint32_t t = tid; t < n_new; t += T) {
+                const unsigned long long w = s_cand[t >> 6];
+                if (!((w >> (t & 63u)) & 1ull)) continue;
+                const uint32_t rank = s_wpre[t >> 6] + (uint32_t)__popcll(w & ((1ull << (t & 63u)) - 1ull));
+                if (rank < kCand) { const uint32_t k = s_k[t]; s_cx[rank] = as_global(rc.q_x)[qo + k]; s_cy[rank] = as_global(rc.q_y)[qo + k]; }
+            }
+        }
+        __syncthreads();
+    }
+    if constexpr (!FAST) {
+        for (uint32_t t0 = tid; t0 < ((n_new + blockDim.x - 1u) / blockDim.x) * blockDim.x; t0 += 4u * blockDim.x) {
+            double cvx[4], cvy[4];
+            uint32_t cE[4], lo[4], hi[4];
+    #pragma unroll
             for (uint32_t u = 0; u < 4u; ++u) {
-                if (lo[u] >= hi[u]) continue;
-                const uint32_t mid = (lo[u] + hi[u]) >> 1;
-                double blx, bhx, bly, bhy;
-                if (mid < kNd) { blx = s_blx[mid]; bhx = s_bhx[mid]; bly = s_bly[mid]; bhy = s_bhy[mid]; }
-                else { const KdBox bx = rc.g_nd_box[mid]; blx = bx.lox; bhx = bx.hix; bly = bx.loy; bhy = bx.hiy; }
-                const bool in = !(cvx[u] < blx) && cvx[u] < bhx && !(cvy[u] < bly) && cvy[u] < bhy;
-                if (in) lo[u] = mid + 1u; else hi[u] = mid;
-            }
-        }
-        GT_MARK(4);
-#pragma unroll
-        for (uint32_t u = 0; u < 4u; ++u) {
-            const uint32_t t = t0 + u * blockDim.x;
-            if (t < n_new && !(cvx[u] == px && cvy[u] == py) && lo[u] < n_nd) cE[u] = lo[u] < kNd ? s_ndi[lo[u]] : as_global(rc.g_nd)[lo[u]];
-        }
-#pragma unroll
-        for (uint32_t u = 0; u < 4u; ++u) {
-            const uint32_t t = t0 + u * blockDim.x;
-            if (t >= n_new) continue;
-            uint32_t E = cE[u];
-            if (cvx[u] < px && d0 < E) E = d0;
-            if (cvy[u] < py && d1 < E) E = d1;
-            if (E != 0xFFFFFFFFu) gex[N + t] = E;
-            else atomicOr(&s_cand[t >> 6], 1ull << (t & 63u));
-        }
-    }
-    __syncthreads();
-    GT_MARK(5);
-    if (tid < 64u) {
-        const uint32_t c = (uint32_t)__popcll(s_cand[tid]);
-        uint32_t inc = c;
-        for (int off = 1; off < 64; off <<= 1) { const uint32_t o = (uint32_t)__shfl_up((int)inc, off); if ((int)lane >= off) inc += o; }
-        s_wpre[tid] = inc - c;
-    }
-    __syncthreads();
-    for (uint32_t t = tid; t < n_new; t += blockDim.x) {
-        const unsigned long long w = s_cand[t >> 6];
-        if (!((w >> (t & 63u)) & 1ull)) continue;
-        const uint32_t rank = s_wpre[t >> 6] + (uint32_t)__popcll(w & ((1ull << (t & 63u)) - 1ull));
-        if (rank < kCand) { const uint32_t k = s_k[t]; s_cx[rank] = as_global(rc.q_x)[qo + k]; s_cy[rank] = as_global(rc.q_y)[qo + k]; }
-    }
-    __syncthreads();
-    GT_MARK(1);
+                const uint32_t t = t0 + u * blockDim.x;
+                const uint32_t k = t < n_new ? s_k[t] : 0u;
+                cvx[u] = t < n_new ? as_global(rc.q_x)[qo + k] : 0.0;
+                cvy[u] = t < n_new ? as_global(rc.q_y)[qo + k] : 0.0;
+                cE[u] = 0xFFFFFFFFu;
+                const bool open = t < n_new && !(cvx[u] == px && cvy[u] == py);
+                lo[u] = 0u; hi[u] = open ? n_nd : 0u;
+            }
+            for (;;) {
+                bool more = false;
+    #pragma unroll
+                for (uint32_t u = 0; u < 4u; ++u) more = more || lo[u] < hi[u];
+                if (!more) break;
+    #pragma unroll
+                for (uint32_t u = 0; u < 4u; ++u) {
+                    if (lo[u] >= hi[u]) continue;
+                    const uint32_t mid = (lo[u] + hi[u]) >> 1;
+                    double blx, bhx, bly, bhy;
+                    if (mid < kNd) { blx = s_blx[mid]; bhx = s_bhx[mid]; bly = s_bly[mid]; bhy = s_bhy[mid]; }
+                    else { const KdBox bx = rc.g_nd_box[mid]; blx = bx.lox; bhx = bx.hix; bly = bx.loy; bhy = bx.hiy; }
+                    const bool in = !(cvx[u] < blx) && cvx[u] < bhx && !(cvy[u] < bly) && cvy[u] < bhy;
+                    if (in) lo[u] = mid + 1u; else hi[u] = mid;
+                }
+            }
+            GT_MARK(4);
+    #pragma unroll
+            for (uint32_t u = 0; u < 4u; ++u) {
+                const uint32_t t = t0 + u * blockDim.x;
+                if (t < n_new && !(cvx[u] == px && cvy[u] == py) && lo[u] < n_nd) cE[u] = lo[u] < kNd ? s_ndi[lo[u]] : as_global(rc.g_nd)[lo[u]];
+            }
+    #pragma unroll
+            for (uint32_t u = 0; u < 4u; ++u) {
+                const uint32_t t = t0 + u * blockDim.x;
+                if (t >= n_new) continue;
+                uint32_t E = cE[u];
+                if (cvx[u] < px && d0 < E) E = d0;
+                if (cvy[u] < py && d1 < E) E = d1;
+                if (E != 0xFFFFFFFFu) gex[N + t] = E;
+                else atomicOr(&s_cand[t >> 6], 1ull << (t & 63u));
+            }
+        }
+        __syncthreads();
+        GT_MARK(5);
+        if (tid < 64u) {
+            const uint32_t c = (uint32_t)__popcll(s_cand[tid]);
+            uint32_t inc = c;
+            for (int off = 1; off < 64; off <<= 1) { const uint32_t o = (uint32_t)__shfl_up((int)inc, off); if ((int)lane >= off) inc += o; }
+            s_wpre[tid] = inc - c;
+        }
+        __syncthreads();
+        for (uint32_t t = tid; t < n_new; t += blockDim.x) {
+            const unsigned long long w = s_cand[t >> 6];
+            if (!((w >> (t & 63u)) & 1ull)) continue;
+            const uint32_t rank = s_wpre[t >> 6] + (uint32_t)__popcll(w & ((1ull << (t & 63u)) - 1ull));
+            if (rank < kCand) { const uint32_t k = s_k[t]; s_cx[rank] = as_global(rc.q_x)[qo + k]; s_cy[rank] = as_global(rc.q_y)[qo + k]; }
+        }
+        __syncthreads();
+        GT_MARK(1);
+    }
     if (tid < 64u) {
         uint32_t len = glen0, nd_len = n_nd, fd0 = d0, fd1 = d1;
-        KdBox cell = n_nd ? rc.g_nd_box[n_nd - 1u] : g_box_all();
+        KdBox cell = g_box_all();
+        if (FAST && n_nd && n_nd - 1u < kNd) { cell.lox = s_blx[n_nd - 1u]; cell.hix = s_bhx[n_nd - 1u]; cell.loy = s_bly[n_nd - 1u]; cell.hiy = s_bhy[n_nd - 1u]; }
+        else if (n_nd) cell = rc.g_nd_box[n_nd - 1u];
         auto gx = as_global(reinterpret_cast<unsigned long long *>(rc.g_x)), gy = as_global(reinterpret_cast<unsigned long long *>(rc.g_y));
         uint32_t c_at = 0;
         for (uint32_t w = 0; w < (n_new + 63u) / 64u; ++w) {
diff --git a/po_rrt_amd/csrc/porrt_engine.hip b/po_rrt_amd/csrc/porrt_engine.hip
--- a/po_rrt_amd/csrc/porrt_engine.hip
+++ b/po_rrt_amd/csrc/porrt_engine.hip
@@ -113,6 +113,7 @@
     uint32_t opt_early_wave = 0;
     uint32_t opt_conn_wg_waves = 1;
     bool opt_conn_riders_first = true;
+    uint32_t opt_riders_fast = 1;
     uint32_t opt_nn_wg_waves = 4;
     uint32_t opt_commit_flat = 1;
     uint32_t opt_batch_streams = 0;
@@ -687,14 +688,14 @@
             const uint32_t spb = 256u / GLc;
             const dim3 g2((nb + spb - 1) / spb + 2 + lazy, Q);
             const size_t dyn = conn2_wg4_lds_bytes(GLc);
-            with_lanes(GLc, [&](auto gl) { hipLaunchKernelGGL(k_conn2_wg4<decltype(gl)::value>, g2, dim3(256), dyn, stream, rcp, b, nb, vwords, lazy); });
+            with_lanes(GLc, [&](auto gl) { hipLaunchKernelGGL(k_conn2_wg4<decltype(gl)::value>, g2, dim3(256), dyn, stream, rcp, b, nb, vwords, lazy, cx.opt_riders_fast); });
         } else {
             const uint32_t spb = 64u / GLc;
             const dim3 g2((nb + spb - 1) / spb, Q), gr(2 + lazy, Q);
             const size_t dyn = conn2_lds_bytes(GLc);
-            if (cx.opt_conn_riders_first) hipLaunchKernelGGL(k_conn2_riders, gr, dim3(256), conn2_riders_lds_bytes(), stream, rcp, b, nb, vwords, lazy);
+            if (cx.opt_conn_riders_first) hipLaunchKernelGGL(k_conn2_riders, gr, dim3(256), conn2_riders_lds_bytes(), stream, rcp, b, nb, vwords, lazy, cx.opt_riders_fast);
             with_lanes(GLc, [&](auto gl) { hipLaunchKernelGGL(k_conn2<decltype(gl)::value>, g2, dim3(64), dyn, stream, rcp, b, nb, vwords); });
-            if (!cx.opt_conn_riders_first) hipLaunchKernelGGL(k_conn2_riders, gr, dim3(256), conn2_riders_lds_bytes(), stream, rcp, b, nb, vwords, lazy);
+            if (!cx.opt_conn_riders_first) hipLaunchKernelGGL(k_conn2_riders, gr, dim3(256), conn2_riders_lds_bytes(), stream, rcp, b, nb, vwords, lazy, cx.opt_riders_fast);
         }
     } else if (lds_bytes) hipLaunchKernelGGL(k_connect_rrt<true>, cgrid, cblock, lds_bytes, stream, rcp, b, nb, vwords);
     else hipLaunchKernelGGL(k_connect_rrt<false>, cgrid, cblock, 0, stream, rcp, b, nb, vwords);
@@ -4795,6 +4796,8 @@
     else if (!strcmp(name, "n_heavy")) *value = (int64_t)c->counters.n_heavy;
     else if (!strcmp(name, "conn_wg_waves")) *value = c->opt_conn_wg_waves;
     else if (!strcmp(name, "conn_riders_first")) *value = c->opt_conn_riders_first ? 1 : 0;
+    else if (!strcmp(name, "riders_fast")) *value = c->opt_riders_fast;
+    else if (!strncmp(name, "tim", 3) && name[3] >= '0' && name[3] <= '9' && atoi(name + 3) < 16) *value = (int64_t)c->counters.tim[atoi(name + 3)];
     else if (!strcmp(name, "nn_wg_waves")) *value = c->opt_nn_wg_waves;
     else if (!strcmp(name, "commit_flat")) *value = c->opt_commit_flat;
     else if (!strcmp(name, "cand_cap")) *value = c->opt_cand_cap;
@@ -4861,6 +4864,7 @@
     else if (!strcmp(name, "early_wave_steps")) c->opt_early_wave = (uint32_t)std::max<int64_t>(0, std::min<int64_t>(value, 64));
     else if (!strcmp(name, "conn_wg_waves")) { if (value != 1 && value != 4) { c->set_err("conn_wg_waves: 1 or 4"); return PORRT_ERR_INVALID; } c->opt_conn_wg_waves = (uint32_t)value; }
     else if (!strcmp(name, "conn_riders_first")) c->opt_conn_riders_first = value != 0;
+    else if (!strcmp(name, "riders_fast")) { if (value != 0 && value != 1) { c->set_err("riders_fast: 0 or 1"); return PORRT_ERR_INVALID; } c->opt_riders_fast = (uint32_t)value; }
     else if (!strcmp(name, "nn_wg_waves")) { if (value != 1 && value != 4) { c->set_err("nn_wg_waves: 1 or 4"); return PORRT_ERR_INVALID; } c->opt_nn_wg_waves = (uint32_t)value; }
     else if (!strcmp(name, "commit_flat")) { if (value != 0 && value != 1) { c->set_err("commit_flat: 0 or 1"); return PORRT_ERR_INVALID; } c->opt_commit_flat = (uint32_t)value; }
     else if (!strcmp(name, "kd_group")) c->opt_kd_group = (uint32_t)std::max<int64_t>(0, std::min<int64_t>(value, 8));
diff --git a/po_rrt_amd/csrc/porrt_group.hpp b/po_rrt_amd/csrc/porrt_group.hpp
--- a/po_rrt_amd/csrc/porrt_group.hpp
+++ b/po_rrt_amd/csrc/porrt_group.hpp
@@ -568,12 +568,34 @@
     (void)GL;
     return (64u / 16u) * kHitBytes;
 }
-__host__ __device__ inline size_t conn2_riders_lds_bytes() { return kInsertLds > kGTrackLds ? kInsertLds : kGTrackLds; }
+static_assert(kInsertLds <= kFileLds && kGTrackLds <= kFileLds, "the filing's one-round-trip form is the largest of the riders' scratch areas");
+__host__ __device__ inline size_t conn2_riders_lds_bytes() { return kFileLds; }
 __host__ __device__ inline size_t conn2_wg4_lds_bytes(uint32_t GL) {
     const size_t a = 4u * conn2_lds_bytes(GL);
     static_assert(kGTrackLds <= 4u * (64u / 16u) * kHitBytes, "g_track_step uses the same bytes");
+    static_assert(kFileLds <= 4u * (64u / 16u) * kHitBytes, "file_step_fast uses the same bytes");
     return a > kInsertLds ? a : kInsertLds;
 }
+
+__device__ __forceinline__ void rider_file(const RunConst &rc, uint32_t b, uint32_t nb, uint32_t vwords, uint8_t *lds, uint32_t fast) {
+    if (fast && nb <= 4u * 256u) file_step_fast<256u, 4u, true>(rc, b, nb, vwords, lds);
+    else insert_step_pages<1>(rc, b, nb, vwords, lds);
+}
+__device__ __forceinline__ void rider_gtrack(const RunConst &rc, uint32_t b, uint32_t nb, uint32_t vwords, uint8_t *lds, uint32_t fast) {
+    if (fast) g_track_step<2>(rc, b, nb, vwords, lds);
+    else g_track_step<1>(rc, b, nb, vwords, lds);
+}
+#if defined(PORRT_TIMING) && PORRT_TIMING == 5
+#define RIDERS_T0() const unsigned long long rt__0 = wall_clock64(); const uint32_t rt__w = b < 8u ? 0u : ((rc.cnt->g_first_dup[0] & rc.cnt->g_first_dup[1]) != 0xFFFFFFFFu ? 2u : 1u)
+#define RIDERS_MARK(role)                                                                                          \
+    do {                                                                                                           \
+        __syncthreads();                                                                                           \
+        if (threadIdx.x == 0) { atomicAdd(&rc.cnt->tim[3u * (role) + rt__w], wall_clock64() - rt__0); if ((role) == 0u) atomicAdd(&rc.cnt->tim[9u + rt__w], 1ull); } \
+    } while (0)
+#else
+#define RIDERS_T0() do {} while (0)
+#define RIDERS_MARK(role) do {} while (0)
+#endif
 
 template <int GL>
 __device__ __attribute__((noinline)) int group_nn_call(const RunConst &rc_arg, uint32_t b, uint32_t gl, uint32_t base, uint32_t N, double px, double py) {
@@ -623,11 +645,42 @@
     if (over) err |= (uint32_t)ERR_CAND_OVERFLOW;
 }
 
-__device__ __attribute__((noinline)) void clone_workgroup(const RunConst &rc_arg, uint32_t b, uint32_t vwords, uint32_t N, double T2) {
+__device__ __forceinline__ void list_scan_waves(const RunConst &rc, uint32_t b, uint32_t N, double T2, uint32_t kh, double pxh, double pyh, uint32_t lane,
+                                                uint32_t wv, uint32_t *tot, uint32_t &err) {
+    auto cid = as_global(rc.cand_id) + cand_off(rc, b, kh);
+    auto cxy = as_global(reinterpret_cast<dbl2 *>(rc.cand_xy)) + cand_off(rc, b, kh);
+    const uint32_t cap = rc.cand_cap;
+    bool over = false;
+    scan_disc(rc, b, pxh, pyh, disc_radius(T2, pxh, pyh), uni(N), lane, [&](double x, double y, int jd, bool ok) {
+        const bool in = ok && dist2(x, y, pxh, pyh) <= T2;
+        const unsigned long long hm = __ballot(in);
+        if (!hm) return;
+        uint32_t base = 0;
+        if (lane == 0) base = atomicAdd(tot, (uint32_t)__popcll(hm));
+        const uint32_t pos = uni(base) + (uint32_t)__popcll(hm & ((1ull << lane) - 1ull));
+        if (in) {
+            if (pos < cap) {
+                cid[pos] = jd;
+                dbl2 v;
+                v.x = x; v.y = y;
+                cxy[pos] = v;
+            } else {
+                over = true;
+            }
+        }
+    }, 0xFFFFFFFFu, wv, kConnectWaves);
+    if (over) err |= (uint32_t)ERR_CAND_OVERFLOW;
+}
+
+#ifndef PORRT_CLONE_SCAN_WAVES
+#define PORRT_CLONE_SCAN_WAVES 4
+#endif
+__device__ __attribute__((noinline)) void clone_workgroup(const RunConst &rc_arg, uint32_t b, uint32_t vwords, uint32_t N, double T2, uint32_t fast) {
     const RunConst &rc = rc_const(rc_arg);
     __shared__ double s_d[kConnectWaves];
     __shared__ int s_i[kConnectWaves];
     __shared__ uint32_t s_cid[64], s_ck[64];
+    __shared__ uint32_t s_tot;
     const uint32_t lane = threadIdx.x & 63u, wv = threadIdx.x >> 6;
     uint32_t err = 0;
     uint32_t n = rc.cnt->clone_n;
@@ -645,17 +698,29 @@
         const uint32_t ti = s_cid[0], tk = s_ck[0];
         s_cid[0] = s_cid[lead]; s_ck[0] = s_ck[lead]; s_cid[lead] = ti; s_ck[lead] = tk;
         rc.cnt->clone_n = 0;
+        s_tot = 0;
     }
     __syncthreads();
     const uint32_t kh = uni(s_ck[0]), idh = uni(s_cid[0]);
     if (threadIdx.x >= 1 && threadIdx.x < n) as_global(rc.cand_cnt)[cand_cnt_at(rc, b, s_ck[threadIdx.x])] = 0u;
     const double pxh = uni_d(as_global(rc.q_x)[kh]), pyh = uni_d(as_global(rc.q_y)[kh]);
-    if (wv == 0) {
-        list_scan_wave(rc, b, N, T2, kh, pxh, pyh, lane, err);
-        __threadfence();
-    }
-    __syncthreads();
-    const uint32_t hc = cand_count(rc, b, kh);
+    uint32_t hc;
+    if (PORRT_CLONE_SCAN_WAVES == 4 && fast) {
+        list_scan_waves(rc, b, N, T2, kh, pxh, pyh, lane, wv, &s_tot, err);
+        __builtin_amdgcn_fence(__ATOMIC_RELEASE, "workgroup");
+        __syncthreads();
+        __builtin_amdgcn_fence(__ATOMIC_ACQUIRE, "workgroup");
+        const uint32_t tot = s_tot;
+        if (threadIdx.x == 0) as_global(rc.cand_cnt)[cand_cnt_at(rc, b, kh)] = tot;
+        hc = tot < rc.cand_cap ? tot : rc.cand_cap;
+    } else {
+        if (wv == 0) {
+            list_scan_wave(rc, b, N, T2, kh, pxh, pyh, lane, err);
+            __threadfence();
+        }
+        __syncthreads();
+        hc = cand_count(rc, b, kh);
+    }
     TableGrid grid;
     grid.p = rc.cls; grid.W = rc.W;
     Team<kConnectWaves> tmh;
@@ -825,19 +890,22 @@
     conn2_wave<GL>(rc, b, vwords, N, T2, k, px, py, lds_dyn);
 }
 
-__global__ __launch_bounds__(256) __attribute__((amdgpu_waves_per_eu(PORRT_CONN2_WAVES, 8))) void k_conn2_riders(const RunConst *__restrict__ rcp, uint32_t b, uint32_t nb, uint32_t vwords, uint32_t lazy) {
+__global__ __launch_bounds__(256) __attribute__((amdgpu_waves_per_eu(PORRT_CONN2_WAVES, 8))) void k_conn2_riders(const RunConst *__restrict__ rcp, uint32_t b, uint32_t nb, uint32_t vwords, uint32_t lazy,
+                                                                                                                  uint32_t fast) {
     extern __shared__ __attribute__((aligned(16))) uint8_t lds_dyn[];
     const RunConst &rc = rc_const(rcp + blockIdx.y);
     const uint32_t role = blockIdx.x;
     nb = row_nb(rc, b, nb);
     if (nb == 0) return;
-    if (role == 0) { insert_step_pages<1>(rc, b, nb, vwords, lds_dyn); return; }
-    if (lazy && role == 2u) { g_track_step<1>(rc, b, nb, vwords, lds_dyn); return; }
-    clone_workgroup(rc, b, vwords, as_global(rc.n_at)[b], as_global(rc.t2_at)[b]);
+    RIDERS_T0();
+    if (role == 0) rider_file(rc, b, nb, vwords, lds_dyn, fast);
+    else if (lazy && role == 2u) rider_gtrack(rc, b, nb, vwords, lds_dyn, fast);
+    else clone_workgroup(rc, b, vwords, as_global(rc.n_at)[b], as_global(rc.t2_at)[b], fast);
+    RIDERS_MARK(role);
 }
 
 template <int GL>
-__global__ __launch_bounds__(256) __attribute__((amdgpu_waves_per_eu(PORRT_CONN2_WAVES, 8))) void k_conn2_wg4(const RunConst *__restrict__ rcp, uint32_t b, uint32_t nb, uint32_t vwords, uint32_t lazy) {
+__global__ __launch_bounds__(256) __attribute__((amdgpu_waves_per_eu(PORRT_CONN2_WAVES, 8))) void k_conn2_wg4(const RunConst *__restrict__ rcp, uint32_t b, uint32_t nb, uint32_t vwords, uint32_t lazy, uint32_t fast) {
     static_assert(GL == 16 || GL == 32 || GL == 64, "group size");
     constexpr uint32_t SPB = 256u / GL;
     extern __shared__ __attribute__((aligned(16))) uint8_t lds_dyn[];
@@ -847,15 +915,15 @@
     const RunConst &rc = rc_const(rcp + by);
     nb = row_nb(rc, b, nb);
     if (nb == 0) return;
-    if (role == 0) { insert_step_pages<1>(rc, b, nb, vwords, lds_dyn); return; }
-    if (lazy && role == 2u) { g_track_step<1>(rc, b, nb, vwords, lds_dyn); return; }
+    if (role == 0) { rider_file(rc, b, nb, vwords, lds_dyn, fast); return; }
+    if (lazy && role == 2u) { rider_gtrack(rc, b, nb, vwords, lds_dyn, fast); return; }
     const uint32_t slot = bx * SPB + threadIdx.x / GL;
     const uint32_t N = as_global(rc.n_at)[b];
     const double T2 = as_global(rc.t2_at)[b];
     uint32_t k = 0xFFFFu;
     double px = 0.0, py = 0.0;
     if (role == ns && slot < nb) { k = as_global(rc.bq_k)[slot]; px = as_global(rc.bq_x)[slot]; py = as_global(rc.bq_y)[slot]; }
-    if (role == 1) { clone_workgroup(rc, b, vwords, N, T2); return; }
+    if (role == 1) { clone_workgroup(rc, b, vwords, N, T2, fast); return; }
     conn2_wave<GL>(rc, b, vwords, N, T2, k, px, py, lds_dyn + (threadIdx.x >> 6) * conn2_lds_bytes(GL));
 }
 
```
